# gvanhorn38/multibox

Hardware: AMD Instinct MI355X
Metric: images/sec (299x299, 5-AR priors) train (higher is better)
Workload: dtype bf16; 1 GPU; full train step: Inception-ResNet-v2 + multibox heads fwd, on-device matching+loss, bwd, RMSProp+EMA; 299x299, k=5 (P=646), BATCH_SIZE=64/GPU, MAX_NUM_BBOXES=13; global_batch=64, parallelism=dp1, hip_graph=True

## Files before the change

include/mbx.h:

```cpp
#ifndef MBX_H
#define MBX_H

#include <stddef.h>
#include <stdint.h>

#ifdef __cplusplus
extern "C" {
#endif

typedef void* mbx_stream_t;

typedef enum {
  MBX_OK = 0,
  MBX_ERR_INVALID_ARG = -1,
  MBX_ERR_UNSUPPORTED = -2,
  MBX_ERR_LAUNCH = -3,
  MBX_ERR_WORKSPACE = -4
} mbx_status;

int mbx_version(void);
const char* mbx_status_string(int status);

int mbx_priors_count(int k, const int* grids, int n_grids);

uint32_t mbx_crc32c(const void* data, uint64_t n, uint32_t crc);
int mbx_generate_priors(const double* aspect_ratios, int k, double min_scale, double max_scale,
                        int restrict_to_image_bounds, const int* grids, int n_grids,
                        double* out );

int mbx_decode_conf(const float* raw_locs , const float* logits ,
                    const float* priors , int B, int P, float eps_add,
                    float* decoded , float* conf , mbx_stream_t stream);

size_t mbx_match_workspace_bytes(int B, int P, int G);
int mbx_match(const float* decoded , const float* conf ,
              const float* gt , const int32_t* n_gt , float alpha,
              int B, int P, int G, int32_t* match , int32_t* status ,
              void* workspace, size_t workspace_bytes, mbx_stream_t stream);

size_t mbx_loss_workspace_bytes(int B);
int mbx_loss_fwd_bwd(const float* decoded , const float* conf_in ,
                     int conf_is_logit, const float* gt ,
                     const int32_t* match , float alpha, float grad_scale, int B, int P,
                     int G, float* loss2 ,
                     float* d_raw_locs , float* d_logits ,
                     void* workspace, size_t workspace_bytes, mbx_stream_t stream);

typedef struct {
  int32_t offset_y, offset_x;
  int32_t patch_h, patch_w;
  int32_t image_h, image_w;
  int32_t is_flipped;
  int32_t max_to_keep;
  float restrictions[4];
} mbx_patch_meta;

int mbx_decode_filter_topk(const float* raw_locs , const float* conf ,
                           const float* priors , const mbx_patch_meta* meta ,
                           int B, int P, int k_max, double* out_boxes ,
                           float* out_scores , int32_t* out_index ,
                           int32_t* out_count , mbx_stream_t stream);

int mbx_nms(double* boxes , float* scores , int32_t* index ,
            int32_t* count , int B, int k_max, double iou_threshold, mbx_stream_t stream);

#define MBX_MERGE_MAX_CANDIDATES 16384
int mbx_merge_detections(const double* boxes , const float* scores ,
                         const int32_t* count , const int32_t* image_rows , int I, int k_max,
                         int max_det, double iou_threshold, double* out_boxes ,
                         float* out_scores , int32_t* out_src ,
                         int32_t* out_count , int32_t* out_status , mbx_stream_t stream);

typedef enum {
  MBX_EPI_STORE = 0,
  MBX_EPI_AFFINE = 1,
  MBX_EPI_RESIDUAL = 2,
  MBX_EPI_STORE_F32 = 3
} mbx_epilogue;

typedef struct {
  int32_t n, rows_mod;
  int32_t c_begin[4];
  const void* y[4]; int32_t ld_y[4];
  const float* relu_thr[4];
  float* stats[4]; int32_t stats_ld[4];
} mbx_bn_bwd_stats;

#define MBX_GRID_BARRIER_BYTES 6400
typedef struct {
  void* barrier;
  void* a; int32_t ld_a;
  const float* beta;
  float* mean; float* rstd;
  float* moving_mean; float* moving_var;
  float* relu_thr;
  int32_t relu; float eps, decay;
  float* step_poison;
} mbx_bn_apply_desc;

#define MBX_BN_BWD_SLOTS 8
typedef struct {
  void* barrier;
  int32_t n;
  int32_t c_begin[4];
  const void* y[4]; int32_t ld_y[4];
  void* dy[4]; int32_t ld_dy[4];
  const float* mean[4]; const float* rstd[4]; const float* beta[4];
  float* dbeta[4];
  float* acc[4]; int32_t acc_ld[4];
  int32_t relu[4];
  float* step_poison;
} mbx_bn_bwd_fused;

typedef struct {
  const void* x; int64_t x_img_stride; int32_t ldx;
  int32_t N, H_in, W_in, C_in;
  const void* w; int32_t C_out, R, S;
  int32_t stride, transposed, pad_t, pad_l, H_out, W_out;
  void* y; int64_t y_img_stride; int32_t ldy;
  int32_t epilogue, relu, accumulate;
  const float* scale; const float* shift;
  const void* skip; int64_t skip_img_stride; int32_t ld_skip; float rscale;
  float* stats_partial;
  int32_t tile_config;
  const void* acc_src; int64_t acc_img_stride; int32_t ld_acc;
  int32_t* work_counter;
  int32_t max_workgroups;
  void* splitk_ws; int64_t splitk_ws_bytes;
  int32_t stats_rows_mod, stats_ld;
  const mbx_bn_bwd_stats* bn_bwd_stats;
  void* relu_bits; int32_t ld_bits;
  const mbx_bn_apply_desc* bn_apply;
  const mbx_bn_bwd_fused* bn_bwd;
} mbx_conv_desc;
#define MBX_CONV_TILE_CONFIGS 14

int mbx_conv_stats_rows(const mbx_conv_desc* desc );
int mbx_conv(const mbx_conv_desc* desc , mbx_stream_t stream);
int mbx_conv_supported(const mbx_conv_desc* desc );
int mbx_conv_pair(const mbx_conv_desc* a , const mbx_conv_desc* b , mbx_stream_t stream);
size_t mbx_conv_splitk_workspace_bytes(const mbx_conv_desc* desc );

int mbx_conv_wgrad(const mbx_conv_desc* desc , const void* dy,
                   int64_t dy_img_stride, int32_t ld_dy, float* dw, float* db, mbx_stream_t stream);

typedef struct {
  mbx_conv_desc desc;
  const void* dy; int64_t dy_img_stride; int32_t ld_dy;
  float scale;
  float* dw; float* db;
} mbx_wgrad_job;
typedef struct {
  int32_t n_layers, n_items;
  int64_t layers_off, items_off;
  int64_t queues_off, heads_off;
  double flops;
  int64_t tally_off;
} mbx_wgrad_plan_info;
#define MBX_WGRAD_DETERMINISTIC 1
#define MBX_WGRAD_SCATTER 2
size_t mbx_wgrad_plan_bytes(const mbx_wgrad_job* jobs , int n_jobs, int flags);
int mbx_wgrad_plan(const mbx_wgrad_job* jobs , int n_jobs, int flags, void* host_image, size_t bytes,
                   mbx_wgrad_plan_info* info );
int mbx_conv_wgrad_grouped(void* device_image , const mbx_wgrad_plan_info* info ,
                           mbx_stream_t stream);
int mbx_conv_wgrad_grouped_capped(void* device_image, const mbx_wgrad_plan_info* info , int max_workgroups,
                                  mbx_stream_t stream);

int mbx_conv_wgrad_scaled(const mbx_conv_desc* desc, const void* dy, int64_t dy_img_stride,
                          int32_t ld_dy, float scale, float* dw, float* db, mbx_stream_t stream);

int mbx_bn_finalize(const float* stats_partial , int rows, int C, int64_t count,
                    float eps, float decay, float* mean , float* rstd ,
                    float* moving_mean , float* moving_var ,
                    mbx_stream_t stream);
int mbx_bn_apply(const void* y, int64_t M, int C, const float* mean, const float* rstd,
                 const float* beta, int relu, void* a, int ld_a, mbx_stream_t stream);
int mbx_bn_apply_fused(const float* stats_partial, int rows, int64_t count, float eps, float decay,
                       const void* y, int64_t M, int C, const float* beta, int relu, void* a, int ld_a,
                       float* mean, float* rstd, float* moving_mean, float* moving_var,
                       mbx_stream_t stream);
int mbx_bn_apply_fused_mapped(const void* stats_fixed, int rows, int64_t count, float eps, float decay,
                              const void* y, int64_t M, int C, const float* beta, int relu, void* a, int ld_a,
                              const struct mbx_chan_map_s* a_map , float* mean, float* rstd, float* moving_mean,
                              float* moving_var, float* relu_thr, mbx_stream_t stream);
int mbx_bn_moving_update(float* moving_mean, float* moving_var, const float* batch_mean, const float* batch_var,
                         int64_t n, float decay, const float* skip_ctl, uint64_t* skipped_steps,
                         float* ema_mean, float* ema_var, float ema_decay, mbx_stream_t stream);
typedef struct mbx_chan_map_s { int32_t n; int32_t c_begin[4]; int32_t offset[4]; } mbx_chan_map;
int mbx_bn_finalize_parts(const float* const* parts , const int32_t* rows ,
                          const int32_t* Cs , int n_parts, int64_t count, float eps, float decay, float* mean,
                          float* rstd, float* moving_mean, float* moving_var, mbx_stream_t stream);
int mbx_bn_apply_mapped(const void* y, int64_t M, int C, const float* mean, const float* rstd, const float* beta,
                        int relu, void* a, int ld_a, const mbx_chan_map* a_map , mbx_stream_t stream);
int mbx_bn_apply_maxpool(const void* y, int N, int H, int W, int C, const float* mean, const float* rstd, const float* beta,
                         int relu, void* p, int64_t p_img_stride, int ld_p, int Ho, int Wo, uint8_t* argmax,
                         mbx_stream_t stream);
int mbx_bn_fold(const float* moving_mean, const float* moving_var, const float* beta, float eps,
                int C, float* scale, float* shift, mbx_stream_t stream);
int mbx_bn_bwd_rows(int64_t M, int C);
int mbx_bn_bwd_reduce(const void* da, int ld_da, const void* a, int ld_a, int relu, const void* y,
                      int64_t M, int C, const float* mean, const float* rstd, const float* beta,
                      float* partial , mbx_stream_t stream);
int mbx_bn_bwd_finalize(const float* partial, int rows, int C, int64_t M, float* dbeta ,
                        float* m12 , mbx_stream_t stream);
int mbx_bn_bwd_apply(const void* da, int ld_da, const void* a, int ld_a, int relu, const void* y,
                     int64_t M, int C, const float* mean, const float* rstd, const float* beta,
                     const float* m12, void* dy , mbx_stream_t stream);

int mbx_bn_bwd_reduce_mapped(const void* da, int ld_da, const void* a, int ld_a, int relu, const void* y, int64_t M, int C,
                             const float* mean, const float* rstd, const float* beta, float* partial,
                             const mbx_chan_map* da_map , mbx_stream_t stream);
int mbx_bn_bwd_apply_mapped(const void* da, int ld_da, const void* a, int ld_a, int relu, const void* y, int64_t M, int C,
                            const float* mean, const float* rstd, const float* beta, const float* m12, void* dy,
                            const mbx_chan_map* da_map , mbx_stream_t stream);

int mbx_bn_bwd_apply_rows(const float* stats, int rows, const void* da, int ld_da, const void* y, int64_t M, int C,
                          const float* mean, const float* rstd, const float* relu_thr, float* dbeta, void* dy,
                          const mbx_chan_map* da_map , mbx_stream_t stream);

size_t mbx_bn_bwd_onepass_workspace_bytes(int C);
int mbx_bn_bwd_onepass_supported(int64_t M, int C, int max_workgroups);
int mbx_bn_bwd_onepass(const void* da, int ld_da, int relu, const void* y, int64_t M, int C,
                       const float* mean, const float* rstd, const float* beta, float* dbeta ,
                       void* dy , void* ws, int max_workgroups, float* step_poison ,
                       mbx_stream_t stream);

int mbx_bn_bwd_rows_pooled(int N, int H, int W, int C);
int mbx_bn_bwd_reduce_pooled(const void* gy, int64_t gy_img_stride, int ld_gy, const uint8_t* argmax, int N, int H, int W,
                             int Ho, int Wo, int relu, const void* y, int C, const float* mean, const float* rstd,
                             const float* beta, float* partial , mbx_stream_t stream);
int mbx_bn_bwd_apply_pooled(const void* gy, int64_t gy_img_stride, int ld_gy, const uint8_t* argmax, int N, int H, int W,
                            int Ho, int Wo, int relu, const void* y, int C, const float* mean, const float* rstd,
                            const float* beta, const float* m12, void* dy, mbx_stream_t stream);
int mbx_bn_bwd_onepass_mapped(const void* da, int ld_da, int relu, const void* y, int64_t M, int C, const float* mean,
                              const float* rstd, const float* beta, float* dbeta, void* dy, void* ws, int max_workgroups,
                              float* step_poison, const mbx_chan_map* da_map , mbx_stream_t stream);

int mbx_maxpool_fwd(const void* x, int64_t x_img_stride, int ldx, int N, int H, int W, int C,
                    int k, int stride, void* y, int64_t y_img_stride, int ldy, int Ho, int Wo,
                    uint8_t* argmax , mbx_stream_t stream);
int mbx_maxpool_bwd(const void* dy, int64_t dy_img_stride, int ld_dy, const uint8_t* argmax,
                    int N, int H, int W, int C, int k, int stride, int Ho, int Wo, void* dx,
                    int64_t dx_img_stride, int ld_dx, int accumulate, mbx_stream_t stream);
int mbx_avgpool_fwd(const void* x, int64_t x_img_stride, int ldx, int N, int H, int W, int C,
                    int k, int pad, void* y, int64_t y_img_stride, int ldy, int Ho, int Wo,
                    mbx_stream_t stream);
int mbx_avgpool_bwd(const void* dy, int64_t dy_img_stride, int ld_dy, int N, int H, int W, int C,
                    int k, int pad, int Ho, int Wo, void* dx, int64_t dx_img_stride, int ld_dx,
                    int accumulate, mbx_stream_t stream);

int mbx_relu_mask(void* g, int ld_g, const void* a, int ld_a, int64_t M, int C, mbx_stream_t stream);
int mbx_pack_input(const float* img, int64_t pixels, void* out, mbx_stream_t stream);
int mbx_head_gather(const float* h, int ld_h, int N, int cells, int k, int P, int off,
                    float* locs, float* logits, mbx_stream_t stream);
int mbx_head_scatter(const float* d_locs, const float* d_logits, int N, int cells, int k, int P,
                     int off, void* g, int ld_g, mbx_stream_t stream);

typedef struct {
  const float* h; int32_t ld_h;
  void* g; int32_t ld_g;
  int32_t cells, k, off;
} mbx_head;
int mbx_head_gather_all(const mbx_head* heads , int n_heads, int N, int P, float* locs, float* logits,
                        mbx_stream_t stream);
int mbx_head_scatter_all(const float* d_locs, const float* d_logits, const mbx_head* heads , int n_heads, int N,
                         int P, mbx_stream_t stream);

int mbx_step_begin(float* grads, int64_t n_grads, float* bn_ws, int64_t n_ws, int64_t ctl_index, uint64_t* timeouts_total,
                   float* zero_scalar, mbx_stream_t stream);

typedef struct {
  int64_t src_off;
  int64_t dst_off;
  int32_t K, R, S, C, Kpad;
  int32_t first_block;
} mbx_filter_entry;
int mbx_filter_prepare(const void* w_bf16, void* w_dgrad, const mbx_filter_entry* table ,
                       int n_entries, int total_blocks, mbx_stream_t stream);

int mbx_rmsprop_ema_step(float* w, const float* g, float* ms, float* mom ,
                         float* ema , void* w_bf16 , int64_t n, float lr,
                         float decay, float momentum, float eps, float wd, float ema_decay,
                         int trainable, float* reg_loss, const float* skip_ctl, mbx_stream_t stream);
int mbx_ema_update(float* ema, const float* value, int64_t n, float ema_decay, const float* skip_ctl ,
                   mbx_stream_t stream);

typedef struct {
  uint64_t src_offset;
  int32_t src_h, src_w;
  int32_t method;
  int32_t flip;
  int32_t n_ops;
  int32_t op[4];
  int32_t pad_;
  double arg[4];
} mbx_augment_item;
size_t mbx_augment_workspace_bytes(int B, int S);
int mbx_augment_batch(const uint8_t* src , const mbx_augment_item* items , int B, int S,
                      int any_contrast, float* out , void* workspace, mbx_stream_t stream);

typedef struct {
  uint64_t src_offset;
  int32_t img_h, img_w;
  int32_t win_y, win_x, win_h, win_w;
  int32_t flip_source;
  int32_t pad_;
} mbx_patch_item;
int mbx_extract_patches(const uint8_t* src , const mbx_patch_item* items , int n, int S,
                        float* out , mbx_stream_t stream);

#ifdef __cplusplus
}
#endif
#endif
```

multibox_amd/_lib.py:

```python
from __future__ import annotations

import ctypes as C
import os

_HERE = os.path.dirname(os.path.abspath(__file__))
LIB_PATH = os.path.join(_HERE, "libmbx.so")

P = C.c_void_p
I = C.c_int
F = C.c_float
D = C.c_double
SZ = C.c_size_t


class PatchMeta(C.Structure):
    _fields_ = [("offset_y", C.c_int32), ("offset_x", C.c_int32), ("patch_h", C.c_int32), ("patch_w", C.c_int32),
                ("image_h", C.c_int32), ("image_w", C.c_int32), ("is_flipped", C.c_int32),
                ("max_to_keep", C.c_int32), ("restrictions", C.c_float * 4)]


_SIGS = {
    "mbx_version": (I, []),
    "mbx_status_string": (C.c_char_p, [I]),
    "mbx_priors_count": (I, [I, P, I]),
    "mbx_crc32c": (C.c_uint32, [P, C.c_uint64, C.c_uint32]),
    "mbx_generate_priors": (I, [P, I, D, D, I, P, I, P]),
    "mbx_decode_conf": (I, [P, P, P, I, I, F, P, P, P]),
    "mbx_match_workspace_bytes": (SZ, [I, I, I]),
    "mbx_match": (I, [P, P, P, P, F, I, I, I, P, P, P, SZ, P]),
    "mbx_loss_workspace_bytes": (SZ, [I]),
    "mbx_loss_fwd_bwd": (I, [P, P, I, P, P, F, F, I, I, I, P, P, P, P, SZ, P]),
    "mbx_decode_filter_topk": (I, [P, P, P, P, I, I, I, P, P, P, P, P]),
    "mbx_nms": (I, [P, P, P, P, I, I, C.c_double, P]),
    "mbx_merge_detections": (I, [P, P, P, P, I, I, I, C.c_double, P, P, P, P, P, P]),
    "mbx_augment_workspace_bytes": (SZ, [I, I]),
    "mbx_augment_batch": (I, [P, P, I, I, I, P, P, P]),
    "mbx_extract_patches": (I, [P, P, I, I, P, P]),
    "mbx_conv_stats_rows": (I, [P]),
    "mbx_conv": (I, [P, P]),
    "mbx_conv_supported": (I, [P]),
    "mbx_conv_pair": (I, [P, P, P]),
    "mbx_conv_splitk_workspace_bytes": (SZ, [P]),
    "mbx_conv_wgrad": (I, [P, P, C.c_int64, I, P, P, P]),
    "mbx_conv_wgrad_scaled": (I, [P, P, C.c_int64, I, F, P, P, P]),
    "mbx_wgrad_plan_bytes": (SZ, [P, I, I]),
    "mbx_wgrad_plan": (I, [P, I, I, P, SZ, P]),
    "mbx_conv_wgrad_grouped": (I, [P, P, P]),
    "mbx_conv_wgrad_grouped_capped": (I, [P, P, I, P]),
    "mbx_bn_finalize": (I, [P, I, I, C.c_int64, F, F, P, P, P, P, P]),
    "mbx_bn_apply": (I, [P, C.c_int64, I, P, P, P, I, P, I, P]),
    "mbx_bn_moving_update": (I, [P, P, P, P, C.c_int64, F, P, P, P, P, F, P]),
    "mbx_bn_finalize_parts": (I, [P, P, P, I, C.c_int64, F, F, P, P, P, P, P]),
    "mbx_bn_apply_mapped": (I, [P, C.c_int64, I, P, P, P, I, P, I, P, P]),
    "mbx_bn_bwd_reduce_mapped": (I, [P, I, P, I, I, P, C.c_int64, I, P, P, P, P, P, P]),
    "mbx_bn_bwd_apply_mapped": (I, [P, I, P, I, I, P, C.c_int64, I, P, P, P, P, P, P, P]),
    "mbx_bn_apply_maxpool": (I, [P, I, I, I, I, P, P, P, I, P, C.c_int64, I, I, I, P, P]),
    "mbx_bn_bwd_rows_pooled": (I, [I, I, I, I]),
    "mbx_bn_bwd_reduce_pooled": (I, [P, C.c_int64, I, P, I, I, I, I, I, I, P, I, P, P, P, P, P]),
    "mbx_bn_bwd_apply_pooled": (I, [P, C.c_int64, I, P, I, I, I, I, I, I, P, I, P, P, P, P, P, P]),
    "mbx_bn_bwd_onepass_mapped": (I, [P, I, I, P, C.c_int64, I, P, P, P, P, P, P, I, P, P, P]),
    "mbx_bn_fold": (I, [P, P, P, F, I, P, P, P]),
    "mbx_bn_apply_fused": (I, [P, I, C.c_int64, F, F, P, C.c_int64, I, P, I, P, I, P, P, P, P, P]),
    "mbx_bn_apply_fused_mapped": (I, [P, I, C.c_int64, F, F, P, C.c_int64, I, P, I, P, I, P, P, P, P, P, P, P]),
    "mbx_bn_bwd_apply_rows": (I, [P, I, P, I, P, C.c_int64, I, P, P, P, P, P, P, P]),
    "mbx_bn_bwd_rows": (I, [C.c_int64, I]),
    "mbx_bn_bwd_onepass_workspace_bytes": (C.c_size_t, [I]),
    "mbx_bn_bwd_onepass_supported": (I, [C.c_int64, I, I]),
    "mbx_bn_bwd_onepass": (I, [P, I, I, P, C.c_int64, I, P, P, P, P, P, P, I, P, P]),
    "mbx_bn_bwd_reduce": (I, [P, I, P, I, I, P, C.c_int64, I, P, P, P, P, P]),
    "mbx_bn_bwd_finalize": (I, [P, I, I, C.c_int64, P, P, P]),
    "mbx_bn_bwd_apply": (I, [P, I, P, I, I, P, C.c_int64, I, P, P, P, P, P, P]),
    "mbx_maxpool_fwd": (I, [P, C.c_int64, I, I, I, I, I, I, I, P, C.c_int64, I, I, I, P, P]),
    "mbx_maxpool_bwd": (I, [P, C.c_int64, I, P, I, I, I, I, I, I, I, I, P, C.c_int64, I, I, P]),
    "mbx_avgpool_fwd": (I, [P, C.c_int64, I, I, I, I, I, I, I, P, C.c_int64, I, I, I, P]),
    "mbx_avgpool_bwd": (I, [P, C.c_int64, I, I, I, I, I, I, I, I, I, P, C.c_int64, I, I, P]),
    "mbx_relu_mask": (I, [P, I, P, I, C.c_int64, I, P]),
    "mbx_pack_input": (I, [P, C.c_int64, P, P]),
    "mbx_head_gather": (I, [P, I, I, I, I, I, I, P, P, P]),
    "mbx_head_scatter": (I, [P, P, I, I, I, I, I, P, I, P]),
    "mbx_head_gather_all": (I, [P, I, I, I, P, P, P]),
    "mbx_head_scatter_all": (I, [P, P, P, I, I, I, P]),
    "mbx_step_begin": (I, [P, C.c_int64, P, C.c_int64, C.c_int64, P, P, P]),
    "mbx_filter_prepare": (I, [P, P, P, I, I, P]),
    "mbx_rmsprop_ema_step": (I, [P, P, P, P, P, P, C.c_int64, F, F, F, F, F, F, I, P, P, P]),
    "mbx_ema_update": (I, [P, P, C.c_int64, F, P, P]),
}

_lib = None


class MbxError(RuntimeError):
    pass


class ChanMap(C.Structure):
    _fields_ = [("n", C.c_int32), ("c_begin", C.c_int32 * 4), ("offset", C.c_int32 * 4)]


class BnBwdStats(C.Structure):
    _fields_ = [("n", C.c_int32), ("rows_mod", C.c_int32), ("c_begin", C.c_int32 * 4), ("y", C.c_void_p * 4), ("ld_y", C.c_int32 * 4),
                ("relu_thr", C.c_void_p * 4), ("stats", C.c_void_p * 4), ("stats_ld", C.c_int32 * 4)]


class Head(C.Structure):
    _fields_ = [("h", C.c_void_p), ("ld_h", C.c_int32), ("g", C.c_void_p), ("ld_g", C.c_int32), ("cells", C.c_int32),
                ("k", C.c_int32), ("off", C.c_int32)]


class FilterEntry(C.Structure):
    _fields_ = [("src_off", C.c_int64), ("dst_off", C.c_int64), ("K", C.c_int32), ("R", C.c_int32), ("S", C.c_int32),
                ("C", C.c_int32), ("Kpad", C.c_int32), ("first_block", C.c_int32)]


def lib():
    global _lib
    if _lib is None:
        if not os.path.exists(LIB_PATH):
            raise MbxError("libmbx.so not built at %s -- run `python -c 'import __graft_entry__ as g; g.build()'` "
                           "(needs hipcc); there is no CPU fallback" % LIB_PATH)
        import torch
        l = C.CDLL(LIB_PATH)
        for name, (res, args) in _SIGS.items():
            fn = getattr(l, name)
            fn.restype = res
            fn.argtypes = args
        _lib = l
    return _lib


def check(status, what=""):
    if status != 0:
        msg = lib().mbx_status_string(int(status))
        raise MbxError("%s failed: %s (%d)" % (what or "libmbx call", msg.decode() if msg else "?", status))


def declared_symbols():
    return sorted(_SIGS)
```

multibox_amd/build.py:

```python
from __future__ import annotations

import os
import shutil
import subprocess
import sys

HERE = os.path.dirname(os.path.abspath(__file__))
CSRC = os.path.join(HERE, "csrc")
OBJ = os.path.join(CSRC, "_obj")
LIB = os.path.join(HERE, "libmbx.so")
ARCH = "gfx950"

SOURCES = {
    "priors.cpp": ["-ffp-contract=off"],
    "postproc.hip": ["-ffp-contract=off"],
    "merge.hip": ["-ffp-contract=off"],
    "conv.hip": ["-munsafe-fp-atomics"],
    "conv5.hip": ["-mllvm", "-amdgpu-atomic-optimizer-strategy=None"],
    "conv7.hip": ["-mllvm", "-amdgpu-atomic-optimizer-strategy=None"],
    "convd.hip": [],
    "convr.hip": [],
    "nnops.hip": ["-munsafe-fp-atomics"],
    "augment.hip": ["-ffp-contract=off"],
}
COMMON = ["-O3", "-std=c++17", "-fPIC", "--offload-arch=" + ARCH, "-Wall", "-Wno-unused-function"]
COMMON += os.environ.get("MBX_BUILD_DEFS", "").split()


def _hipcc():
    for c in (shutil.which("hipcc"), "/opt/rocm/bin/hipcc"):
        if c and os.path.exists(c):
            return c
    raise RuntimeError("hipcc not found: libmbx needs ROCm's hipcc to build")


def _newer(a, bs):
    if not os.path.exists(a):
        return True
    ta = os.path.getmtime(a)
    return any(os.path.getmtime(b) > ta for b in bs)


def build(force=False, verbose=True):
    hipcc = _hipcc()
    os.makedirs(OBJ, exist_ok=True)
    headers = [os.path.join(CSRC, f) for f in os.listdir(CSRC) if f.endswith(".h")]
    headers.append(os.path.join(os.path.dirname(HERE), "include", "mbx.h"))
    headers.append(os.path.abspath(__file__))
    objs = []
    procs = []
    for src, flags in SOURCES.items():
        s = os.path.join(CSRC, src)
        o = os.path.join(OBJ, src.rsplit(".", 1)[0] + ".o")
        objs.append(o)
        if force or _newer(o, [s] + headers):
            cmd = [hipcc] + COMMON + flags + (["-x", "hip"] if src.endswith(".hip") else []) + ["-c", s, "-o", o]
            if verbose:
                print("[mbx build]", " ".join(cmd), flush=True)
            procs.append((src, subprocess.Popen(cmd, stdout=subprocess.PIPE, stderr=subprocess.STDOUT, text=True)))
    failed = []
    for src, p in procs:
        out, _ = p.communicate()
        if p.returncode != 0:
            failed.append((src, out))
        elif verbose and out.strip():
            print(out)
    if failed:
        raise RuntimeError("hipcc failed:\n" + "\n".join("== %s ==\n%s" % f for f in failed))
    if force or _newer(LIB, objs):
        cmd = [hipcc, "-shared", "-fPIC", "--offload-arch=" + ARCH, "-o", LIB] + objs
        if verbose:
            print("[mbx build]", " ".join(cmd), flush=True)
        subprocess.check_call(cmd)
    return LIB


if __name__ == "__main__":
    build(force="--force" in sys.argv)
    print(LIB)
```

multibox_amd/csrc/conv.hip:

```cpp
#include <stdlib.h>
#include <string.h>
#include <algorithm>
#include <vector>

#include "conv_common.h"

int mbx_launch_igemm5(void* convk, int index, hipStream_t s);
int mbx_launch_igemm7(void* convk, hipStream_t s);
int mbx_launch_direct3(void* convk, int N, int H_out, hipStream_t s);
int mbx_direct3_grid(int N, int H_out, int W_out);
int mbx_launch_directw(void* convk, int N, int H_out, hipStream_t s);
int mbx_directw_grid(int N, int H_out, int W_out);
int mbx_launch_resident(void* convk, int N, int H_out, hipStream_t s);
int mbx_resident_rows(int N);
int mbx_launch_pwres(void* convk, hipStream_t s);
extern const int mbx_i5_tiles[][2];
extern const int mbx_i5_num_tiles;

namespace {

template <int BM, int BN, int WNW, int WMW, int EV, int MODE = 0, int NSTG = 3>
__device__ __forceinline__ void conv_igemm3_body(const ConvK& p, const int bid_, const int nblk_) {
  constexpr bool SH = MODE == 2, PW = MODE == 1;
  static_assert(WNW * WMW == 4 || WNW * WMW == 8, "four or eight waves");
// ... 56 lines not shown
    if (c0 == pixel_class(p, mlast)) {
      kr0 = (p.pad_t + (c0 >> 1)) & 1;
      ks0 = (p.pad_l + (c0 & 1)) & 1;
      kstep = 2;
      nk = ((p.R - kr0 + 1) >> 1) * ((p.S - ks0 + 1) >> 1) * (p.C_in >> 6);
    }
  }
  int kt0 = 0;
  if constexpr (EV == 5) { kt0 = split * p.kps; nk = min(p.kps, nk - kt0); }
  int kc = chunk * 8 + kt0 * 64, kr = kr0, ks = ks0;
  while (kc >= p.C_in) { kc -= p.C_in; if ((ks += kstep) >= p.S) { ks = ks0; kr += kstep; } }
  const int ldx2 = p.ldx * 2;
  int st_issue = 0, st_comp = 0;
#define MBX_ISSUE_TILE(LT)                                                                                   \
  do {                                                                                                       \
    u32x4* sp = smem + st_issue * STAGE + wave * 64;                                                         \
    const bool kv = kr < p.R;                                                                                \
    if (PW) {                                                                                                \
      _Pragma("unroll") for (int i = 0; i < PI; ++i)                                                         \
        glds16(xr, sp + i * NT, (kv && ro[i] >= 0) ? (ro[i] + kc * 2) : (int)kOOB);                          \
    } else if (!SH) {                                                                                        \
      const int toff = (kr * p.W_in + ks) * ldx2 + kc * 2;                                                   \
      _Pragma("unroll") for (int i = 0; i < PI; ++i) {                                                       \
        const bool ok = kv && ((unsigned)(hb[i] + kr) < (unsigned)p.H_in) &&                                 \
                        ((unsigned)(wb[i] + ks) < (unsigned)p.W_in);                                         \
        glds16(xr, sp + i * NT, ok ? (ro[i] + toff) : (int)kOOB);                                            \
      }                                                                                                      \
    } else {                                                                                                 \
      _Pragma("unroll") for (int i = 0; i < PI; ++i) {                                                       \
        const int hn = hb[i] + kr, wn_ = wb[i] + ks;                                                         \
        const bool ok = kv && (((hn | wn_) & 1) == 0) && ((unsigned)(hn >> 1) < (unsigned)p.H_in) &&         \
                        ((unsigned)(wn_ >> 1) < (unsigned)p.W_in);                                           \
        glds16(xr, sp + i * NT, ok ? (ro[i] + ((hn >> 1) * p.W_in + (wn_ >> 1)) * ldx2 + kc * 2) : (int)kOOB); \
      }                                                                                                      \
    }                                                                                                        \
                                 \
    const int kb = (SH && kstep == 2) ? ((kr * p.S + ks) * p.C_in + kc + (chunkw - chunk) * 8) * 2                \
                                      : (((LT) + kt0) * 64 + chunkw * 8) * 2;                                  \
    const bool kvw = (SH && kstep == 2) ? kv : (kb < p.Ktot * 2);                                              \
    u32x4* sw = sp + BM * 8;                                                                                 \
    _Pragma("unroll") for (int i = 0; i < WI; ++i)                                                           \
      glds16(wr, sw + i * NT, (kvw && wo[i] >= 0) ? (wo[i] + kb) : (int)kOOB);                               \
    kc += 64;                                                                                                \
    while (kc >= p.C_in) { kc -= p.C_in; if ((ks += kstep) >= p.S) { ks = ks0; kr += kstep; } }              \
    st_issue = st_issue == NSTG - 1 ? 0 : st_issue + 1;                                                      \
  } while (0)

  static_assert(NSTG == 2 || NSTG == 3, "ring depth");
  u32x4* const probe_base = smem + (PI + WI - 1) * NT + wave * 64 + lane;
  MBX_ISSUE_TILE(0);
  if (NSTG == 3 && nk > 1) { MBX_ISSUE_TILE(1); wait_vmcnt<NL>(); } else wait_vmcnt<0>();
  lds_readback_wait(lds_readback_issue(probe_base));
  raw_barrier();
  for (int it = 0; it < nk; ++it) {
    const bool more = it + NSTG - 1 < nk;
    if (more) MBX_ISSUE_TILE(it + NSTG - 1);
    st_comp = st_comp == NSTG - 1 ? 0 : st_comp + 1;
    const int st_prev = st_comp == 0 ? NSTG - 1 : st_comp - 1;
#ifndef MBX_NO_PROBE_I3
    unsigned probe;
    if constexpr (NSTG == 3) {
      if (more) wait_vmcnt<NL>(); else wait_vmcnt<0>();
      probe = lds_readback_issue(probe_base + st_comp * STAGE);
    }
#endif
    {
      const u32x4* cP = smem + st_prev * STAGE + (wm * TM) * 8;
      const u32x4* cW = smem + st_prev * STAGE + BM * 8 + (wn * TN) * 8;
#pragma unroll
      for (int kk = 0; kk < 2; ++kk) {
        const int fr = kk ? fr1 : fr0, fw = kk ? fw1 : fw0;
        bf16x8 wf[NI], pf[MI];
#pragma unroll
        for (int a = 0; a < NI; ++a) wf[a] = __builtin_bit_cast(bf16x8, cW[(a >> 1) * 256 + (a & 1) * 32 + fw]);
#pragma unroll
        for (int b = 0; b < MI; ++b) pf[b] = __builtin_bit_cast(bf16x8, cP[b * 128 + fr]);
#pragma unroll
        for (int a = 0; a < NI; ++a)
#pragma unroll
          for (int b = 0; b < MI; ++b)
            acc[a][b] = __builtin_amdgcn_mfma_f32_16x16x32_bf16(wf[a], pf[b], acc[a][b], 0, 0, 0);
      }
    }
#ifndef MBX_NO_PROBE_I3
    if constexpr (NSTG == 2) {
      wait_vmcnt<0>();
      probe = lds_readback_issue(probe_base + st_comp * STAGE);
    }
    lds_readback_wait(probe);
#else
    if (NSTG == 3 && more) wait_vmcnt<NL>(); else wait_vmcnt<0>();
#endif
    raw_barrier();
  }
#undef MBX_ISSUE_TILE
  wait_vmcnt<0>();
  static_assert(NI % 2 == 0, "wave tile: a multiple of 32 output channels");
  constexpr int NA = NI / 2;
  const int cl0 = wn * TN + fch * 8;
  if constexpr (EV == 5) {
#pragma unroll
    for (int b = 0; b < MI; ++b) {
      const int m = m0 + wm * TM + b * 16 + frow;
      if (m >= p.M) continue;
      const int img = (int)fast_div((unsigned)m, p.mg_hw, p.sh_hw), pix = m - img * p.HW_out;
      float* yrow = reinterpret_cast<float*>(p.y) + split * p.y_split_stride + img * p.y_img_stride + pix * p.ldy;
#pragma unroll
      for (int a = 0; a < NI; ++a) {
        const int c0 = n0 + cl0 + 32 * (a >> 1) + 4 * (a & 1);
#pragma unroll
        for (int r = 0; r < 4; ++r)
          if (c0 + r < p.C_out) yrow[c0 + r] = acc[a][b][r];
      }
    }
  } else {
    float s1[NA][8], s2[NA][8];
    conv_epilogue_direct<EV, SH, NI, MI, ((EV == 2 || EV == 6) && MI * NA >= 8 && MI % 2 == 0) ? 2 : MI>(p, acc, m0 + wm * TM + frow, n0 + cl0, s1, s2);
    if constexpr (EV == 1 || EV == 6) {
      float* red = reinterpret_cast<float*>(smem);
#pragma unroll
      for (int A = 0; A < NA; ++A) { row_sum16_x8(s1[A]); row_sum16_x8(s2[A]); }
#pragma unroll
      for (int A = 0; A < NA; ++A)
#pragma unroll
        for (int j = 0; j < 8; ++j) {
          const float x1 = s1[A][j], x2 = s2[A][j];
          if (frow == 0) {
            red[((wm * BN) + cl0 + 32 * A + j) * 2] = x1;
            red[((wm * BN) + cl0 + 32 * A + j) * 2 + 1] = x2;
          }
        }
      __syncthreads();
      if (tid < BN && n0 + tid < p.C_out) {
        float x1 = 0.f, x2 = 0.f;
#pragma unroll
        for (int w = 0; w < WMW; ++w) { x1 += red[(w * BN + tid) * 2]; x2 += red[(w * BN + tid) * 2 + 1]; }
        if constexpr (EV == 6) bw_stats_write(p, tile_m, n0 + tid, x1, x2); else stats_write(p, tile_m, n0 + tid, x1, x2);
      }
    }
  }
}

template <int BM, int BN, int WNW, int WMW, int EV, int MODE = 0, int NSTG = 3>
__global__ void __launch_bounds__(64 * WNW * WMW)
conv_igemm3_kernel(const ConvK p) {
  conv_igemm3_body<BM, BN, WNW, WMW, EV, MODE, NSTG>(p, (int)blockIdx.x, (int)gridDim.x);
}

template <int BM, int BN, int WNW, int WMW, int EV, int MODE = 0, int NSTG = 3>
__global__ void __launch_bounds__(64 * WNW * WMW)
conv_igemm3_pair_kernel(const ConvK p0, const ConvK p1, const int n0) {
  if ((int)blockIdx.x < n0) conv_igemm3_body<BM, BN, WNW, WMW, EV, MODE, NSTG>(p0, (int)blockIdx.x, n0);
  else conv_igemm3_body<BM, BN, WNW, WMW, EV, MODE, NSTG>(p1, (int)blockIdx.x - n0, (int)gridDim.x - n0);
}


struct WgradK {
  const unsigned short* x; int x_img_stride, ldx, H_in, W_in, C_in;
  const unsigned short* dy; int dy_img_stride, ld_dy;
  int C_out, S, Ktot, stride, pad_t, pad_l, W_out, HW_out, M;
  float* dw; float* db; float scale;
  unsigned x_bytes, dy_bytes;
  unsigned mg_hw, sh_hw, mg_w, sh_w;
  int H_out;
  int tiles_n, tiles_k, m_per_split;
};

__device__ __forceinline__ int wg_swz(int row) { return ((row & 3) | (((row >> 3) & 1) << 2)) << 1; }

struct WgradK2 {
  WgradK b;
  int pw;
  int ydense;
  int dbg;
};

template <int NST, int NG, bool LIN, bool BIAS>
__device__ __forceinline__ void wgrad_wide_body(const WgradK2& q, u32x4* smem, const int tile_n, const int tile_k,
                                                const int blk_begin, const int blk_end) {
  const WgradK& p = q.b;
  constexpr int STAGE = 2 * 64 * 16;
  const int lane = threadIdx.x & 63;
  const int wave8 = wave_id();
  const int grp = NG == 2 ? (wave8 >> 2) : 0, wave = wave8 & 3;
  const int tid = threadIdx.x & 255;
  const int wn = wave & 1, wk = wave >> 1;
  const int n0 = tile_n * 128, k0 = tile_k * 128;
  const int half = NG == 2 ? ((((blk_end - blk_begin) + 1) / 2 + 63) & ~63) : (blk_end - blk_begin);
  const int m_begin = blk_begin + grp * half;
  const int m_end = NG == 2 ? (grp == 0 ? min(blk_end, blk_begin + half) : blk_end) : blk_end;
  const __amdgpu_buffer_rsrc_t xr = make_rsrc(p.x, p.x_bytes);
  const __amdgpu_buffer_rsrc_t yr = make_rsrc(p.dy, p.dy_bytes);

  const int r4 = lane >> 4;
  const int swz = ((r4 & 3) | (((wave >> 1) & 1) << 2)) << 1;
  const int lc = (lane & 15) ^ swz;
  const int kcol = k0 + lc * 8;
  const bool kvalid = kcol < p.Ktot;
  const int tap = (kvalid ? kcol : 0) / p.C_in, tc = (kvalid ? kcol : 0) - tap * p.C_in;
  const int tr = kvalid ? tap / p.S : (1 << 24), ts = tap - (tap / p.S) * p.S;
  const int toff = ((tr * p.W_in + ts) * p.ldx + tc) * 2;
  const int ycol = (n0 + lc * 8 < p.C_out) ? (n0 + lc * 8) * 2 : -1;
  const int ldx2 = p.ldx * 2, ldy2 = p.ld_dy * 2;
  int m_run = m_begin + wave * 4 + r4;
  int img = 0, oh = 0, ow = 0;
  {
    const unsigned mm = (unsigned)min(m_run, p.M - 1);
    img = (int)fast_div(mm, p.mg_hw, p.sh_hw);
    const int pix = (int)mm - img * p.HW_out;
    oh = (int)fast_div((unsigned)pix, p.mg_w, p.sh_w);
    ow = pix - oh * p.W_out;
  }

  const int g = lane >> 4, t = lane & 15, fq = t >> 2, pp = t & 3;
  const int lb = (8 * g + fq) * 256 + (pp & 1) * 8;
  const int sx = ((fq & 3) | ((g & 1) << 2)) << 1;
  int yo[4], xo[4];
#pragma unroll
  for (int a = 0; a < 4; ++a) {
    yo[a] = lb + (((2 * (wn * 4 + a) + (pp >> 1)) ^ sx) << 4);
    xo[a] = lb + (((2 * (wk * 4 + a) + (pp >> 1)) ^ sx) << 4) + 64 * 256;
  }

  f32x4 acc[4][4];
#pragma unroll
  for (int a = 0; a < 4; ++a)
#pragma unroll
    for (int b = 0; b < 4; ++b) acc[a][b] = f32x4{0.f, 0.f, 0.f, 0.f};
  float bsum = 0.f;
  const bool do_bias = BIAS && p.db != nullptr && tile_k == 0 && tid < 128 && n0 + tid < p.C_out;

  const int nsteps = (half + 63) >> 6;
  int st_issue = 0, st_comp = 0;
  typedef s16x4 __attribute__((address_space(3))) * lds_tr;
  typedef __attribute__((ext_vector_type(8))) short s16x8;
#define MBX_ISSUE_STEP()                                                                                      \
  do {                                                                                                        \
    u32x4* sp = smem + (grp * NST + st_issue) * STAGE + wave * 64;                                            \
    _Pragma("unroll") for (int i = 0; i < 4; ++i) {                                                           \
      const bool mv = m_run < m_end;                                                                          \
      int xoff, yoff;                                                                                         \
      if (LIN || q.pw) xoff = (mv && kvalid) ? (m_run * ldx2 + kcol * 2) : (int)kOOB;                         \
      else {                                                                                                  \
        const int hb = oh * p.stride - p.pad_t + tr, wb = ow * p.stride - p.pad_l + ts;                       \
        const bool ok = mv && ((unsigned)hb < (unsigned)p.H_in) && ((unsigned)wb < (unsigned)p.W_in);         \
        xoff = ok ? ((img * p.x_img_stride + ((oh * p.stride - p.pad_t) * p.W_in + ow * p.stride - p.pad_l) * p.ldx) * 2 + toff) \
                  : (int)kOOB;                                                                                \
      }                                                                                                       \
      if (LIN || q.ydense) yoff = (mv && ycol >= 0) ? (m_run * ldy2 + ycol) : (int)kOOB;                      \
      else yoff = (mv && ycol >= 0) ? ((img * p.dy_img_stride + (oh * p.W_out + ow) * p.ld_dy) * 2 + ycol) : (int)kOOB; \
      glds16(yr, sp + i * 256, yoff);                                                                         \
      glds16(xr, sp + 1024 + i * 256, xoff);                                                                  \
      m_run += 16;                                                                                            \
      if (!LIN && !(q.pw && q.ydense)) {                                                                      \
        ow += 16;                                                                                             \
        while (ow >= p.W_out) { ow -= p.W_out; ++oh; }                                                        \
        while (oh >= p.H_out) { oh -= p.H_out; ++img; }                                                       \
      }                                                                                                       \
    }                                                                                                         \
    st_issue = st_issue == NST - 1 ? 0 : st_issue + 1;                                                        \
  } while (0)

  static_assert(NST == 2, "ring depth 2: one step in flight");
  if (nsteps > 0) MBX_ISSUE_STEP();
  wait_vmcnt<0>();
  raw_barrier();
  for (int it = 0; it < nsteps; ++it) {
    if (it + 1 < nsteps) MBX_ISSUE_STEP();
    {
      const char* base = reinterpret_cast<const char*>(smem + (grp * NST + st_comp) * STAGE);
#pragma unroll
      for (int kk = 0; kk < 2; ++kk) {
        bf16x8 yf[4], xf[4];
#pragma unroll
        for (int a = 0; a < 4; ++a) {
          const s16x4 lo = __builtin_amdgcn_ds_read_tr16_b64_v4i16((lds_tr)(base + yo[a] + kk * 8192));
          const s16x4 hi = __builtin_amdgcn_ds_read_tr16_b64_v4i16((lds_tr)(base + yo[a] + kk * 8192 + 1024));
          const s16x8 v = {lo[0], lo[1], lo[2], lo[3], hi[0], hi[1], hi[2], hi[3]};
          yf[a] = __builtin_bit_cast(bf16x8, v);
        }
#pragma unroll
        for (int b = 0; b < 4; ++b) {
          const s16x4 lo = __builtin_amdgcn_ds_read_tr16_b64_v4i16((lds_tr)(base + xo[b] + kk * 8192));
          const s16x4 hi = __builtin_amdgcn_ds_read_tr16_b64_v4i16((lds_tr)(base + xo[b] + kk * 8192 + 1024));
          const s16x8 v = {lo[0], lo[1], lo[2], lo[3], hi[0], hi[1], hi[2], hi[3]};
          xf[b] = __builtin_bit_cast(bf16x8, v);
        }
#pragma unroll
        for (int a = 0; a < 4; ++a)
#pragma unroll
          for (int b = 0; b < 4; ++b)
            acc[a][b] = __builtin_amdgcn_mfma_f32_16x16x32_bf16(yf[a], xf[b], acc[a][b], 0, 0, 0);
      }
      if (do_bias) {
        const unsigned short* cY = reinterpret_cast<const unsigned short*>(base);
        const int ch = tid >> 3, e = tid & 7;
        for (int r = 0; r < 64; ++r) bsum += bf2f(cY[r * 128 + ((ch ^ wg_swz(r)) << 3) + e]);
      }
      st_comp = st_comp == NST - 1 ? 0 : st_comp + 1;
    }
    wait_vmcnt<0>();
    if (it + 1 < nsteps) {
      lds_readback_wait(lds_readback_issue(smem + (grp * NST + (st_issue ^ 1)) * STAGE + wave * 64 + lane));
    }
    raw_barrier();
  }
// ... 631 lines not shown
    const long tiles5 = ((M + 255) / 256) * ((C_out + 127) / 128);
    const long rounds5 = (tiles5 + 255) / 256;
    if (tiles5 >= 128 && (double)tiles5 / (double)(rounds5 * 256) >= 0.7) return 5;
  }
  return pick_cfg(M, C_out);
}

struct PairCapture { ConvK k; int bm, bn, wnw, wmw, nstg, ev, mode, valid; };
thread_local PairCapture g_capture;

template <int BM, int BN, int WNW, int WMW, int EV, int NSTG>
int launch_pair_inst(const ConvK& a, const ConvK& b, hipStream_t s) {
  static bool attr = false;
  const size_t lds = NSTG * (size_t)(BM + BN) * 128;
  if (!attr) {
    (void)hipFuncSetAttribute(reinterpret_cast<const void*>(conv_igemm3_pair_kernel<BM, BN, WNW, WMW, EV, 0, NSTG>),
                              hipFuncAttributeMaxDynamicSharedMemorySize, (int)lds);
    attr = true;
  }
  const int n0 = a.tiles_m * a.tiles_n, n1 = b.tiles_m * b.tiles_n;
  hipLaunchKernelGGL((conv_igemm3_pair_kernel<BM, BN, WNW, WMW, EV, 0, NSTG>), dim3(n0 + n1), dim3(64 * WNW * WMW), lds, s, a, b, n0);
  MBX_LAUNCH_CHECK();
  return MBX_OK;
}

template <int BM, int BN, int WNW, int WMW, int NSTG = 3>
int launch_igemm(ConvK& k, hipStream_t s) {
  k.tiles_m = (k.M + BM - 1) / BM;
  k.tiles_n = (k.C_out + BN - 1) / BN;
  k.stats_cap = stats_cap_for(k.tiles_m);
  if (k.dry == 2) {
    g_capture.k = k; g_capture.bm = BM; g_capture.bn = BN; g_capture.wnw = WNW; g_capture.wmw = WMW; g_capture.nstg = NSTG;
    g_capture.ev = k.epi == MBX_EPI_STORE_F32 ? 5 : k.epi == MBX_EPI_RESIDUAL ? 4 : k.epi == MBX_EPI_AFFINE ? 3
                   : k.bw_n ? 6 : k.stats ? 1 : (k.accumulate || k.skip || k.bits) ? 2 : 0;
    g_capture.mode = k.shift ? 2 : k.pw ? 1 : 0;
    g_capture.valid = 1;
    return MBX_OK;
  }
  {
    const size_t lds = NSTG * (size_t)(BM + BN) * 128;
    const int ev = k.epi == MBX_EPI_STORE_F32 ? 5 : k.epi == MBX_EPI_RESIDUAL ? 4 : k.epi == MBX_EPI_AFFINE ? 3
                   : k.bw_n ? 6 : k.stats ? 1 : (k.accumulate || k.skip || k.bits) ? 2 : 0;
    static bool attr_set3[7] = {false, false, false, false, false, false, false};
#define MBX_LAUNCH_EV(EV)                                                                                     \
    case EV:                                                                                                  \
      if (!attr_set3[EV]) {                                                                                   \
        (void)hipFuncSetAttribute(reinterpret_cast<const void*>(conv_igemm3_kernel<BM, BN, WNW, WMW, EV, 0, NSTG>), \
                                  hipFuncAttributeMaxDynamicSharedMemorySize, (int)lds);                      \
        (void)hipFuncSetAttribute(reinterpret_cast<const void*>(conv_igemm3_kernel<BM, BN, WNW, WMW, EV, 1, NSTG>), \
                                  hipFuncAttributeMaxDynamicSharedMemorySize, (int)lds);                      \
        attr_set3[EV] = true;                                                                                 \
      }                                                                                                       \
      if (k.pw)                                                                                               \
        hipLaunchKernelGGL((conv_igemm3_kernel<BM, BN, WNW, WMW, EV, 1, NSTG>), dim3(k.tiles_m * k.tiles_n * (EV == 5 ? k.ksplit : 1)), \
                           dim3(64 * WNW * WMW), lds, s, k);                                                  \
      else                                                                                                    \
        hipLaunchKernelGGL((conv_igemm3_kernel<BM, BN, WNW, WMW, EV, 0, NSTG>), dim3(k.tiles_m * k.tiles_n * (EV == 5 ? k.ksplit : 1)), \
                           dim3(64 * WNW * WMW), lds, s, k);                                                  \
      break;
    static bool attr_sh[2] = {false, false};
#define MBX_LAUNCH_SH(EV, SLOT)                                                                               \
    do {                                                                                                      \
      if (!attr_sh[SLOT]) {                                                                                   \
        (void)hipFuncSetAttribute(reinterpret_cast<const void*>(conv_igemm3_kernel<BM, BN, WNW, WMW, EV, 2, NSTG>), \
                                  hipFuncAttributeMaxDynamicSharedMemorySize, (int)lds);                      \
        attr_sh[SLOT] = true;                                                                                 \
      }                                                                                                       \
      hipLaunchKernelGGL((conv_igemm3_kernel<BM, BN, WNW, WMW, EV, 2, NSTG>), dim3(k.tiles_m * k.tiles_n),      \
                         dim3(64 * WNW * WMW), lds, s, k);                                                    \
    } while (0)
    if (k.dry) return (k.shift && ev != 0 && ev != 2) ? MBX_ERR_UNSUPPORTED : MBX_OK;
    if (k.shift) {
      if (ev == 0) MBX_LAUNCH_SH(0, 0);
      else if (ev == 2) MBX_LAUNCH_SH(2, 1);
      else return MBX_ERR_UNSUPPORTED;
    } else
    switch (ev) {
      MBX_LAUNCH_EV(0) MBX_LAUNCH_EV(1) MBX_LAUNCH_EV(2) MBX_LAUNCH_EV(3) MBX_LAUNCH_EV(4) MBX_LAUNCH_EV(5) MBX_LAUNCH_EV(6)
    }
#undef MBX_LAUNCH_SH
#undef MBX_LAUNCH_EV
  }
  MBX_LAUNCH_CHECK();
  return MBX_OK;
}

void set_magic(unsigned d, unsigned& mg, unsigned& sh) {
  unsigned l = 0;
  while ((1ull << l) < d) ++l;
  sh = 31 + l;
  mg = (unsigned)((1ull << sh) / d + 1);
}

int check_desc(const mbx_conv_desc* d) {
  if (!d || !d->x || !d->N || d->N < 0) return MBX_ERR_INVALID_ARG;
  if (d->C_in <= 0 || d->C_in % 8 || d->ldx % 8 || d->ldx < d->C_in) return MBX_ERR_INVALID_ARG;
  if (d->R <= 0 || d->S <= 0 || d->C_out <= 0 || d->H_out <= 0 || d->W_out <= 0) return MBX_ERR_INVALID_ARG;
  if (d->stride != 1 && d->stride != 2) return MBX_ERR_UNSUPPORTED;
  if ((reinterpret_cast<uintptr_t>(d->x) & 15)) return MBX_ERR_INVALID_ARG;
  const long long xe = (long long)d->N * d->x_img_stride;
  if (xe >= (1LL << 30) || (long long)d->N * d->H_out * d->W_out >= (1LL << 31)) return MBX_ERR_UNSUPPORTED;
  return MBX_OK;
}

}

extern "C" int mbx_conv_stats_rows(const mbx_conv_desc* d) {
  if (!d) return MBX_ERR_INVALID_ARG;
  if (d->stats_rows_mod > 0) return d->stats_rows_mod;
  const long M = (long)d->N * d->H_out * d->W_out;
  if (d->tile_config > kSplitFlag) return (int)((M + kSplitRows - 1) / kSplitRows);
  if (d->tile_config == kDirectCfg) return mbx_direct3_grid(d->N, d->H_out, d->W_out);
  if (d->tile_config == kDirectWCfg) { const int g = mbx_directw_grid(d->N, d->H_out, d->W_out); return g > 0 ? g : MBX_ERR_UNSUPPORTED; }
  if (d->tile_config == kResidentCfg) return mbx_resident_rows(d->N);
  if (d->tile_config == kI7Cfg) return (int)((M + 127) / 128);
  if (d->tile_config > kI5Flag) {
    const int i = d->tile_config - kI5Flag - 1;
    if (i >= mbx_i5_num_tiles) return MBX_ERR_INVALID_ARG;
    return (int)((M + mbx_i5_tiles[i][0] - 1) / mbx_i5_tiles[i][0]);
  }
  const TileCfg& c = kCfgs[choose_cfg(M, d->C_out, d->tile_config)];
  return (int)((M + c.BM - 1) / c.BM);
}

static int conv_impl(const mbx_conv_desc* d, mbx_stream_t stream, int dry);
extern "C" int mbx_conv(const mbx_conv_desc* d, mbx_stream_t stream) { return conv_impl(d, stream, 0); }
extern "C" int mbx_conv_supported(const mbx_conv_desc* d) { return conv_impl(d, nullptr, 1); }
extern "C" int mbx_conv_pair(const mbx_conv_desc* a, const mbx_conv_desc* b, mbx_stream_t stream) {
  PairCapture ca, cb;
  g_capture.valid = 0;
  int st = conv_impl(a, stream, 2);
  if (st != MBX_OK) return st;
  if (!g_capture.valid) return MBX_ERR_UNSUPPORTED;
  ca = g_capture;
  g_capture.valid = 0;
  st = conv_impl(b, stream, 2);
  if (st != MBX_OK) return st;
  if (!g_capture.valid) return MBX_ERR_UNSUPPORTED;
  cb = g_capture;
  if (ca.bm != cb.bm || ca.bn != cb.bn || ca.wnw != cb.wnw || ca.wmw != cb.wmw || ca.nstg != cb.nstg || ca.ev != cb.ev ||
      ca.mode != 0 || cb.mode != 0 || (ca.ev != 0 && ca.ev != 1 && ca.ev != 6) || ca.wnw != 2 || ca.wmw != 2 || ca.bn != 64)
    return MBX_ERR_UNSUPPORTED;
  ca.k.dry = cb.k.dry = 0;
  hipStream_t s = mbx_s(stream);
#define MBX_PAIR(BM_, NSTG_)                                                                                      \
  if (ca.bm == BM_ && ca.nstg == NSTG_)                                                                           \
    return ca.ev == 6 ? launch_pair_inst<BM_, 64, 2, 2, 6, NSTG_>(ca.k, cb.k, s)                                    \
           : ca.ev ? launch_pair_inst<BM_, 64, 2, 2, 1, NSTG_>(ca.k, cb.k, s) : launch_pair_inst<BM_, 64, 2, 2, 0, NSTG_>(ca.k, cb.k, s);
  MBX_PAIR(128, 2) MBX_PAIR(128, 3) MBX_PAIR(64, 2) MBX_PAIR(64, 3)
#undef MBX_PAIR
  return MBX_ERR_UNSUPPORTED;
}

extern "C" size_t mbx_conv_splitk_workspace_bytes(const mbx_conv_desc* d) {
  if (!d || d->tile_config <= kSplitFlag || d->tile_config > kSplitFlag + kSplitMax) return 0;
  int ksplit, kps;
  splitk_geom((d->R * d->S * d->C_in + 63) >> 6, d->tile_config - kSplitFlag, ksplit, kps);
  return (size_t)4 * d->N * d->H_out * d->W_out * (((d->C_out + 7) / 8) * 8) * ksplit;
}

static int conv_impl(const mbx_conv_desc* d, mbx_stream_t stream, int dry) {
  int st = check_desc(d);
  if (st != MBX_OK) return st;
  if (!d->w || !d->y) return MBX_ERR_INVALID_ARG;
  if ((reinterpret_cast<uintptr_t>(d->w) & 15)) return MBX_ERR_INVALID_ARG;
  const bool f32 = d->epilogue == MBX_EPI_STORE_F32;
  if (!f32 && (d->C_out % 8 || d->ldy % 8 || (reinterpret_cast<uintptr_t>(d->y) & 15))) return MBX_ERR_INVALID_ARG;
  if (d->epilogue == MBX_EPI_RESIDUAL && (!d->skip || d->ld_skip % 8 || (reinterpret_cast<uintptr_t>(d->skip) & 15)))
    return MBX_ERR_INVALID_ARG;
  if ((long long)d->N * d->y_img_stride >= (1LL << 31)) return MBX_ERR_UNSUPPORTED;
  if (d->stats_partial && (d->epilogue != MBX_EPI_STORE || d->accumulate || d->skip)) return MBX_ERR_INVALID_ARG;
  if (d->epilogue == MBX_EPI_STORE && d->skip && (d->ld_skip % 8 || (reinterpret_cast<uintptr_t>(d->skip) & 15))) return MBX_ERR_INVALID_ARG;
  MBX_ENTER();
  ConvK k;
  k.x = reinterpret_cast<const unsigned short*>(d->x);
  k.x_img_stride = (int)d->x_img_stride; k.ldx = d->ldx; k.H_in = d->H_in; k.W_in = d->W_in; k.C_in = d->C_in;
  k.w = reinterpret_cast<const unsigned short*>(d->w);
  k.C_out = d->C_out; k.R = d->R; k.S = d->S; k.Ktot = d->R * d->S * d->C_in;
  k.x_bytes = (unsigned)(2 * ((long long)(d->N - 1) * d->x_img_stride + ((long long)d->H_in * d->W_in - 1) * d->ldx + d->C_in));
  k.w_bytes = (unsigned)(2LL * d->C_out * k.Ktot);
  if (d->transposed) { k.mul = 1; k.shift = d->stride == 2 ? 1 : 0; } else { k.mul = d->stride; k.shift = 0; }
  k.pad_t = d->pad_t; k.pad_l = d->pad_l; k.W_out = d->W_out; k.HW_out = d->H_out * d->W_out;
  k.M = d->N * k.HW_out;
  k.y = d->y; k.y_img_stride = (int)d->y_img_stride; k.ldy = d->ldy;
  k.epi = d->epilogue; k.relu = d->relu; k.accumulate = d->accumulate;
  k.scale = d->scale; k.shiftv = d->shift;
  k.skip = reinterpret_cast<const unsigned short*>(d->skip);
  k.skip_img_stride = (int)d->skip_img_stride; k.ld_skip = d->ld_skip; k.rscale = d->rscale;
  k.bits = nullptr; k.bits_ld = 0; k.bits_bytes = 0;
  if (d->relu_bits) {
    const bool wr = d->epilogue == MBX_EPI_RESIDUAL && d->relu, rd = d->epilogue == MBX_EPI_STORE && !d->skip;
    if ((!wr && !rd) || d->ld_bits % 4 || d->ld_bits < 4 * ((d->C_out + 31) / 32) || (reinterpret_cast<uintptr_t>(d->relu_bits) & 3)) return MBX_ERR_INVALID_ARG;
    if (d->stats_partial || d->bn_bwd_stats) return MBX_ERR_UNSUPPORTED;
    const long long bb = (long long)d->N * d->H_out * d->W_out * d->ld_bits;
    if (bb >= (1LL << 31)) return MBX_ERR_UNSUPPORTED;
    k.bits = reinterpret_cast<unsigned char*>(d->relu_bits); k.bits_ld = d->ld_bits; k.bits_bytes = (unsigned)bb;
  }
  k.stats = d->stats_partial;
  if (d->stats_rows_mod < 0 || d->stats_rows_mod > 1024 || d->stats_ld < 0 || (d->stats_ld && d->stats_ld < d->C_out)) return MBX_ERR_INVALID_ARG;
  k.stats_mod = d->stats_rows_mod; k.stats_ld = d->stats_ld ? d->stats_ld : d->C_out;
  k.stats_cap = 0.f;
  k.fa = FusedApply{};
  k.fa.bar = nullptr;
  k.fb = FusedBwd{};
  k.fb.bar = nullptr;
  if (d->bn_bwd) {
    const mbx_bn_bwd_fused* b = d->bn_bwd;
    if (!b->barrier || (reinterpret_cast<uintptr_t>(b->barrier) & 127) || b->n < 1 || b->n > 4 || b->c_begin[0] != 0) return MBX_ERR_INVALID_ARG;
    if (d->epilogue != MBX_EPI_STORE || d->accumulate || d->skip || d->relu_bits || d->stats_partial || d->bn_bwd_stats || d->bn_apply ||
        d->stride != 1 || d->C_out > 2048 || d->y_img_stride != (int64_t)d->H_out * d->W_out * d->ldy)
      return MBX_ERR_UNSUPPORTED;
    const int tc = d->tile_config;
    if (!((tc > kI5Flag && tc <= kI5Flag + 7) || tc == kDirectWCfg || tc == kResidentCfg)) return MBX_ERR_UNSUPPORTED;
    const long long Mll = (long long)d->N * d->H_out * d->W_out;
    for (int i = 0; i < 4; ++i) k.fb.cb[i] = 1 << 30;
    for (int i = 0; i < b->n; ++i) {
      if (!b->y[i] || !b->dy[i] || !b->mean[i] || !b->rstd[i] || (b->relu[i] && !b->beta[i]) || !b->acc[i] ||
          (reinterpret_cast<uintptr_t>(b->y[i]) & 15) || (reinterpret_cast<uintptr_t>(b->dy[i]) & 15) || b->ld_y[i] % 8 || b->ld_dy[i] % 8 ||
          b->c_begin[i] % 8 || b->c_begin[i] >= d->C_out || (i && b->c_begin[i] <= b->c_begin[i - 1]) || b->acc_ld[i] <= 0)
        return MBX_ERR_INVALID_ARG;
      if (Mll * b->ld_y[i] >= (1LL << 31) || Mll * b->ld_dy[i] >= (1LL << 31)) return MBX_ERR_UNSUPPORTED;
      k.fb.cb[i] = b->c_begin[i];
      k.fb.y[i] = reinterpret_cast<const unsigned short*>(b->y[i]); k.fb.ldy[i] = b->ld_y[i];
      k.fb.dy[i] = reinterpret_cast<unsigned short*>(b->dy[i]); k.fb.lddy[i] = b->ld_dy[i];
      k.fb.mean[i] = b->mean[i]; k.fb.rstd[i] = b->rstd[i]; k.fb.beta[i] = b->beta[i]; k.fb.dbeta[i] = b->dbeta[i];
      k.fb.acc[i] = b->acc[i]; k.fb.acc_ld[i] = b->acc_ld[i]; k.fb.relu[i] = b->relu[i];
    }
    static int fault = -1;
    if (fault < 0) { const char* e = getenv("MBX_DEBUG_BARRIER_FAULT"); fault = (e && e[0] == '3') ? 1 : 0; }
    k.fb.n = b->n;
    k.fb.bar = reinterpret_cast<unsigned*>(b->barrier);
    static int probe = -1;
    if (probe < 0) { const char* e = getenv("MBX_FUSED_PROBE"); probe = e ? (atoi(e) & ~1) : 0; }
    k.fb.spin_limit = fault ? (1u << 10) : (1u << 22); k.fb.fault = fault | probe; k.fb.step_poison = b->step_poison;
    k.fb.inv_M = (float)(1.0 / (double)Mll);
  }
  if (d->bn_apply) {
    const mbx_bn_apply_desc* b = d->bn_apply;
    if (!b->barrier || !b->a || !b->beta || !b->mean || !b->rstd || (reinterpret_cast<uintptr_t>(b->barrier) & 127) ||
        (reinterpret_cast<uintptr_t>(b->a) & 15) || b->ld_a % 8 || b->ld_a < d->C_out)
      return MBX_ERR_INVALID_ARG;
    if (!d->stats_partial || d->stats_rows_mod < 1 || d->stats_rows_mod > 16 || d->epilogue != MBX_EPI_STORE || d->accumulate || d->skip ||
        d->transposed || d->rscale != 0.f || d->C_out > 2048 || d->y_img_stride != (int64_t)d->H_out * d->W_out * d->ldy ||
        (long long)d->N * d->H_out * d->W_out * b->ld_a >= (1LL << 31))
      return MBX_ERR_UNSUPPORTED;
    const int tc = d->tile_config;
    if (!((tc > kI5Flag && tc <= kI5Flag + 7) || tc == kDirectWCfg || tc == kResidentCfg)) return MBX_ERR_UNSUPPORTED;
    static int fault = -1;
    if (fault < 0) { const char* e = getenv("MBX_DEBUG_BARRIER_FAULT"); fault = (e && e[0] == '2') ? 1 : 0; }
    k.fa.bar = reinterpret_cast<unsigned*>(b->barrier);
    static int probe = -1;
    if (probe < 0) { const char* e = getenv("MBX_FUSED_PROBE"); probe = e ? (atoi(e) & ~1) : 0; }
    k.fa.spin_limit = fault ? (1u << 10) : (1u << 22); k.fa.fault = fault | probe; k.fa.step_poison = b->step_poison;
    k.fa.a = reinterpret_cast<unsigned short*>(b->a); k.fa.ld_a = b->ld_a; k.fa.beta = b->beta;
    k.fa.mean = b->mean; k.fa.rstd = b->rstd; k.fa.mmean = b->moving_mean; k.fa.mvar = b->moving_var; k.fa.thr = b->relu_thr;
    k.fa.relu = b->relu; k.fa.eps = b->eps; k.fa.decay = b->decay;
    k.fa.inv_count = 1.0 / (double)((long long)d->N * d->H_out * d->W_out);
  }
  k.bw_n = 0; k.bw_mod = 1;
  for (int i = 0; i < 4; ++i) { k.bw_cb[i] = 1 << 30; k.bw_ldy[i] = 0; k.bw_sld[i] = 0; k.bw_y[i] = nullptr; k.bw_thr[i] = nullptr; k.bw_stats[i] = nullptr; }
  if (d->bn_bwd_stats) {
    const mbx_bn_bwd_stats* b = d->bn_bwd_stats;
    if (d->epilogue != MBX_EPI_STORE || d->accumulate || d->skip || d->stats_partial || b->n < 1 || b->n > 4 || b->rows_mod < 1 ||
        b->rows_mod > 1024 || b->c_begin[0] != 0)
      return MBX_ERR_INVALID_ARG;
    for (int i = 0; i < b->n; ++i) {
      if (!b->y[i] || !b->relu_thr[i] || !b->stats[i] || (reinterpret_cast<uintptr_t>(b->y[i]) & 15) || b->ld_y[i] % 8 || b->c_begin[i] % 32 ||
          b->c_begin[i] >= d->C_out || (i && b->c_begin[i] <= b->c_begin[i - 1]) || b->stats_ld[i] <= 0)
        return MBX_ERR_INVALID_ARG;
      k.bw_cb[i] = b->c_begin[i]; k.bw_ldy[i] = b->ld_y[i]; k.bw_sld[i] = b->stats_ld[i];
      k.bw_y[i] = reinterpret_cast<const unsigned short*>(b->y[i]); k.bw_thr[i] = b->relu_thr[i]; k.bw_stats[i] = b->stats[i];
    }
    k.bw_n = b->n; k.bw_mod = b->rows_mod;
  }
  if (d->accumulate && d->acc_src) {
    if (d->ld_acc % 8 || (reinterpret_cast<uintptr_t>(d->acc_src) & 15) || (long long)d->N * d->acc_img_stride >= (1LL << 31))
      return MBX_ERR_INVALID_ARG;
    k.acc_src = reinterpret_cast<const unsigned short*>(d->acc_src); k.acc_img_stride = (int)d->acc_img_stride; k.ld_acc = d->ld_acc;
  } else {
    k.acc_src = reinterpret_cast<const unsigned short*>(d->y); k.acc_img_stride = (int)d->y_img_stride; k.ld_acc = d->ldy;
  }
  {
    const long long last_pix = (long long)k.HW_out - 1, span = ((d->C_out + 7) / 8) * 8;
    const long long yb = 2 * ((long long)(d->N - 1) * d->y_img_stride + last_pix * d->ldy + span);
    const long long sb = d->skip ? 2 * ((long long)(d->N - 1) * d->skip_img_stride + last_pix * d->ld_skip + span) : 0;
    const long long ab = 2 * ((long long)(d->N - 1) * k.acc_img_stride + last_pix * k.ld_acc + span);
    if (!f32 && (yb >= (1LL << 31) || sb >= (1LL << 31) || ab >= (1LL << 31))) return MBX_ERR_UNSUPPORTED;
    k.y_bytes = (unsigned)yb; k.skip_bytes = (unsigned)sb; k.acc_bytes = (unsigned)ab;
  }
  set_magic((unsigned)k.HW_out, k.mg_hw, k.sh_hw);
  set_magic((unsigned)k.W_out, k.mg_w, k.sh_w);
  k.pw = (d->R == 1 && d->S == 1 && d->pad_t == 0 && d->pad_l == 0 && d->stride == 1) ? 1 : 0;
  k.skip_taps = 0; k.parity = 0;
  k.work_counter = d->work_counter;
  k.max_wg = d->max_workgroups;
  k.dry = dry;
  k.ksplit = 1; k.kps = 1 << 30; k.y_split_stride = 0;
#ifdef MBX_I5_STAMPS
  {
    static const unsigned long long sp = getenv("MBX_I5_STAMP_PTR") ? strtoull(getenv("MBX_I5_STAMP_PTR"), nullptr, 10) : 0ull;
    k.stamps = reinterpret_cast<unsigned long long*>(sp);
    k.dbg = getenv("MBX_I5_DBG") ? atoi(getenv("MBX_I5_DBG")) : 0;
    k.stagger = getenv("MBX_STAGGER") ? atoi(getenv("MBX_STAGGER")) : 0;
  }
#endif
  for (int c = 0; c < 4; ++c) { k.cls_m0[c] = 0; k.cls_hw[c] = 1; k.cls_w[c] = 1; }
// ... 379 lines not shown
```

multibox_amd/csrc/nnops.hip:

```cpp
#include "common.h"
#include <stdlib.h>
#include <string.h>

namespace {

__device__ __forceinline__ int xcd_logical(int bid, int nblk) {
  const int xcd = bid & 7, q = nblk >> 3, r = nblk & 7;
  return (xcd < r ? xcd * (q + 1) : r * (q + 1) + (xcd - r) * q) + (bid >> 3);
}
inline int xcd_rows_on() { static const int v = [] { const char* e = getenv("MBX_XCD_ROWS"); return e ? atoi(e) : 0; }(); return v; }


typedef __attribute__((ext_vector_type(4))) unsigned int u32x4;
typedef __attribute__((ext_vector_type(2))) unsigned int u32x2;
constexpr int kT = 256;

__device__ __forceinline__ float bf2f(unsigned h) { return __uint_as_float(h << 16); }
__device__ __forceinline__ unsigned f2bf(float f) { return (unsigned)__builtin_bit_cast(unsigned short, (__bf16)f); }
__device__ __forceinline__ unsigned pack2bf(float lo, float hi) {
  typedef float pk_f32x2 __attribute__((ext_vector_type(2)));
  typedef __bf16 pk_bf16x2 __attribute__((ext_vector_type(2)));
  return __builtin_bit_cast(unsigned, __builtin_convertvector(pk_f32x2{lo, hi}, pk_bf16x2));
}
__device__ __forceinline__ float relu_f(float x) {
// ... 211 lines not shown
    for (int j = 0; j < 8; ++j) { s1[j] = 0.f; s2[j] = 0.f; }
    for (int r = 0; r < rpi; ++r) {
      const float* o = sred + ((size_t)r * C8 + threadIdx.x) * 16;
#pragma unroll
      for (int j = 0; j < 8; ++j) { s1[j] += o[j]; s2[j] += o[8 + j]; }
    }
    float* p = partial + ((size_t)blockIdx.x * C + (threadIdx.x << 3)) * 2;
#pragma unroll
    for (int j = 0; j < 8; ++j) { p[2 * j] = s1[j]; p[2 * j + 1] = s2[j]; }
  }
}

__global__ void __launch_bounds__(kT)
bn_bwd_finalize_kernel(const float* __restrict__ part, int rows, int C, double inv_M, float* __restrict__ dbeta,
                       float* __restrict__ m12) {
  const int c = blockIdx.x;
  double s1 = 0.0, s2 = 0.0;
  for (int r = threadIdx.x; r < rows; r += kT) {
    const float2 v = *reinterpret_cast<const float2*>(part + ((size_t)r * C + c) * 2);
    s1 += v.x; s2 += v.y;
  }
  block_sum2(s1, s2);
  if (threadIdx.x == 0) {
    if (dbeta) dbeta[c] += (float)s1;
    m12[c] = (float)(s1 * inv_M);
    m12[C + c] = (float)(s2 * inv_M);
  }
}

template <int MASK>
__global__ void __launch_bounds__(kT)
bn_bwd_apply_kernel(const unsigned short* __restrict__ da, int ld_da, const unsigned short* __restrict__ a, int ld_a,
                    const unsigned short* __restrict__ y, long long M, int C,
                    const float* __restrict__ mean, const float* __restrict__ rstd, const float* __restrict__ beta,
                    const float* __restrict__ m12, unsigned short* __restrict__ dy, const ChanMap map) {
  const int C8 = C >> 3;
  const long long total = M * C8;
  for (long long i = (long long)blockIdx.x * kT + threadIdx.x; i < total; i += (long long)gridDim.x * kT) {
    const long long m = i / C8;
    const int c = (int)(i - m * C8) << 3;
    float g[8], yy[8], aa[8], o[8];
    unpack8(ld8(da + m * ld_da + c + chan_off(map, c)), g);
    unpack8(ld8(y + m * C + c), yy);
    if (MASK == 1) unpack8(ld8(a + m * ld_a + c), aa);
#pragma unroll
    for (int j = 0; j < 8; ++j) {
      const float rs = rstd[c + j];
      const float xh = (yy[j] - mean[c + j]) * rs;
      const bool pass = MASK == 0 || (MASK == 1 ? aa[j] > 0.f : xh + beta[c + j] > 0.f);
      const float gj = pass ? g[j] : 0.f;
      o[j] = rs * (gj - m12[c + j] - xh * m12[C + c + j]);
    }
    st8(dy + m * C + c, pack8(o));
  }
}

constexpr int kBnGroup = 64;

__global__ void __launch_bounds__(kT)
bn_apply_fused_kernel(const float* __restrict__ part, int rows, double inv_count, float eps, float decay,
                      const unsigned short* __restrict__ y, long long M, int C, const float* __restrict__ beta, int relu,
                      unsigned short* __restrict__ a, int ld_a, float* __restrict__ mean, float* __restrict__ rstd,
                      float* __restrict__ mmean, float* __restrict__ mvar, int rows_per_chunk, const ChanMap map,
                      float* __restrict__ thr) {
  __shared__ double red[8][kBnGroup][2];
  __shared__ float s_mean[kBnGroup], s_rstd[kBnGroup], s_beta[kBnGroup];
  const int c0 = blockIdx.x * kBnGroup;
  const int cw = min(kBnGroup, C - c0);
  const int V = cw >> 3;
  const long long r_begin = (long long)blockIdx.y * rows_per_chunk;
  long long r_end = r_begin + rows_per_chunk;
  if (r_end > M) r_end = M;
  const int total = (int)(r_end - r_begin) * V;
  constexpr int kPre = 4;
  u32x4 pre[kPre];
#pragma unroll
  for (int u = 0; u < kPre; ++u) {
    const int i = threadIdx.x + u * kT;
    pre[u] = u32x4{0u, 0u, 0u, 0u};
    if (i < total) pre[u] = ld8(y + (r_begin + i / V) * C + c0 + ((i % V) << 3));
  }
  {
    const int cp = (threadIdx.x & 31) * 2, rl = threadIdx.x >> 5;
    double s1a = 0.0, s2a = 0.0, s1b = 0.0, s2b = 0.0;
    if (cp < cw) {
      const float* src = part + ((size_t)c0 + cp) * 2;
      int r = rl;
      for (; r + 8 * 15 < rows; r += 8 * 16) {
        float4 v[16];
#pragma unroll
        for (int u = 0; u < 16; ++u) v[u] = *reinterpret_cast<const float4*>(src + (size_t)(r + 8 * u) * C * 2);
#pragma unroll
        for (int u = 0; u < 16; ++u) { s1a += v[u].x; s2a += v[u].y; s1b += v[u].z; s2b += v[u].w; }
      }
      if (r + 8 < rows) {
        const float4 v0 = *reinterpret_cast<const float4*>(src + (size_t)r * C * 2);
        const float4 v1 = *reinterpret_cast<const float4*>(src + (size_t)(r + 8) * C * 2);
        s1a += v0.x; s2a += v0.y; s1b += v0.z; s2b += v0.w;
        s1a += v1.x; s2a += v1.y; s1b += v1.z; s2b += v1.w;
        r += 16;
      }
      for (; r < rows; r += 8) {
        const float4 v = *reinterpret_cast<const float4*>(src + (size_t)r * C * 2);
        s1a += v.x; s2a += v.y; s1b += v.z; s2b += v.w;
      }
    }
    red[rl][cp][0] = s1a; red[rl][cp][1] = s2a; red[rl][cp + 1][0] = s1b; red[rl][cp + 1][1] = s2b;
    __syncthreads();
    const int ch = threadIdx.x;
    if (ch < cw) {
      double s1 = red[0][ch][0], s2 = red[0][ch][1];
      for (int r = 1; r < 8; ++r) { s1 += red[r][ch][0]; s2 += red[r][ch][1]; }
      const double m = s1 * inv_count;
      double var = s2 * inv_count - m * m;
      if (var < 0.0) var = 0.0;
      const float fm = (float)m, fr = (float)(1.0 / sqrt(var + (double)eps));
      s_mean[ch] = fm; s_rstd[ch] = fr; s_beta[ch] = beta[c0 + ch];
      if (blockIdx.y == 0) {
        mean[c0 + ch] = fm; rstd[c0 + ch] = fr;
        if (thr) thr[c0 + ch] = relu ? fm - s_beta[ch] / fr : -__builtin_inff();
        if (decay < 0.f) {
          if (mmean) mmean[c0 + ch] = fm;
          if (mvar) mvar[c0 + ch] = (float)var;
        } else {
          if (mmean) mmean[c0 + ch] -= (1.0f - decay) * (mmean[c0 + ch] - fm);
          if (mvar) mvar[c0 + ch] -= (1.0f - decay) * (mvar[c0 + ch] - (float)var);
        }
      }
    }
    __syncthreads();
  }
  auto finish = [&](const int i, const u32x4 raw) {
    const long long m = r_begin + i / V;
    const int vc = (i % V) << 3;
    float f[8];
    unpack8(raw, f);
#pragma unroll
    for (int j = 0; j < 8; ++j) {
      const float v = (f[j] - s_mean[vc + j]) * s_rstd[vc + j] + s_beta[vc + j];
      f[j] = relu ? relu_f(v) : v;
    }
    st8(a + m * ld_a + c0 + vc + chan_off(map, c0 + vc), pack8(f));
  };
#pragma unroll
  for (int u = 0; u < kPre; ++u) {
    const int i = threadIdx.x + u * kT;
    if (i < total) finish(i, pre[u]);
  }
  for (int i = threadIdx.x + kPre * kT; i < total; i += kT)
    finish(i, ld8(y + (r_begin + i / V) * C + c0 + ((i % V) << 3)));
}

constexpr int kRowsMaxC = 2048;
__global__ void __launch_bounds__(kT)
bn_apply_rows_kernel(const float* __restrict__ part, int rows, double inv_count, float eps, float decay,
                     const unsigned short* __restrict__ y, long long M, int C, const float* __restrict__ beta, int relu,
                     unsigned short* __restrict__ a, int ld_a, float* __restrict__ mean, float* __restrict__ rstd,
                     float* __restrict__ mmean, float* __restrict__ mvar, const ChanMap map, float* __restrict__ thr, int xcd_rows) {
  extern __shared__ __attribute__((aligned(16))) float s_par[];
  const int C8 = C >> 3;
  const int rpi = kT / C8 > 0 ? kT / C8 : 1;
  const int vc = threadIdx.x % C8, rr = threadIdx.x / C8;
  const bool active = rr < rpi;
  const int c = vc << 3;
  long long step = (long long)gridDim.x * rpi, Mend = M;
  long long m = (long long)blockIdx.x * rpi + rr;
  if (xcd_rows && gridDim.x >= 8) {
    const int xcd = (int)blockIdx.x & 7, nx = ((int)gridDim.x - xcd + 7) >> 3;
    const long long perx = ((M + 7) / 8 + rpi - 1) / rpi * rpi;
    const long long lo = (long long)xcd * perx;
    step = (long long)nx * rpi; m = lo + (long long)((int)blockIdx.x >> 3) * rpi + rr; Mend = lo + perx < M ? lo + perx : M;
  }
  constexpr int kRowsAhead = 4;
  u32x4 pre[kRowsAhead];
#pragma unroll
  for (int i = 0; i < kRowsAhead; ++i) {
    const long long mi = m + i * step;
    pre[i] = (active && mi < Mend) ? ld8(y + mi * C + c) : u32x4{0u, 0u, 0u, 0u};
  }
  for (int chb = threadIdx.x; chb < C; chb += 2 * kT) {
   longlong2 w0[8], w1[8];
   const bool two = chb + kT < C;
   const float be0 = beta[chb], be1 = beta[two ? chb + kT : chb];
   if (rows == 8) {
     const longlong2* a0 = reinterpret_cast<const longlong2*>(part) + chb;
     const longlong2* a1 = reinterpret_cast<const longlong2*>(part) + (two ? chb + kT : chb);
#pragma unroll
     for (int r = 0; r < 8; ++r) { w0[r] = a0[(size_t)r * C]; w1[r] = a1[(size_t)r * C]; }
   }
   for (int half = 0; half < (two ? 2 : 1); ++half) {
    const int ch = chb + half * kT;
    const longlong2* src = reinterpret_cast<const longlong2*>(part) + ch;
    long long i1 = 0, i2 = 0;
    bool bad = false;
    int r = 0;
    if (rows == 8) {
#pragma unroll
      for (int q = 0; q < 8; ++q) {
        const longlong2 v = half ? w1[q] : w0[q];
        i1 += v.x; i2 += v.y;
        bad |= v.y < 0;
      }
      r = 8;
    }
    for (; r + 3 < rows; r += 4) {
      const longlong2 v0 = src[(size_t)(r + 0) * C], v1 = src[(size_t)(r + 1) * C], v2 = src[(size_t)(r + 2) * C], v3 = src[(size_t)(r + 3) * C];
      i1 += (v0.x + v1.x) + (v2.x + v3.x);
      i2 += (v0.y + v1.y) + (v2.y + v3.y);
      bad |= ((v0.y | v1.y) | (v2.y | v3.y)) < 0;
    }
    for (; r < rows; ++r) {
      const longlong2 v = src[(size_t)r * C];
      i1 += v.x; i2 += v.y;
      bad |= v.y < 0;
    }
    const double s1 = (double)i1 * (1.0 / 1048576.0), s2 = (double)i2 * (1.0 / 1048576.0);
    const double mu = s1 * inv_count;
    double var = s2 * inv_count - mu * mu;
    if (var < 0.0) var = 0.0;
    const bool poisoned = bad || i2 < 0;
    if (poisoned) var = (double)__builtin_nanf("");
    const float fm = poisoned ? __builtin_nanf("") : (float)mu, fr = poisoned ? __builtin_nanf("") : (float)(1.0 / sqrt(var + (double)eps)), be = half ? be1 : be0;
    s_par[ch] = fm; s_par[C + ch] = fr; s_par[2 * C + ch] = be;
    if (blockIdx.x == 0) {
      mean[ch] = fm; rstd[ch] = fr;
      if (thr) thr[ch] = relu ? fm - be / fr : -__builtin_inff();
      if (decay < 0.f) {
        if (mmean) mmean[ch] = fm;
        if (mvar) mvar[ch] = (float)var;
      } else {
        if (mmean) mmean[ch] -= (1.0f - decay) * (mmean[ch] - fm);
        if (mvar) mvar[ch] -= (1.0f - decay) * (mvar[ch] - (float)var);
      }
    }
   }
  }
  __syncthreads();
  if (!active) return;
  a += chan_off(map, c);
  float mu[8], rs[8], be[8];
#pragma unroll
  for (int j = 0; j < 8; ++j) { mu[j] = s_par[c + j]; rs[j] = s_par[C + c + j]; be[j] = s_par[2 * C + c + j]; }
  auto finish = [&](const long long mi, const u32x4 v) {
    float f[8];
    unpack8(v, f);
#pragma unroll
    for (int j = 0; j < 8; ++j) {
      const float t = (f[j] - mu[j]) * rs[j] + be[j];
      f[j] = relu ? relu_f(t) : t;
    }
    st8(a + mi * ld_a + c, pack8(f));
  };
  u32x4 cur = u32x4{0u, 0u, 0u, 0u};
  const long long mrest = m + kRowsAhead * step;
  if (mrest < Mend) cur = ld8(y + mrest * C + c);
#pragma unroll
  for (int i = 0; i < kRowsAhead; ++i) {
    const long long mi = m + i * step;
    if (mi < Mend) finish(mi, pre[i]);
  }
  for (m = mrest; m < Mend; m += step) {
    u32x4 nxt = u32x4{0u, 0u, 0u, 0u};
    if (m + step < Mend) nxt = ld8(y + (m + step) * C + c);
    finish(m, cur);
    cur = nxt;
  }
}

__global__ void __launch_bounds__(kT)
bn_bwd_rows_kernel(const float* __restrict__ part, int rows, double inv_M, const unsigned short* __restrict__ da, int ld_da,
                   const unsigned short* __restrict__ y, long long M, int C, const float* __restrict__ mean,
                   const float* __restrict__ rstd, const float* __restrict__ thr, float* __restrict__ dbeta,
                   unsigned short* __restrict__ dy, const ChanMap map) {
  extern __shared__ __attribute__((aligned(16))) float s_par[];
  const int C8 = C >> 3;
  const int rpi = kT / C8 > 0 ? kT / C8 : 1;
  const int vc = threadIdx.x % C8, rr = threadIdx.x / C8;
  const bool active = rr < rpi;
  const int c = vc << 3;
  const long long step = (long long)gridDim.x * rpi;
  long long m = (long long)blockIdx.x * rpi + rr;
  const unsigned short* dap = da + c + chan_off(map, c);
  u32x4 g0 = u32x4{0u, 0u, 0u, 0u}, y0 = u32x4{0u, 0u, 0u, 0u};
  if (active && m < M) { g0 = ld8(dap + m * ld_da); y0 = ld8(y + m * C + c); }
  for (int ch = threadIdx.x; ch < C; ch += kT) {
    const float* src = part + (size_t)ch * 2;
    double s1 = 0.0, s2 = 0.0;
    int r = 0;
    for (; r + 3 < rows; r += 4) {
      const float2 v0 = *reinterpret_cast<const float2*>(src + (size_t)(r + 0) * C * 2);
      const float2 v1 = *reinterpret_cast<const float2*>(src + (size_t)(r + 1) * C * 2);
      const float2 v2 = *reinterpret_cast<const float2*>(src + (size_t)(r + 2) * C * 2);
      const float2 v3 = *reinterpret_cast<const float2*>(src + (size_t)(r + 3) * C * 2);
      s1 += ((double)v0.x + (double)v1.x) + ((double)v2.x + (double)v3.x);
      s2 += ((double)v0.y + (double)v1.y) + ((double)v2.y + (double)v3.y);
    }
    for (; r < rows; ++r) {
      const float2 v = *reinterpret_cast<const float2*>(src + (size_t)r * C * 2);
      s1 += v.x; s2 += v.y;
    }
    const float mu = mean[ch], rs = rstd[ch];
    const double sgx = (double)rs * (s2 - (double)mu * s1);
    s_par[ch] = mu; s_par[C + ch] = rs; s_par[2 * C + ch] = thr[ch];
    s_par[3 * C + ch] = (float)(s1 * inv_M); s_par[4 * C + ch] = (float)(sgx * inv_M);
    if (blockIdx.x == 0 && dbeta) dbeta[ch] += (float)s1;
  }
  __syncthreads();
  if (!active) return;
  float mu[8], rs[8], th[8], m1[8], m2[8];
#pragma unroll
  for (int j = 0; j < 8; ++j) {
    mu[j] = s_par[c + j]; rs[j] = s_par[C + c + j]; th[j] = s_par[2 * C + c + j]; m1[j] = s_par[3 * C + c + j]; m2[j] = s_par[4 * C + c + j];
  }
  u32x4 gc = g0, yc = y0;
  for (; m < M; m += step) {
    u32x4 gn = u32x4{0u, 0u, 0u, 0u}, yn = u32x4{0u, 0u, 0u, 0u};
    if (m + step < M) { gn = ld8(dap + (m + step) * ld_da); yn = ld8(y + (m + step) * C + c); }
    float g[8], yy[8], o[8];
    unpack8(gc, g);
    unpack8(yc, yy);
#pragma unroll
    for (int j = 0; j < 8; ++j) {
      const float xh = (yy[j] - mu[j]) * rs[j];
      const float gj = yy[j] > th[j] ? g[j] : 0.f;
      o[j] = rs[j] * (gj - m1[j] - xh * m2[j]);
    }
    st8(dy + m * C + c, pack8(o));
    gc = gn; yc = yn;
  }
}

inline int env_int(const char* name, int dflt) { const char* e = getenv(name); return e ? atoi(e) : dflt; }
inline void bn_fused_grid(long long M, int C, int rows, int& groups, int& chunks, int& rpc) {
  groups = (C + kBnGroup - 1) / kBnGroup;
  static const int blocks_few = env_int("MBX_BN_FUSED_BLOCKS", 1024), blocks_many = env_int("MBX_BN_FUSED_BLOCKS_MANY", 256);
  long long want = (rows > 16 ? blocks_many : blocks_few) / groups;
  if (want < 1) want = 1;
  long long maxc = (M + 255) / 256;
  if (want > maxc) want = maxc;
  rpc = (int)((M + want - 1) / want);
  chunks = (int)((M + rpc - 1) / rpc);
}

#ifndef MBX_OB_SLOTS
#define MBX_OB_SLOTS 8
#endif
#ifndef MBX_OB_SLEEP
#define MBX_OB_SLEEP 8
#endif
constexpr int kObT = 512;
constexpr int kObSlots = MBX_OB_SLOTS;
constexpr int kObMaxNV = 20;
#ifndef MBX_OB_SUB
#define MBX_OB_SUB 16
#endif
#ifndef MBX_OB_REL
#define MBX_OB_REL 32
#endif
constexpr int kObSub = MBX_OB_SUB, kObRel = MBX_OB_REL, kObLine = 32;
constexpr int kObCtlWords = kObLine * (2 + kObSub + kObRel);

struct ObGeom { int C8, rpi, G, rpb, nv; };
inline ObGeom ob_geom(long long M, int C, int ncu) {
  ObGeom g;
  g.C8 = C / 8;
  g.rpi = g.C8 <= kObT ? kObT / g.C8 : 0;
  if (g.rpi == 0) { g.G = g.rpb = 0; g.nv = 1 << 30; return g; }
  long long G = (M + g.rpi - 1) / g.rpi;
  if (G > ncu) G = ncu;
  g.rpb = (int)((M + G - 1) / G);
  g.G = (int)((M + g.rpb - 1) / g.rpb);
  g.nv = (g.rpb + g.rpi - 1) / g.rpi;
  return g;
}

__device__ __forceinline__ unsigned ld_agent(const unsigned* p) {
  return __hip_atomic_load(p, __ATOMIC_RELAXED, __HIP_MEMORY_SCOPE_AGENT);
}
__device__ __forceinline__ float ld_agent(const float* p) {
  return __hip_atomic_load(p, __ATOMIC_RELAXED, __HIP_MEMORY_SCOPE_AGENT);
}

__device__ __forceinline__ __amdgpu_buffer_rsrc_t ob_rsrc(const void* p, unsigned bytes) {
  return __builtin_amdgcn_make_buffer_rsrc(const_cast<void*>(p), (short)0, (int)bytes, 0x00020000);
}
__device__ __forceinline__ u32x4 ob_load16(__amdgpu_buffer_rsrc_t r, unsigned byte_off) {
  return __builtin_amdgcn_raw_buffer_load_b128(r, (int)byte_off, 0, 0);
}
__device__ __forceinline__ void ob_store16(__amdgpu_buffer_rsrc_t r, unsigned byte_off, u32x4 v) {
  __builtin_amdgcn_raw_buffer_store_b128(v, r, (int)byte_off, 0, 0);
}

template <int NV, bool RELU>
__global__ void __launch_bounds__(kObT)
bn_bwd_onepass_kernel(const unsigned short* __restrict__ da, int ld_da, const unsigned short* __restrict__ y,
                      long long M, int C, const float* __restrict__ mean, const float* __restrict__ rstd,
                      const float* __restrict__ beta, float* __restrict__ dbeta, unsigned short* __restrict__ dy,
                      float* __restrict__ ws, int rpi, int rpb, float inv_M, unsigned spin_limit, int fault,
                      float* __restrict__ step_poison, const ChanMap map, int map_max) {
  extern __shared__ __attribute__((aligned(16))) float sred[];
  __shared__ int s_timeout;
  const int C8 = C >> 3;
  const int vc = threadIdx.x % C8, rr = threadIdx.x / C8;
  const bool active = rr < rpi;
  const int c = vc << 3;
  const long long r0 = (long long)((fault & 2) ? xcd_logical((int)blockIdx.x, (int)gridDim.x) : (int)blockIdx.x) * rpb;
  long long nr = (r0 + rpb > M ? M : r0 + rpb) - r0;
  const int nrows = nr > 0 ? (int)nr : 0;
  const __amdgpu_buffer_rsrc_t gr = ob_rsrc(da + r0 * ld_da, nrows ? (unsigned)(((nrows - 1) * ld_da + C + map_max) * 2) : 0u);
  const int cg = c + chan_off(map, c);
  const __amdgpu_buffer_rsrc_t yr = ob_rsrc(y + r0 * C, (unsigned)(nrows * C * 2));
  const __amdgpu_buffer_rsrc_t dr = ob_rsrc(dy + r0 * C, (unsigned)(nrows * C * 2));
  constexpr unsigned kPast = 0x80000000u;
  u32x4 vg[NV], vy[NV];
#pragma unroll
  for (int i = 0; i < NV; ++i) {
    const int lr = rr + i * rpi;
    const bool ok = active && lr < nrows;
    vg[i] = ob_load16(gr, ok ? (unsigned)((lr * ld_da + cg) * 2) : kPast);
// ... 1200 lines not shown
  return MBX_OK;
}

extern "C" int mbx_pack_input(const float* img, int64_t pixels, void* out, mbx_stream_t stream) {
  if (!img || !out || pixels <= 0 || !al16(out)) return MBX_ERR_INVALID_ARG;
  MBX_ENTER();
  hipLaunchKernelGGL(pack_input_kernel, dim3(grid_for(pixels)), dim3(kT), 0, mbx_s(stream), img, (long long)pixels, (us)out);
  MBX_LAUNCH_CHECK();
  return MBX_OK;
}

extern "C" int mbx_head_gather(const float* h, int ld_h, int N, int cells, int k, int P, int off, float* locs,
                               float* logits, mbx_stream_t stream) {
  if (!h || !locs || !logits || N <= 0 || cells <= 0 || k <= 0 || ld_h < 5 * k || off < 0 || off + cells * k > P)
    return MBX_ERR_INVALID_ARG;
  MBX_ENTER();
  hipLaunchKernelGGL(head_gather_kernel, dim3(grid_for((long long)N * cells * k)), dim3(kT), 0, mbx_s(stream), h, ld_h, N,
                     cells, k, P, off, locs, logits);
  MBX_LAUNCH_CHECK();
  return MBX_OK;
}

extern "C" int mbx_head_scatter(const float* d_locs, const float* d_logits, int N, int cells, int k, int P, int off, void* g,
                                int ld_g, mbx_stream_t stream) {
  if (!d_locs || !d_logits || !g || N <= 0 || cells <= 0 || k <= 0 || ld_g < 5 * k || off < 0 || off + cells * k > P)
    return MBX_ERR_INVALID_ARG;
  MBX_ENTER();
  hipLaunchKernelGGL(head_scatter_kernel, dim3(grid_for((long long)N * cells * ld_g)), dim3(kT), 0, mbx_s(stream), d_locs,
                     d_logits, N, cells, k, P, off, (us)g, ld_g);
  MBX_LAUNCH_CHECK();
  return MBX_OK;
}

static int fill_head_table(const mbx_head* heads, int n_heads, int N, int P, bool scatter, HeadTable& t) {
  if (!heads || n_heads <= 0 || n_heads > kMaxHeads || N <= 0 || P <= 0) return MBX_ERR_INVALID_ARG;
  long long acc = 0;
  t.n = n_heads;
  for (int j = 0; j < n_heads; ++j) {
    const mbx_head& H = heads[j];
    if (H.cells <= 0 || H.k <= 0 || H.off < 0 || H.off + H.cells * H.k > P) return MBX_ERR_INVALID_ARG;
    if (scatter ? (!H.g || H.ld_g < 5 * H.k) : (!H.h || H.ld_h < 5 * H.k)) return MBX_ERR_INVALID_ARG;
    t.h[j] = H.h; t.g[j] = reinterpret_cast<unsigned short*>(H.g);
    t.ld_h[j] = H.ld_h; t.ld_g[j] = H.ld_g; t.cells[j] = H.cells; t.k[j] = H.k; t.off[j] = H.off;
    t.start[j] = (int)acc;
    acc += (long long)N * H.cells * (scatter ? H.ld_g : H.k);
    if (acc >= (1LL << 31)) return MBX_ERR_UNSUPPORTED;
  }
  for (int j = n_heads; j <= kMaxHeads; ++j) t.start[j] = (int)acc;
  return MBX_OK;
}

extern "C" int mbx_head_gather_all(const mbx_head* heads, int n_heads, int N, int P, float* locs, float* logits,
                                   mbx_stream_t stream) {
  if (!locs || !logits) return MBX_ERR_INVALID_ARG;
  HeadTable t;
  const int st = fill_head_table(heads, n_heads, N, P, false, t);
  if (st != MBX_OK) return st;
  MBX_ENTER();
  hipLaunchKernelGGL(head_gather_all_kernel, dim3(grid_for(t.start[t.n])), dim3(kT), 0, mbx_s(stream), t, P, locs, logits);
  MBX_LAUNCH_CHECK();
  return MBX_OK;
}

extern "C" int mbx_head_scatter_all(const float* d_locs, const float* d_logits, const mbx_head* heads, int n_heads, int N,
                                    int P, mbx_stream_t stream) {
  if (!d_locs || !d_logits) return MBX_ERR_INVALID_ARG;
  HeadTable t;
  const int st = fill_head_table(heads, n_heads, N, P, true, t);
  if (st != MBX_OK) return st;
  MBX_ENTER();
  hipLaunchKernelGGL(head_scatter_all_kernel, dim3(grid_for(t.start[t.n])), dim3(kT), 0, mbx_s(stream), t, P, d_locs, d_logits);
  MBX_LAUNCH_CHECK();
  return MBX_OK;
}

extern "C" int mbx_step_begin(float* grads, int64_t n_grads, float* bn_ws, int64_t n_ws, int64_t ctl_index,
                              uint64_t* timeouts_total, float* zero_scalar, mbx_stream_t stream) {
  if (!grads || n_grads <= 0 || n_grads % 4 || n_ws < 0 || n_ws % 4 || (n_ws && !bn_ws) || !al16(grads) || (bn_ws && !al16(bn_ws)) ||
      (timeouts_total && (ctl_index < 0 || ctl_index >= n_grads)))
    return MBX_ERR_INVALID_ARG;
  MBX_ENTER();
  hipLaunchKernelGGL(step_begin_kernel, dim3(grid_for((n_grads + n_ws) / 4)), dim3(kT), 0, mbx_s(stream), grads,
                     (long long)n_grads, bn_ws, (long long)n_ws, (long long)ctl_index,
                     reinterpret_cast<unsigned long long*>(timeouts_total), zero_scalar);
  MBX_LAUNCH_CHECK();
  return MBX_OK;
}

extern "C" int mbx_filter_prepare(const void* w_bf16, void* w_dgrad, const mbx_filter_entry* table, int n_entries,
                                  int total_blocks, mbx_stream_t stream) {
  if (!w_bf16 || !w_dgrad || !table || n_entries <= 0 || total_blocks <= 0) return MBX_ERR_INVALID_ARG;
  MBX_ENTER();
  hipLaunchKernelGGL(filter_prepare_kernel, dim3(total_blocks), dim3(kT), 0, mbx_s(stream), (cus)w_bf16, (us)w_dgrad, table,
                     n_entries);
  MBX_LAUNCH_CHECK();
  return MBX_OK;
}

extern "C" int mbx_rmsprop_ema_step(float* w, const float* g, float* ms, float* mom, float* ema, void* w_bf16, int64_t n,
                                    float lr, float decay, float momentum, float eps, float wd, float ema_decay,
                                    int trainable, float* reg_loss, const float* skip_ctl, mbx_stream_t stream) {
  if (!w || n <= 0 || (trainable && (!g || !ms))) return MBX_ERR_INVALID_ARG;
  if (trainable && momentum != 0.f && !mom) return MBX_ERR_INVALID_ARG;
  MBX_ENTER();
  hipLaunchKernelGGL(rmsprop_ema_kernel, dim3(grid_for(n)), dim3(kT), 0, mbx_s(stream), w, g, ms, momentum != 0.f ? mom : nullptr,
                     ema, (us)w_bf16, (long long)n, lr, decay, momentum, eps, wd, ema_decay, trainable, reg_loss, skip_ctl);
  MBX_LAUNCH_CHECK();
  return MBX_OK;
}

extern "C" int mbx_bn_moving_update(float* moving_mean, float* moving_var, const float* batch_mean, const float* batch_var,
                                    int64_t n, float decay, const float* skip_ctl, uint64_t* skipped_steps,
                                    float* ema_mean, float* ema_var, float ema_decay, mbx_stream_t stream) {
  if (!moving_mean || !moving_var || !batch_mean || !batch_var || n <= 0 || decay < 0.f) return MBX_ERR_INVALID_ARG;
  MBX_ENTER();
  hipLaunchKernelGGL(bn_moving_update_kernel, dim3(grid_for(n)), dim3(kT), 0, mbx_s(stream), moving_mean, moving_var,
                     batch_mean, batch_var, (long long)n, decay, skip_ctl, reinterpret_cast<unsigned long long*>(skipped_steps),
                     ema_mean, ema_var, ema_decay);
  MBX_LAUNCH_CHECK();
  return MBX_OK;
}

extern "C" int mbx_ema_update(float* ema, const float* value, int64_t n, float ema_decay, const float* skip_ctl,
                              mbx_stream_t stream) {
  if (!ema || !value || n <= 0) return MBX_ERR_INVALID_ARG;
  MBX_ENTER();
  hipLaunchKernelGGL(ema_update_kernel, dim3(grid_for(n)), dim3(kT), 0, mbx_s(stream), ema, value, (long long)n, ema_decay, skip_ctl);
  MBX_LAUNCH_CHECK();
  return MBX_OK;
}

extern "C" int mbx_bn_apply_fused_mapped(const void* stats_partial, int rows, int64_t count, float eps, float decay,
                                         const void* y, int64_t M, int C, const float* beta, int relu, void* a, int ld_a,
                                         const mbx_chan_map* a_map, float* mean, float* rstd, float* mmean, float* mvar,
                                         float* relu_thr, mbx_stream_t stream) {
  if (!stats_partial || !y || !a || !beta || !mean || !rstd || rows <= 0 || M <= 0 || C <= 0 || C % 8 || ld_a % 8 ||
      count <= 0 || !al16(y) || !al16(a) || !al16(stats_partial))
    return MBX_ERR_INVALID_ARG;
  if (rows > 16 || C > kRowsMaxC) return MBX_ERR_UNSUPPORTED;
  ChanMap cm;
  if (to_chan_map(a_map, C, cm) != MBX_OK) return MBX_ERR_INVALID_ARG;
  MBX_ENTER();
  static const int rows_blocks = env_int("MBX_BN_ROWS_BLOCKS", 1024);
  const int C8 = C / 8, rpi = kT / C8 > 0 ? kT / C8 : 1;
  long long g = (M + rpi - 1) / rpi;
  if (g > rows_blocks) g = rows_blocks;
  hipLaunchKernelGGL(bn_apply_rows_kernel, dim3((unsigned)g), dim3(kT), (size_t)3 * C * sizeof(float), mbx_s(stream),
                     reinterpret_cast<const float*>(stats_partial), rows, 1.0 / (double)count, eps, decay, (cus)y, (long long)M, C,
                     beta, relu, (us)a, ld_a, mean, rstd, mmean, mvar, cm, relu_thr, xcd_rows_on());
  MBX_LAUNCH_CHECK();
  return MBX_OK;
}

extern "C" int mbx_bn_apply_fused(const float* stats_partial, int rows, int64_t count, float eps, float decay, const void* y,
                                  int64_t M, int C, const float* beta, int relu, void* a, int ld_a, float* mean,
                                  float* rstd, float* mmean, float* mvar, mbx_stream_t stream) {
  if (!stats_partial || !y || !a || !beta || !mean || !rstd || rows <= 0 || M <= 0 || C <= 0 || C % 8 || ld_a % 8 ||
      count <= 0 || !al16(y) || !al16(a))
    return MBX_ERR_INVALID_ARG;
  static const int fused_rows = env_int("MBX_BN_FUSED_ROWS", 16);
  static const long long fused_elems = env_int("MBX_BN_FUSED_KELEMS", 6200) * 1000LL;
  if (rows > 16 && (rows > fused_rows || M * C > fused_elems)) {
    int st = mbx_bn_finalize(stats_partial, rows, C, count, eps, decay, mean, rstd, mmean, mvar, stream);
    if (st != MBX_OK) return st;
    return mbx_bn_apply(y, M, C, mean, rstd, beta, relu, a, ld_a, stream);
  }
  MBX_ENTER();
  int groups, chunks, rpc;
  bn_fused_grid(M, C, rows, groups, chunks, rpc);
  hipLaunchKernelGGL(bn_apply_fused_kernel, dim3(groups, chunks), dim3(kT), 0, mbx_s(stream), stats_partial, rows,
                     1.0 / (double)count, eps, decay, (cus)y, (long long)M, C, beta, relu, (us)a, ld_a, mean, rstd, mmean,
                     mvar, rpc, ChanMap{}, nullptr);
  MBX_LAUNCH_CHECK();
  return MBX_OK;
}
```

multibox_amd/engine.py:

```python
from __future__ import annotations

import ctypes as C
import math
import os
import re

import numpy as np
import torch

from . import _lib, ops
from .ops import View

BN_EPS = 0.001
STATS_ROWS = int(os.environ.get("MBX_STATS_ROWS", "8"))
WEIGHT_DECAY = 0.00004


def _same_pad(n, k, s):
    out = -(-n // s)
    total = max((out - 1) * s + k - n, 0)
    return out, total // 2


def _valid(n, k, s):
    return (n - k) // s + 1, 0


class ParamSpec:

    def __init__(self, scope, K, R, S, Cin, bn, bias):
        self.scope, self.K, self.R, self.S, self.Cin, self.bn, self.bias = scope, K, R, S, Cin, bn, bias


class ConvOp:

    def __init__(self, net, members, x: View, out: View, R, S, stride, pad_t, pad_l, kind, relu=True, skip=None,
                 rscale=0.0, trainable=True, need_dx=True, head=None):
        self.net, self.members, self.x, self.out = net, members, x, out
        self.R, self.S, self.stride, self.pad_t, self.pad_l = R, S, stride, pad_t, pad_l
        self.kind, self.relu, self.skip, self.rscale = kind, relu, skip, rscale
        self.trainable, self.need_dx, self.head = trainable, need_dx, head
        self.K = sum(m.K for m in members)
        self.Cin = x.C
        self.M = out.M
        self.name = members[0].scope if len(members) == 1 else "+".join(m.scope for m in members)

    w_off = b_off = beta_off = dw_off = -1


class BnGroup:

    def __init__(self, members):
        self.members = list(members)
        self.K = sum(m.K for m in members)
        self.koff, k = [], 0
        for m in members:
            self.koff.append(k)
            k += m.K
        self.y = self.dy = None
        self.fwd_desc, self.dgrad_desc = {}, {}
        self.pair_fwd = self.pair_bwd = False
        self.rows = [0] * len(members)
        self.stats_off = [0] * len(members)

    def chan_map(self, views):
        rel = [v.ch_off - ko for v, ko in zip(views, self.koff)]
        base = min(rel)
        m = _lib.ChanMap()
        m.n = len(self.members)
        for i, (ko, r) in enumerate(zip(self.koff, rel)):
            m.c_begin[i], m.offset[i] = ko, r - base
        return base, m


class Net:
    def __init__(self, batch, input_size=299, k=5, mode="train", fine_tune=False, device="cuda", seed=2,
                 bn_decay=0.9997, repeats=(10, 20, 9), bn_max_workgroups=0, wgrad_overlap_cus=None):
        assert mode in ("train", "infer")
        self.repeats = tuple(repeats)
        self.B, self.S, self.k, self.mode, self.fine_tune, self.dev = batch, input_size, k, mode, fine_tune, device
        self.bn_decay = bn_decay
        self.tune_registry = []
        self.deterministic = bool(int(os.environ.get("MBX_DETERMINISTIC", "0")))
        self.no_onepass = self.deterministic or bool(int(os.environ.get("MBX_NO_BN_ONEPASS", "0")))
        self.atomic_stats = mode == "train" and not self.deterministic and os.environ.get("MBX_ATOMIC_STATS", "1") != "0"
        self.bw_stats = self.atomic_stats and os.environ.get("MBX_BW_STATS", "0") == "1"
        self.fuse_apply = self.atomic_stats and os.environ.get("MBX_FUSE_APPLY", "0") == "1"
        self.fused_apply_launches = 0
        self.fuse_bwd = (mode == "train" and not self.deterministic and not self.bw_stats and torch.device(device).type == "cuda"
                         and os.environ.get("MBX_FUSE_BWD", "0") == "1")
        self.fused_bwd_launches = self.fused_bwd_layers = 0
        self.relu_bits = mode == "train" and os.environ.get("MBX_RELU_BITS", "1") != "0"
        self.autotune = torch.device(device).type == "cuda" and bool(int(os.environ.get("MBX_AUTOTUNE", "1")))
        self.bn_max_wg = int(os.environ.get("MBX_BN_MAX_WG", "0")) or (bn_max_workgroups or 0)
        self.wgrad_overlap_cus = ops.wgrad_overlap_cus() if wgrad_overlap_cus is None else int(wgrad_overlap_cus)
        self.n_cus = torch.cuda.get_device_properties(device).multi_processor_count if torch.device(device).type == "cuda" else 256
        self.chain_cap = 0
        if self.wgrad_overlap_cus > 0 and mode == "train":
            self.wgrad_overlap_cus = min(self.wgrad_overlap_cus, self.n_cus // 2)
            self.chain_cap = min(self.bn_max_wg or self.n_cus, self.n_cus - self.wgrad_overlap_cus)
        self.cu_cap = 0
        self.defer_moving = False
        self.i5_counters = torch.zeros(8192, dtype=torch.int32, device=device)
        self._i5_used = 0
        self._probe_skip_apply = self._probe_skip_bn_bwd = False
        self.convs, self.fwd, self.bwd = [], [], []
        self._bn_group_requests, self.bn_groups = [], []
        self.grad_alias = {}
        self.written = set()
        self.heads = []
        self._bufs = []
        self._build()
        self._finalize(seed)

    def alloc(self, H, W, Cc, dtype=torch.bfloat16, zero=False):
        v = View.alloc(self.B, H, W, Cc, dtype=dtype, device=self.dev, zero=zero)
        self._bufs.append(v.buf)
        return v

    def grad_of(self, v: View) -> View:
        key = id(v.buf)
        if key not in self.grad_alias:
            g = torch.zeros_like(v.buf)
            self._bufs.append(g)
            self.grad_alias[key] = g
        return View(self.grad_alias[key], v.N, v.H, v.W, v.C, v.ld, v.ch_off, v.elem_size)

    def share_grad(self, v: View, like: View):
        self.grad_alias[id(v.buf)] = self.grad_of(like).buf

    def _training_bn(self, is_head):
        if self.mode == "infer":
            return False
        return is_head if self.fine_tune else True

    def conv(self, members, x, out, kh, kw, stride=1, padding="SAME", kind=None, relu=True, skip=None, rscale=0.0,
             is_head=False, need_dx=True, head=None):
        fh = _same_pad if padding == "SAME" else _valid
        Ho, pt = fh(x.H, kh, stride)
        Wo, pl = fh(x.W, kw, stride)
        assert (Ho, Wo) == (out.H, out.W), (members, Ho, Wo, out.H, out.W)
        if kind is None:
            kind = "bn" if self._training_bn(is_head) else "frozen"
        trainable = self.mode == "train" and (is_head or not self.fine_tune)
        specs = [ParamSpec(s, K, kh, kw, x.C, bn=kind in ("bn", "frozen"), bias=kind == "residual") for s, K in members]
        op = ConvOp(self, specs, x, out, kh, kw, stride, pt, pl, kind, relu, skip, rscale, trainable,
                    need_dx and trainable, head)
        op.is_head = is_head
        assert op.K == out.C or kind == "head", (op.name, op.K, out.C)
        self.convs.append(op)
        self.fwd.append(op)
        return op

    def group_bn(self, *members):
        if os.environ.get("MBX_BN_GROUPS", "1") != "0" and len(members) >= 2:
            self._bn_group_requests.append(members)

    def _build(self):
        B, S, k = self.B, self.S, self.k
        P = "InceptionResnetV2/"
        self.images = self.alloc(S, S, 8)
        s1, _ = _valid(S, 3, 2)
        a1 = self.alloc(s1, s1, 32)
        self.conv([(P + "Conv2d_1a_3x3", 32)], self.images, a1, 3, 3, 2, "VALID", need_dx=False)
        s2 = s1 - 2
        a2 = self.alloc(s2, s2, 32)
        self.conv([(P + "Conv2d_2a_3x3", 32)], a1, a2, 3, 3, 1, "VALID")
        a3 = self.alloc(s2, s2, 64)
        self.conv([(P + "Conv2d_2b_3x3", 64)], a2, a3, 3, 3, 1, "SAME")
        s3, _ = _valid(s2, 3, 2)
        p3 = self.alloc(s3, s3, 64)
        self.pool("max", a3, p3, 3, 2, scope=P + "MaxPool_3a_3x3")
        a4 = self.alloc(s3, s3, 80)
        self.conv([(P + "Conv2d_3b_1x1", 80)], p3, a4, 1, 1, 1, "VALID")
        s4 = s3 - 2
        a5 = self.alloc(s4, s4, 192)
        self.conv([(P + "Conv2d_4a_3x3", 192)], a4, a5, 3, 3, 1, "VALID")
        s5, _ = _valid(s4, 3, 2)
        t5 = self.alloc(s5, s5, 192)
        self.pool("max", a5, t5, 3, 2, scope=P + "MaxPool_5a_3x3")

        Q = P + "Mixed_5b/"
        z = self.alloc(s5, s5, 528)
        self.conv([(Q + "Branch_1/Conv2d_0a_1x1", 48), (Q + "Branch_2/Conv2d_0a_1x1", 64), (Q + "Branch_0/Conv2d_1x1", 96)],
                  t5, z.slice(0, 208), 1, 1)
        ga = self.conv([(Q + "Branch_1/Conv2d_0b_5x5", 64)], z.slice(0, 48), z.slice(208, 64), 5, 5)
        gb = self.conv([(Q + "Branch_2/Conv2d_0b_3x3", 96)], z.slice(48, 64), z.slice(432, 96), 3, 3)
        self.group_bn(ga, gb)
        self.conv([(Q + "Branch_2/Conv2d_0c_3x3", 96)], z.slice(432, 96), z.slice(272, 96), 3, 3)
        p5 = self.alloc(s5, s5, 192)
        self.pool("avg", t5, p5, 3, 1, pad=1, scope=Q + "Branch_3/AvgPool_0a_3x3")
        self.conv([(Q + "Branch_3/Conv2d_0b_1x1", 64)], p5, z.slice(368, 64), 1, 1)
        net = z.slice(112, 320)
        self.endpoints = {"MaxPool_5a_3x3": t5, "Mixed_5b": net}

        trunk0 = net
        zg = None
        for i in range(1, self.repeats[0] + 1):
            Q = P + "Repeat/block35_%d/" % i
            z = self.alloc(s5, s5, 240)
            if zg is None:
                zg = z
            else:
                self.share_grad(z, zg)
            self.conv([(Q + "Branch_1/Conv2d_0a_1x1", 32), (Q + "Branch_2/Conv2d_0a_1x1", 32), (Q + "Branch_0/Conv2d_1x1", 32)],
                      net, z.slice(0, 96), 1, 1)
            ga = self.conv([(Q + "Branch_1/Conv2d_0b_3x3", 32)], z.slice(0, 32), z.slice(96, 32), 3, 3)
            gb = self.conv([(Q + "Branch_2/Conv2d_0b_3x3", 48)], z.slice(32, 32), z.slice(192, 48), 3, 3)
            self.group_bn(ga, gb)
            self.conv([(Q + "Branch_2/Conv2d_0c_3x3", 64)], z.slice(192, 48), z.slice(128, 64), 3, 3)
            out = self.alloc(s5, s5, 320)
            self.residual(Q + "Conv2d_1x1", z.slice(64, 128), net, out, 0.17, True, trunk0)
            net = out

        Q = P + "Mixed_6a/"
        s6, _ = _valid(s5, 3, 2)
        o6 = self.alloc(s6, s6, 1088)
        self.conv([(Q + "Branch_0/Conv2d_1a_3x3", 384)], net, o6.slice(0, 384), 3, 3, 2, "VALID")
        t6a = self.alloc(s5, s5, 256)
        self.conv([(Q + "Branch_1/Conv2d_0a_1x1", 256)], net, t6a, 1, 1)
        t6b = self.alloc(s5, s5, 256)
        self.conv([(Q + "Branch_1/Conv2d_0b_3x3", 256)], t6a, t6b, 3, 3)
        self.conv([(Q + "Branch_1/Conv2d_1a_3x3", 384)], t6b, o6.slice(384, 384), 3, 3, 2, "VALID")
        self.pool("max", net, o6.slice(768, 320), 3, 2, scope=Q + "Branch_2/MaxPool_1a_3x3")
        self.endpoints["block35_10"] = net
        net = o6
        self.endpoints["Mixed_6a"] = net

        trunk0, zg = net, None
        for i in range(1, self.repeats[1] + 1):
            Q = P + "Repeat_1/block17_%d/" % i
            z = self.alloc(s6, s6, 672)
            if zg is None:
                zg = z
            else:
                self.share_grad(z, zg)
            self.conv([(Q + "Branch_1/Conv2d_0a_1x1", 128), (Q + "Branch_0/Conv2d_1x1", 192)], net, z.slice(0, 320), 1, 1)
            self.conv([(Q + "Branch_1/Conv2d_0b_1x7", 160)], z.slice(0, 128), z.slice(512, 160), 1, 7)
            self.conv([(Q + "Branch_1/Conv2d_0c_7x1", 192)], z.slice(512, 160), z.slice(320, 192), 7, 1)
            out = self.alloc(s6, s6, 1088)
            self.residual(Q + "Conv2d_1x1", z.slice(128, 384), net, out, 0.10, True, trunk0)
            net = out

        Q = P + "Mixed_7a/"
# ... 410 lines not shown

        def readers(buf, lo, hi):
            r = [o for o in self.fwd if o.x.buf is buf and o.x.ch_off < hi and o.x.ch_off + o.x.C > lo]
            r += [o for o in self.fwd if isinstance(o, ConvOp) and o.skip is not None and o.skip.buf is buf and
                  o.skip.ch_off < hi and o.skip.ch_off + o.skip.C > lo]
            return r

        def segments(X):
            segs, c, end = [], X.x.ch_off, X.x.ch_off + X.x.C
            while c < end:
                m = member_at(X.x.buf, c)
                if m is None:
                    return None
                n = min(end, m.out.ch_off + m.K) - c
                segs.append((c - X.x.ch_off, m, c - m.out.ch_off, n))
                c += n
            if len(segs) > 4 or any(sg[0] % 8 for sg in segs):
                return None
            return segs

        eligible = set(id(u) for u in units)
        conv_ok = {}
        while True:
            conv_ok = {}
            for X in self.fwd:
                if not isinstance(X, ConvOp) or not X.need_dx or not X.trainable or X.stride != 1:
                    continue
                if X.x.img_stride != X.x.H * X.x.W * X.x.ld or X.Cin % 8 or (only is not None and not only.search(X.name)):
                    continue
                if not pairs_ok and X.kind == "bn" and X.group is not None and len(X.group.members) == 2:
                    continue
                segs = segments(X)
                if segs is None or any(id(unit_of[id(sg[1])]) not in eligible for sg in segs):
                    continue
                if len(readers(X.x.buf, X.x.ch_off, X.x.ch_off + X.x.C)) != 1:
                    continue
                dd = ops.ConvDesc()
                dd.R, dd.S, dd.stride, dd.epilogue, dd.C_in, dd.C_out = X.R, X.S, 1, ops.EPI_STORE, X.K, X.Cin
                dd.N, dd.H_in, dd.W_in, dd.H_out, dd.W_out = X.x.N, X.out.H, X.out.W, X.x.H, X.x.W
                if ops.direct3_applies(dd):
                    continue
                if ops.fused_tail_rounds(dd, self.n_cus) > int(os.environ.get("MBX_FUSE_BWD_MAX_ROUNDS", "1")):
                    continue
                conv_ok[id(X)] = segs
            drop = set()
            for u in units:
                if id(u) not in eligible:
                    continue
                for m in u:
                    rd = readers(m.out.buf, m.out.ch_off, m.out.ch_off + m.K)
                    covered = sorted((max(o.x.ch_off, m.out.ch_off), min(o.x.ch_off + o.x.C, m.out.ch_off + m.K)) for o in rd)
                    tiled = bool(covered) and covered[0][0] == m.out.ch_off and covered[-1][1] == m.out.ch_off + m.K and \
                        all(a[1] == b[0] for a, b in zip(covered, covered[1:]))
                    if not tiled or any(id(o) not in conv_ok for o in rd):
                        drop.add(id(u))
            if not drop:
                break
            eligible -= drop
        for u in units:
            if id(u) in eligible:
                for m in u:
                    m.fb_unit = u
        for X in self.fwd:
            if isinstance(X, ConvOp) and id(X) in conv_ok:
                X.fb_segments = conv_ok[id(X)]

    def _fb_table(self, X):
        t = ops.BnBwdFused()
        t.barrier = self.bn_ws.data_ptr() + 4 * X.fb_bar_off
        t.n = len(X.fb_segments)
        t.step_poison = self.step_ctl.data_ptr()
        for i, (c_rel, m, c_in, n) in enumerate(X.fb_segments):
            lead = m.fb_unit[0]
            K_all = sum(q.K for q in m.fb_unit)
            ko = m.y_view.ch_off
            assert m.y_view.ld == K_all and m.dy_view.ld == K_all and lead.fb_acc_off >= 0
            t.c_begin[i] = c_rel
            t.y[i], t.ld_y[i] = m.y_view.buf.data_ptr() + 2 * (ko + c_in), K_all
            t.dy[i], t.ld_dy[i] = m.dy_view.buf.data_ptr() + 2 * (ko + c_in), K_all
            t.mean[i] = self.bn_mean.data_ptr() + 4 * (m.beta_off + c_in)
            t.rstd[i] = self.bn_rstd.data_ptr() + 4 * (m.beta_off + c_in)
            t.beta[i] = self.Bt.data_ptr() + 4 * (m.beta_off + c_in)
            t.dbeta[i] = self.Btg.data_ptr() + 4 * (m.beta_off + c_in)
            t.acc[i], t.acc_ld[i] = self.bn_ws.data_ptr() + 4 * (lead.fb_acc_off + ko + c_in), K_all
            t.relu[i] = int(m.relu)
        self._keep_fb = getattr(self, "_keep_fb", []) + [t]
        return t

    def _bw_table(self, X):
        t = _lib.BnBwdStats()
        t.n, t.rows_mod = len(X.bw_segments), STATS_ROWS
        for i, (c_rel, m, c_in, n) in enumerate(X.bw_segments):
            lead = m.bw_unit[0]
            K_all = sum(q.K for q in m.bw_unit)
            ko = m.y_view.ch_off
            t.c_begin[i] = c_rel
            t.y[i], t.ld_y[i] = m.y_view.buf.data_ptr() + 2 * (ko + c_in), K_all
            t.relu_thr[i] = self.bn_thr.data_ptr() + 4 * (m.beta_off + c_in)
            t.stats[i], t.stats_ld[i] = self.bn_ws.data_ptr() + 4 * (lead.bw_rows_off + 2 * (ko + c_in)), K_all
        self._keep_bw = getattr(self, "_keep_bw", []) + [t]
        return t

    def _w(self, op):
        return self.Wb[op.w_off:]

    def _desc(self, op, y: View, **kw):
        return ops.make_desc(op.x, self._w(op), op.K, op.R, op.S, op.stride, op.pad_t, op.pad_l, y, **kw)

    def _sl(self, t, off, n):
        return t[off:off + n]

    def _tune(self, op, d, what):
        key = (what, op.x.N, op.x.H, op.x.W, op.x.C, op.K, op.R, op.S, op.stride, op.pad_t, op.pad_l, d.C_out, d.C_in,
               d.epilogue, bool(d.stats_partial), d.accumulate, bool(d.skip) or (bool(d.relu_bits) and d.epilogue == ops.EPI_STORE), d.relu)
        if d.relu_bits and d.epilogue == ops.EPI_RESIDUAL:
            key = key + ("bits",)
        self.tune_registry.append((repr(key), d, what))
        if self.autotune:
            ops.autotune(d, key)
            over = ops._TUNED.get(repr(key) + "#norule") if os.environ.get("MBX_NO_RULE_EXCEPTIONS") != "1" else None
            if over is not None:
                keep = d.tile_config
                d.tile_config = int(over)
                if _lib.lib().mbx_conv_supported(C.byref(d)) != 0:
                    d.tile_config, over = keep, None
            if os.environ.get("MBX_NO_I5") == "1" and d.tile_config > ops.I5_FLAG:
                d.tile_config = ops._TUNED.get(repr(key) + "#i3", 0)
            if d.tile_config > ops.I5_FLAG and os.environ.get("MBX_I5_STATIC") != "1":
                n = ops.I7_COUNTERS if d.tile_config == ops.I7_TILE_CONFIG else 1
                assert self._i5_used + n <= self.i5_counters.numel()
                d.work_counter = self.i5_counters.data_ptr() + 4 * self._i5_used
                self._i5_used += n
            if os.environ.get("MBX_NO_2STAGE") == "1":
                d.tile_config = {9: 7, 10: 2, 11: 5, 12: 2, 13: 8, 14: 1}.get(d.tile_config, d.tile_config)
            if over is not None:
                pass
            elif ops.direct3_applies(d):
                d.tile_config, d.work_counter = ops.DIRECT3_TILE_CONFIG, None
                _lib.check(_lib.lib().mbx_conv_supported(C.byref(d)), "direct 3x3 " + op.name)
            elif ops.directw_applies(d) and not (what == "fwd" and d.stats_partial and getattr(op, "group", None) is not None
                                                 and len(op.group.members) == 2 and os.environ.get("MBX_CONV_PAIR", "1") != "0"):
                d.tile_config, d.work_counter = ops.DIRECTW_TILE_CONFIG, None
                _lib.check(_lib.lib().mbx_conv_supported(C.byref(d)), "direct 3x3 (whole-width) " + op.name)
            elif ops.pwres_applies(d):
                d.tile_config, d.work_counter = ops.PWRES_TILE_CONFIG, None
                _lib.check(_lib.lib().mbx_conv_supported(C.byref(d)), "pixel-resident 1x1 " + op.name)
            elif ops.resident_applies(d):
                d.tile_config, d.work_counter = ops.RESIDENT_TILE_CONFIG, None
                _lib.check(_lib.lib().mbx_conv_supported(C.byref(d)), "resident image " + op.name)
        return d

    def _build_forward_launches(self):
        L = []
        l = _lib.lib()
        st = lambda: torch.cuda.current_stream().cuda_stream
        for op in self.fwd:
            if isinstance(op, PoolOp):
                if not getattr(op, "fused_fwd", False):
                    L.append(op.forward)
                continue
            if op.kind == "bn" and op.group is not None:
                g = op.group
                i = g.members.index(op)
                use16 = self.atomic_stats
                if use16:
                    d = self._tune(op, self._desc(op, op.y_view, stats=self.stats16[op.stats16_off:], stats_rows_mod=STATS_ROWS,
                                                  stats_ld=g.K), "fwd")
                else:
                    d = self._tune(op, self._desc(op, op.y_view, stats=self.stats_scratch[op.stats_off:]), "fwd")
                g.rows[i] = ops.conv_stats_rows(d)
                assert use16 or g.rows[i] * op.K * 2 <= (g.stats_off[i + 1] - g.stats_off[i] if i + 1 < len(g.members) else 1 << 62)
                g.fwd_desc[i] = d
                if i + 1 < len(g.members):
                    L.append(lambda d=d, op=op, g=g: None if g.pair_fwd else _lib.check(l.mbx_conv(C.byref(d), st()), op.name))
                    continue
                if len(g.members) == 2 and torch.device(self.dev).type == "cuda" and os.environ.get("MBX_CONV_PAIR", "1") != "0":
                    g.pair_fwd = l.mbx_conv_pair(C.byref(g.fwd_desc[0]), C.byref(d), st()) == 0
                lead, n = g.members[0], len(g.members)
                parts = (C.c_void_p * n)(*[self.stats_scratch.data_ptr() + 4 * o for o in g.stats_off])
                rows_a, cs_a = (C.c_int32 * n)(*g.rows), (C.c_int32 * n)(*[m.K for m in g.members])
                base, amap = g.chan_map([m.out for m in g.members])
                a_ptr = op.out.buf.data_ptr() + 2 * base
                mean, rstd = self._sl(self.bn_mean, lead.beta_off, g.K), self._sl(self.bn_rstd, lead.beta_off, g.K)
                mm, mv = self._sl(self.MM, lead.beta_off, g.K), self._sl(self.MV, lead.beta_off, g.K)
                var, beta = self._sl(self.bn_var, lead.beta_off, g.K), self._sl(self.Bt, lead.beta_off, g.K)
                thr = self._sl(self.bn_thr, lead.beta_off, g.K)
                s16 = self.stats16[lead.stats16_base:]

                def run(d=d, op=op, g=g, parts=parts, rows_a=rows_a, cs_a=cs_a, amap=amap, a_ptr=a_ptr, mean=mean, rstd=rstd,
                        mm=mm, mv=mv, var=var, beta=beta, n=n, use16=use16, thr=thr, s16=s16):
                    s = st()
                    if g.pair_fwd:
                        _lib.check(l.mbx_conv_pair(C.byref(g.fwd_desc[0]), C.byref(d), s), "pair " + op.name)
                    else:
                        _lib.check(l.mbx_conv(C.byref(d), s), op.name)
                    decay = self.bn_decay
                    if self.defer_moving:
                        mm, mv, decay = None, var, -1.0
                    if use16:
                        _lib.check(l.mbx_bn_apply_fused_mapped(s16.data_ptr(), STATS_ROWS, op.M, BN_EPS, decay, g.y.data_ptr(), op.M,
                                                               g.K, beta.data_ptr(), int(op.relu), a_ptr, op.out.ld, C.byref(amap),
                                                               mean.data_ptr(), rstd.data_ptr(), ops._p(mm), ops._p(mv),
                                                               thr.data_ptr(), s), "bn_apply_fused_mapped")
                        return
                    _lib.check(l.mbx_bn_finalize_parts(parts, rows_a, cs_a, n, op.M, BN_EPS, decay, mean.data_ptr(), rstd.data_ptr(),
                                                       ops._p(mm), ops._p(mv), s), "bn_finalize_parts")
                    _lib.check(l.mbx_bn_apply_mapped(g.y.data_ptr(), op.M, g.K, mean.data_ptr(), rstd.data_ptr(), beta.data_ptr(),
                                                     int(op.relu), a_ptr, op.out.ld, C.byref(amap), s), "bn_apply_mapped")
                L.append(run)
            elif op.kind == "bn":
                yv = op.y_view
                fpool = getattr(op, "fused_pool", None)
                use16 = self.atomic_stats and fpool is None
                if use16:
                    d = self._tune(op, self._desc(op, yv, stats=self.stats16[op.stats16_off:], stats_rows_mod=STATS_ROWS), "fwd")
                else:
                    d = self._tune(op, self._desc(op, yv, stats=self.stats_scratch), "fwd")
                S_ = ops.splitk_slices(d, self.n_cus) if torch.device(self.dev).type == "cuda" else 0
                if S_:
                    d.tile_config = ops.SPLITK_FLAG + S_
                    need = int(l.mbx_conv_splitk_workspace_bytes(C.byref(d)))
                    ws = torch.empty(need // 4, dtype=torch.float32, device=self.dev)
                    self._splitk_ws = getattr(self, "_splitk_ws", []) + [ws]
                    d.splitk_ws, d.splitk_ws_bytes = ws.data_ptr(), ws.numel() * 4
                    _lib.check(l.mbx_conv_supported(C.byref(d)), "split-K " + op.name)
                rows = ops.conv_stats_rows(d)
                mean, rstd = self._sl(self.bn_mean, op.beta_off, op.K), self._sl(self.bn_rstd, op.beta_off, op.K)
                mm, mv = self._sl(self.MM, op.beta_off, op.K), self._sl(self.MV, op.beta_off, op.K)
                beta = self._sl(self.Bt, op.beta_off, op.K)
                out = op.out

                var = self._sl(self.bn_var, op.beta_off, op.K)
                thr = self._sl(self.bn_thr, op.beta_off, op.K)
                s16 = self.stats16[op.stats16_off:]

                if fpool is not None:
                    fpool.fused_fwd = True
                fd = ba = None
                if use16 and self.fuse_apply and not S_ and torch.device(self.dev).type == "cuda" and out.img_stride == out.H * out.W * out.ld \
                        and (not os.environ.get("MBX_FUSE_APPLY_ONLY") or re.search(os.environ["MBX_FUSE_APPLY_ONLY"], op.name)):
                    ba = ops.BnApplyDesc()
                    ba.barrier = self._fwd_barrier_base + ops.GRID_BARRIER_BYTES * self._fwd_barriers_used
                    ba.a, ba.ld_a, ba.beta, ba.mean, ba.rstd = out.ptr, out.ld, beta.data_ptr(), mean.data_ptr(), rstd.data_ptr()
                    ba.relu_thr, ba.relu, ba.eps, ba.step_poison = thr.data_ptr(), int(op.relu), BN_EPS, self.step_ctl.data_ptr()
                    fd = ops.ConvDesc.from_buffer_copy(d)
                    fd.bn_apply = C.addressof(ba)
                    fd.work_counter = None
                    if l.mbx_conv_supported(C.byref(fd)) == 0:
                        assert self._fwd_barriers_used < self._n_fwd_barriers
                        self._fwd_barriers_used += 1
                        self.fused_apply_launches += 1
                        self._keep_ba = getattr(self, "_keep_ba", []) + [ba]
                    else:
                        fd = ba = None

                def run(d=d, rows=rows, op=op, mean=mean, rstd=rstd, mm=mm, mv=mv, beta=beta, out=out, var=var, fpool=fpool,
                        use16=use16, thr=thr, s16=s16, fd=fd, ba=ba):
                    s = st()
                    decay = self.bn_decay
                    if self.defer_moving:
                        mm, mv, decay = None, var, -1.0
                    if fd is not None and not self.no_onepass:
                        ba.moving_mean, ba.moving_var, ba.decay = ops._p(mm), ops._p(mv), decay
                        fd.max_workgroups = self.cu_cap or self.bn_max_wg
                        _lib.check(l.mbx_conv(C.byref(fd), s), op.name + " + bn apply")
                        return
                    _lib.check(l.mbx_conv(C.byref(d), s), op.name)
                    if use16:
                        _lib.check(l.mbx_bn_apply_fused_mapped(s16.data_ptr(), STATS_ROWS, op.M, BN_EPS, decay, op.y_view.ptr, op.M,
                                                               op.K, beta.data_ptr(), int(op.relu), out.ptr, out.ld, None,
                                                               mean.data_ptr(), rstd.data_ptr(), ops._p(mm), ops._p(mv),
                                                               thr.data_ptr(), s), "bn_apply_fused_mapped")
                        return
                    if fpool is not None:
                        po = fpool.out
                        _lib.check(l.mbx_bn_finalize(self.stats_scratch.data_ptr(), rows, op.K, op.M, BN_EPS, decay,
                                                     mean.data_ptr(), rstd.data_ptr(), ops._p(mm), ops._p(mv), s), "bn_finalize")
                        _lib.check(l.mbx_bn_apply_maxpool(op.y_view.ptr, out.N, out.H, out.W, op.K, mean.data_ptr(), rstd.data_ptr(),
                                                          beta.data_ptr(), int(op.relu), po.ptr, po.img_stride, po.ld, po.H, po.W,
                                                          fpool.argmax.data_ptr(), s), "bn_apply_maxpool")
                        return
                    if self._probe_skip_apply and ("/block" in op.name or "/Block8" in op.name):
                        _lib.check(l.mbx_bn_finalize(self.stats_scratch.data_ptr(), rows, op.K, op.M, BN_EPS, decay,
                                                     mean.data_ptr(), rstd.data_ptr(), ops._p(mm), ops._p(mv), s), "fin")
                        return
                    _lib.check(l.mbx_bn_apply_fused(self.stats_scratch.data_ptr(), rows, op.M, BN_EPS, decay,
                                                    op.y_view.ptr, op.M, op.K, beta.data_ptr(), int(op.relu), out.ptr, out.ld,
                                                    mean.data_ptr(), rstd.data_ptr(), ops._p(mm), ops._p(mv), s), "bn_apply_fused")
                L.append(run)
            elif op.kind == "frozen":
                d = self._tune(op, self._desc(op, op.out, epilogue=ops.EPI_AFFINE, relu=op.relu,
                                              scale=self._sl(self.bn_scale, op.beta_off, op.K),
                                              shift=self._sl(self.bn_shift, op.beta_off, op.K)), "fwd")
                L.append(lambda d=d, op=op: _lib.check(l.mbx_conv(C.byref(d), st()), op.name))
            elif op.kind == "residual":
                d = self._tune(op, self._desc(op, op.out, epilogue=ops.EPI_RESIDUAL, relu=op.relu,
                                              shift=self._sl(self.W, op.b_off, op.K), skip=op.skip, rscale=op.rscale,
                                              relu_bits=getattr(op, "relu_bits", None)), "fwd")
                L.append(lambda d=d, op=op: _lib.check(l.mbx_conv(C.byref(d), st()), op.name))
            elif op.kind == "head":
                d = self._desc(op, op.out, epilogue=ops.EPI_STORE_F32)
                L.append(lambda d=d, op=op: _lib.check(l.mbx_conv(C.byref(d), st()), op.name))
                if op is self.heads[-1]:
                    L.append(lambda: _lib.check(l.mbx_head_gather_all(self.head_table, len(self.heads), self.B, self.P,
                                                                      self.locs.data_ptr(), self.logits.data_ptr(), st()), "head_gather_all"))
        return L

    def _gview(self, v: View) -> View:
        return self.grad_of(v)

    def _claim(self, g: View):
        key = (id(g.buf), g.ch_off, g.C)
        if key in self.written:
            return 1, None
        self.written.add(key)
        src = self.pending_acc.pop(key, None)
        return (1, src) if src is not None else (0, None)

    def _make_head_table(self):
        arr = (_lib.Head * len(self.heads))()
        for j, op in enumerate(self.heads):
            cells, kk, off = op.head
            op.head_grad = None
            if self.mode == "train":
                op.head_grad = View(torch.zeros((op.M, self.head_ld), dtype=torch.bfloat16, device=self.dev),
                                    op.out.N, op.out.H, op.out.W, self.head_ld)
                self._bufs.append(op.head_grad.buf)
            arr[j].h, arr[j].ld_h = op.out.buf.data_ptr(), self.head_ld
            arr[j].g, arr[j].ld_g = (op.head_grad.buf.data_ptr() if op.head_grad is not None else None), self.head_ld
            arr[j].cells, arr[j].k, arr[j].off = cells, kk, off
        self.head_table = arr

    def _build_backward(self):
        self._make_head_table()
        if self.mode != "train":
            self.fwd_launches = self._build_forward_launches()
            self.bwd_launches = []
            self.bwd_jobs = []
            return
        l = _lib.lib()
        st = lambda: torch.cuda.current_stream().cuda_stream
        entries, d_off, blocks = [], 0, 0
        for op in self.convs:
            if op.need_dx:
                kpad = (op.K + 7) // 8 * 8
                e = _lib.FilterEntry(op.w_off, d_off, op.K, op.R, op.S, op.Cin, kpad, blocks)
                op.dgrad_off, op.kpad = d_off, kpad
                n = op.Cin * op.R * op.S * kpad
                d_off += (n + 7) // 8 * 8
                blocks += op.R * op.S * ((op.Cin + 31) // 32) * ((kpad + 63) // 64)
                entries.append(e)
        self.Wd = torch.zeros(max(d_off, 8), dtype=torch.bfloat16, device=self.dev)
        arr = (_lib.FilterEntry * len(entries))(*entries)
        raw = np.frombuffer(C.string_at(C.addressof(arr), C.sizeof(arr)), dtype=np.uint8).copy()
        self.filter_table = torch.from_numpy(raw).to(self.dev)
        self.filter_blocks, self.filter_entries = blocks, len(entries)

        mask_of = {}
        fused_mask = set()
        for r in self.convs:
            if r.kind == "residual" and r.relu and r.trainable:
                for c in self.fwd:
                    if isinstance(c, ConvOp) and c.x.buf is r.out.buf:
                        if c.need_dx and c.x.ch_off == r.out.ch_off and c.x.C == r.out.C:
                            mask_of[id(c)] = r
                            fused_mask.add(id(r))
                        break
                    if isinstance(c, PoolOp) and c.x.buf is r.out.buf:
                        break
        self.pending_acc = {}
        L = []
        self.bwd_ops = []
        self.bwd_jobs = []
        for op in reversed(self.fwd):
            if isinstance(op, PoolOp):
                if op.needs_backward():
                    prod = self._pool_producer(op)
                    if prod is not None:
                        prod.fused_pool = op
                        continue
                    gx = self._gview(op.x)
                    acc, src = self._claim(gx)
                    assert src is None, "a pooling layer cannot be the first writer of a residual block's input gradient"
                    L.append(op.make_backward(self._gview(op.out), gx, acc))
                    self.bwd_ops.append(op)
                    self.bwd_jobs.append(None)
                continue
            if not op.trainable:
                continue
            K, M = op.K, op.M
            dw = self._sl(self.Wg, op.w_off, K * op.R * op.S * op.Cin)
            if op.kind == "head":
                cells, kk, off = op.head
                g = op.head_grad
                dyv, scale, db = g, 1.0, None
                pre = None
                if op is self.heads[-1]:
                    pre = lambda s: _lib.check(l.mbx_head_scatter_all(self.d_locs.data_ptr(), self.d_logits.data_ptr(), self.head_table,
                                                                      len(self.heads), self.B, self.P, s), "head_scatter_all")
            elif op.kind == "residual":
                gout = self._gview(op.out)
                gs = self._gview(op.skip)
                self.pending_acc[(id(gs.buf), gs.ch_off, gs.C)] = gout
                zb = id(self.grad_of(op.x).buf)
                self.written = {k for k in self.written if k[0] != zb}
                dyv, scale, db = gout, op.rscale, self._sl(self.Wg, op.b_off, K)
                if op.relu and id(op) not in fused_mask:
                    pre = lambda s, gout=gout, op=op: _lib.check(
                        l.mbx_relu_mask(gout.ptr, gout.ld, op.out.ptr, op.out.ld, op.M, op.K, s), "relu_mask")
                else:
                    pre = None
            else:
                dyv = op.dy_view
                scale, db = 1.0, None
                g = op.group
                if g is not None and op is not g.members[-1]:
                    pre = None
                else:
                    lead = op if g is None else g.members[0]
                    Kb = K if g is None else g.K
                    y_ptr, dy_ptr = (op.y_view.ptr, op.dy_view.ptr) if g is None else (g.y.data_ptr(), g.dy.data_ptr())
                    fpool = getattr(op, "fused_pool", None)
                    if fpool is not None:
                        da = da_ptr = dmap = None
                    elif g is None:
                        da, da_ptr, dmap = self._gview(op.out), self._gview(op.out).ptr, None
                    else:
                        gviews = [self._gview(m.out) for m in g.members]
                        assert all(v.buf is gviews[0].buf and v.ld == gviews[0].ld for v in gviews)
                        base, cm = g.chan_map(gviews)
                        da, da_ptr, dmap = gviews[0], gviews[0].buf.data_ptr() + 2 * base, C.byref(cm)
                        self._keep = getattr(self, "_keep", []) + [cm]
                    mean, rstd = self._sl(self.bn_mean, lead.beta_off, Kb), self._sl(self.bn_rstd, lead.beta_off, Kb)
                    dbeta = self._sl(self.Btg, lead.beta_off, Kb)
                    rows = l.mbx_bn_bwd_rows(M, Kb)
                    beta = self._sl(self.Bt, lead.beta_off, Kb)
                    ws_off = lead.bn_ws_off

                    def pre_onepass(s, op=op, da=da, da_ptr=da_ptr, dmap=dmap, mean=mean, rstd=rstd, beta=beta, dbeta=dbeta, Kb=Kb, M=M,
                                    y_ptr=y_ptr, dy_ptr=dy_ptr, ws_off=ws_off):
                        _lib.check(l.mbx_bn_bwd_onepass_mapped(da_ptr, da.ld, int(op.relu), y_ptr, M, Kb, mean.data_ptr(),
                                                               rstd.data_ptr(), beta.data_ptr(), dbeta.data_ptr(),
                                                               dy_ptr, self.bn_ws.data_ptr() + 4 * ws_off,
                                                               self.cu_cap or self.bn_max_wg, self.step_ctl.data_ptr(), dmap, s),
                                   "bn_bwd_onepass")

                    def pre(s, op=op, da=da, da_ptr=da_ptr, dmap=dmap, mean=mean, rstd=rstd, beta=beta, dbeta=dbeta, rows=rows, Kb=Kb,
                            M=M, y_ptr=y_ptr, dy_ptr=dy_ptr):
                        _lib.check(l.mbx_bn_bwd_reduce_mapped(da_ptr, da.ld, None, 0, int(op.relu), y_ptr, M, Kb,
                                                              mean.data_ptr(), rstd.data_ptr(), beta.data_ptr(),
                                                              self.bwd_scratch.data_ptr(), dmap, s), "bn_bwd_reduce")
                        _lib.check(l.mbx_bn_bwd_finalize(self.bwd_scratch.data_ptr(), rows, Kb, M, dbeta.data_ptr(),
                                                         self.m12.data_ptr(), s), "bn_bwd_finalize")
                        _lib.check(l.mbx_bn_bwd_apply_mapped(da_ptr, da.ld, None, 0, int(op.relu), y_ptr, M, Kb,
                                                             mean.data_ptr(), rstd.data_ptr(), beta.data_ptr(), self.m12.data_ptr(),
                                                             dy_ptr, dmap, s), "bn_bwd_apply")
                    if op.bw_unit is not None:
                        thr = self._sl(self.bn_thr, lead.beta_off, Kb)
                        rows_off = lead.bw_rows_off

                        def pre(s, da=da, da_ptr=da_ptr, dmap=dmap, mean=mean, rstd=rstd, thr=thr, dbeta=dbeta, Kb=Kb, M=M,
                                y_ptr=y_ptr, dy_ptr=dy_ptr, rows_off=rows_off):
                            _lib.check(l.mbx_bn_bwd_apply_rows(self.bn_ws.data_ptr() + 4 * rows_off, STATS_ROWS, da_ptr, da.ld, y_ptr, M, Kb,
                                                               mean.data_ptr(), rstd.data_ptr(), thr.data_ptr(), dbeta.data_ptr(),
                                                               dy_ptr, dmap, s), "bn_bwd_apply_rows")
                    if fpool is not None:
                        gy = self._gview(fpool.out)
                        rows = l.mbx_bn_bwd_rows_pooled(fpool.x.N, fpool.x.H, fpool.x.W, Kb)
                        assert 0 < rows * Kb * 2 <= self.bwd_scratch.numel()

                        def pre(s, op=op, gy=gy, fpool=fpool, mean=mean, rstd=rstd, beta=beta, dbeta=dbeta, rows=rows, Kb=Kb, M=M,
                                y_ptr=y_ptr, dy_ptr=dy_ptr):
                            geo = (gy.ptr, gy.img_stride, gy.ld, fpool.argmax.data_ptr(), fpool.x.N, fpool.x.H, fpool.x.W, fpool.out.H,
                                   fpool.out.W, int(op.relu), y_ptr, Kb, mean.data_ptr(), rstd.data_ptr(), beta.data_ptr())
                            _lib.check(l.mbx_bn_bwd_reduce_pooled(*geo, self.bwd_scratch.data_ptr(), s), "bn_bwd_reduce_pooled")
                            _lib.check(l.mbx_bn_bwd_finalize(self.bwd_scratch.data_ptr(), rows, Kb, M, dbeta.data_ptr(),
                                                             self.m12.data_ptr(), s), "bn_bwd_finalize")
                            _lib.check(l.mbx_bn_bwd_apply_pooled(*geo, self.m12.data_ptr(), dy_ptr, s), "bn_bwd_apply_pooled")
                if pre is not None and op.bw_unit is None and (op.bn_ws_off if g is None else g.members[0].bn_ws_off) >= 0:
                    def pre(s, one=pre_onepass, three=pre):
                        (three if self.no_onepass else one)(s)
                    if os.environ.get("MBX_PROBE_BN_APPLY_ONLY") == "1":
                        def pre(s, op=op, da=da, da_ptr=da_ptr, dmap=dmap, mean=mean, rstd=rstd, beta=beta, Kb=Kb, M=M, y_ptr=y_ptr,
                                dy_ptr=dy_ptr):
                            _lib.check(l.mbx_bn_bwd_apply_mapped(da_ptr, da.ld, None, 0, int(op.relu), y_ptr, M, Kb,
                                                                 mean.data_ptr(), rstd.data_ptr(), beta.data_ptr(), self.m12.data_ptr(),
                                                                 dy_ptr, dmap, s), "bn_bwd_apply")
            if op.kind == "bn" and op.fb_unit is not None and pre is not None:
                def pre(s, split=pre):
                    if self.no_onepass:
                        split(s)
                self.fused_bwd_layers += 1
            ddesc = fdesc = None
            if op.need_dx:
                gx = self._gview(op.x)
                acc, acc_src = self._claim(gx)
                dyin = View(dyv.buf, dyv.N, dyv.H, dyv.W, op.kpad, dyv.ld, dyv.ch_off, 2)
                mr = mask_of.get(id(op))
                ddesc = ops.make_desc(dyin, self.Wd[op.dgrad_off:], op.Cin, op.R, op.S, op.stride,
                                      op.R - 1 - op.pad_t, op.S - 1 - op.pad_l, gx, transposed=1, accumulate=acc,
                                      rscale=(scale if scale != 1.0 else 0.0), skip=(mr.out if mr is not None else None),
                                      acc_src=acc_src)
                if mr is not None and self.relu_bits and op.Cin % 8 == 0:
                    bits = torch.zeros((op.x.N * op.x.H * op.x.W, (op.Cin + 31) // 32 * 4), dtype=torch.uint8, device=self.dev)
                    alt = ops.make_desc(dyin, self.Wd[op.dgrad_off:], op.Cin, op.R, op.S, op.stride,
                                        op.R - 1 - op.pad_t, op.S - 1 - op.pad_l, gx, transposed=1, accumulate=acc,
                                        rscale=(scale if scale != 1.0 else 0.0), acc_src=acc_src, relu_bits=bits)
                    if torch.device(self.dev).type != "cuda" or l.mbx_conv_supported(C.byref(alt)) == 0:
                        ddesc, mr.relu_bits = alt, bits
                self._tune(op, ddesc, "dgrad")
                if op.fb_segments is not None:
                    assert acc == 0 and acc_src is None and mr is None, op.name
                    fdesc = ops.ConvDesc.from_buffer_copy(ddesc)
                    fdesc.bn_bwd = C.addressof(self._fb_table(op))
                    fdesc.work_counter = None
                    if not (ops.I5_FLAG < fdesc.tile_config <= ops.I5_FLAG + 7 or fdesc.tile_config in (ops.DIRECTW_TILE_CONFIG, ops.RESIDENT_TILE_CONFIG)):
                        fdesc.tile_config = ops.i5_tile_for(op.x.M, op.Cin, self.n_cus)
                    if l.mbx_conv_supported(C.byref(fdesc)) != 0:
                        fdesc.tile_config = ops.i5_tile_for(op.x.M, op.Cin, self.n_cus)
                    _lib.check(l.mbx_conv_supported(C.byref(fdesc)), "data gradient + BN backward " + op.name)
                    self.fused_bwd_launches += 1
                if op.bw_segments is not None:
                    assert acc == 0 and acc_src is None and mr is None, op.name
                    ddesc.bn_bwd_stats = C.addressof(self._bw_table(op))
                    if l.mbx_conv_supported(C.byref(ddesc)) != 0:
                        for alt in (ops.I5_TILE_CONFIGS[2], ops.I5_TILE_CONFIGS[1], 0):
                            ddesc.tile_config = alt
                            if alt == 0:
                                ddesc.work_counter = None
                            if l.mbx_conv_supported(C.byref(ddesc)) == 0:
                                break
                        _lib.check(l.mbx_conv_supported(C.byref(ddesc)), "statistics epilogue " + op.name)

            job = ops.WgradJob()
            job.desc = ops.make_desc(op.x, None, K, op.R, op.S, op.stride, op.pad_t, op.pad_l,
                                     View(dyv.buf, op.out.N, op.out.H, op.out.W, 8, dyv.ld, dyv.ch_off, 2))
            job.desc.C_out = K
            job.dy, job.dy_img_stride, job.ld_dy = dyv.ptr, dyv.img_stride, dyv.ld
            job.scale = float(scale)
            job.dw, job.db = dw.data_ptr(), (None if db is None else db.data_ptr())

            grp = getattr(op, "group", None) if op.kind == "bn" else None
            if grp is not None and ddesc is not None:
                grp.dgrad_desc[grp.members.index(op)] = ddesc

            op.fdesc = fdesc

            def run(op=op, pre=pre, ddesc=ddesc, grp=grp, fdesc=fdesc):
                s = st()
                if pre is not None and not (op.kind == "bn" and self._probe_skip_bn_bwd):
                    pre(s)
                if fdesc is not None and not self.no_onepass:
                    fdesc.max_workgroups = self.cu_cap or self.bn_max_wg
                    _lib.check(l.mbx_conv(C.byref(fdesc), s), "dgrad + bn backward " + op.name)
                    return
                if ddesc is not None:
                    if grp is not None and grp.pair_bwd:
                        if op is grp.members[-1]:
                            _lib.check(l.mbx_conv_pair(C.byref(ddesc), C.byref(grp.dgrad_desc[0]), s), "dgrad pair " + op.name)
                        return
                    ddesc.max_workgroups = self.cu_cap
                    _lib.check(l.mbx_conv(C.byref(ddesc), s), "dgrad " + op.name)
            L.append(run)
            self.bwd_ops.append(op)
            self.bwd_jobs.append(job)
        if torch.device(self.dev).type == "cuda" and os.environ.get("MBX_CONV_PAIR", "1") != "0":
            for grp in self.bn_groups:
                if len(grp.members) == 2 and len(grp.dgrad_desc) == 2 and not any(getattr(m, "fdesc", None) is not None for m in grp.members):
                    grp.pair_bwd = l.mbx_conv_pair(C.byref(grp.dgrad_desc[1]), C.byref(grp.dgrad_desc[0]), st()) == 0
        assert not self.pending_acc, "a residual block's input gradient was never written"
        self.bwd_launches = L
        self.fwd_launches = self._build_forward_launches()
        self._default_groups = None

    def _pool_producer(self, pool):
        if os.environ.get("MBX_POOL_FUSE", "1") == "0" or pool.kind != "max" or pool.k != 3 or pool.stride != 2 or pool.pad != 0 \
                or pool.argmax is None:
            return None
        readers = [o for o in self.fwd if o is not pool and o.x.buf is pool.x.buf]
        if readers:
            return None
        for c in self.convs:
            if c.out.buf is pool.x.buf and c.out.ch_off == pool.x.ch_off and c.out.C == pool.x.C and c.out.ld == pool.x.ld == pool.x.C:
                ok = c.kind == "bn" and c.trainable and c.group is None and (c.bn_ws_off < 0 or self.deterministic)
                return c if ok else None
        return None

    def make_wgrad_groups(self, job_lists):
        return [ops.WgradGroup(jobs, deterministic=self.deterministic, device=self.dev) for jobs in job_lists if jobs]

    def prepare_filters(self):
        if self.mode == "train" and self.filter_entries:
            _lib.check(_lib.lib().mbx_filter_prepare(self.Wb.data_ptr(), self.Wd.data_ptr(), self.filter_table.data_ptr(),
                                                     self.filter_entries, self.filter_blocks,
                                                     torch.cuda.current_stream().cuda_stream), "filter_prepare")

    def apply_moving_update(self, skip_ctl=None, skipped_steps=None, ema_mean=None, ema_var=None, ema_decay=0.0):
        lo = self.head_bt_start if self.fine_tune else 0
        n = self.nBt - lo
        if n > 0 and self.mode == "train":
            _lib.check(_lib.lib().mbx_bn_moving_update(self.MM.data_ptr() + 4 * lo, self.MV.data_ptr() + 4 * lo,
                                                       self.bn_mean.data_ptr() + 4 * lo, self.bn_var.data_ptr() + 4 * lo, n,
                                                       self.bn_decay, ops._p(skip_ctl), ops._p(skipped_steps),
                                                       None if ema_mean is None else ema_mean.data_ptr() + 4 * lo,
                                                       None if ema_var is None else ema_var.data_ptr() + 4 * lo, float(ema_decay),
                                                       torch.cuda.current_stream().cuda_stream), "bn_moving_update")

    def fold_bn(self):
        _lib.check(_lib.lib().mbx_bn_fold(self.MM.data_ptr(), self.MV.data_ptr(), self.Bt.data_ptr(), BN_EPS, self.nBt,
                                          self.bn_scale.data_ptr(), self.bn_shift.data_ptr(),
                                          torch.cuda.current_stream().cuda_stream), "bn_fold")

    def set_input(self, images_f32):
        assert images_f32.shape == (self.B, self.S, self.S, 3) and images_f32.dtype == torch.float32
        _lib.check(_lib.lib().mbx_pack_input(images_f32.contiguous().data_ptr(), self.B * self.S * self.S,
                                             self.images.buf.data_ptr(), torch.cuda.current_stream().cuda_stream), "pack_input")

    def forward(self):
        if self._i5_used or self.atomic_stats:
            self._fwd_clear.zero_()
        for f in self.fwd_launches:
            f()
        return self.locs, self.logits

    def layer_table(self):
        writers = {}

        def record(v: View, scope):
            lst = [w for w in writers.get(id(v.buf), []) if w[1] <= v.ch_off or w[0] >= v.ch_off + v.C]
            lst.append((v.ch_off, v.ch_off + v.C, scope))
            writers[id(v.buf)] = lst

        def producers(v: View):
            if v.buf is self.images.buf:
                return ["inputs"]
            inside = sorted(w for w in writers.get(id(v.buf), []) if w[0] >= v.ch_off and w[1] <= v.ch_off + v.C)
            assert inside and inside[0][0] == v.ch_off and inside[-1][1] == v.ch_off + v.C and \
                all(a[1] == b[0] for a, b in zip(inside, inside[1:])), "input view is not tiled by earlier outputs"
            return [w[2] for w in inside]

        table = []
        for op in self.fwd:
            if isinstance(op, PoolOp):
                table.append({"scope": op.scope, "op": op.kind + "_pool2d", "in_channels": op.x.C, "out_channels": op.out.C,
                              "kernel": [op.k, op.k], "stride": op.stride, "pad": [op.pad, op.pad],
                              "out_hw": [op.out.H, op.out.W], "inputs": producers(op.x)})
                record(op.out, op.scope)
                continue
            ins = producers(op.x)
            off = 0
            for m in op.members:
                e = {"scope": m.scope, "op": "conv2d", "in_channels": 3 if op.x.buf is self.images.buf else op.Cin,
                     "out_channels": m.K, "kernel": [op.R, op.S], "stride": op.stride, "pad": [op.pad_t, op.pad_l],
                     "out_hw": [op.out.H, op.out.W], "inputs": ins, "bn": op.kind in ("bn", "frozen"),
                     "bias": op.kind == "residual", "activation": "relu" if (op.relu and op.kind != "residual") else None}
                if op.kind == "residual":
                    e["residual"] = {"scale": op.rscale, "skip": producers(op.skip), "activation": "relu" if op.relu else None}
                table.append(e)
                if op.kind != "head":
                    record(op.out.slice(off, m.K), m.scope)
                off += m.K
        return table

    def flops_per_image(self, train=True):
        total = 0.0
        for op in self.convs:
            f = 2.0 * (op.M // self.B) * op.K * op.Cin * op.R * op.S
            total += f * (3.0 if (train and op.trainable) else 1.0)
        return total

    def barrier_timeouts(self):
        if self.mode != "train":
            return 0
        return int(self.bn_timeouts_total) + int(float(self.step_ctl[0]))

    def zero_grads(self):
        n_clear = self.G_off if self.fine_tune else self.G.numel()
        _lib.check(_lib.lib().mbx_step_begin(self.G.data_ptr(), n_clear, self.bn_ws.data_ptr(), self.bn_ws.numel(),
                                             self.nBt, self.bn_timeouts_total.data_ptr(), self.reg_loss.data_ptr(),
                                             torch.cuda.current_stream().cuda_stream), "step_begin")
        if self.fine_tune:
            self.Wg[self.head_w_start:].zero_()

    def backward(self):
        if self._i5_used:
            self.i5_counters.zero_()
        for f in self.bwd_launches:
            f()
        self.run_deferred_wgrad()

    def run_deferred_wgrad(self):
        if self._default_groups is None:
            jobs = [j for j in self.bwd_jobs if j is not None]
            n = max(1, (len(jobs) + 3) // 4)
            self._default_groups = self.make_wgrad_groups([jobs[i:i + n] for i in range(0, len(jobs), n)])
        for g in self._default_groups:
            g.launch()


class PoolOp:
    def __init__(self, net, kind, x: View, out: View, k, stride, pad):
        self.net, self.kind, self.x, self.out, self.k, self.stride, self.pad = net, kind, x, out, k, stride, pad
        self.argmax = None
        if kind == "max" and net.mode == "train" and not net.fine_tune:
            self.argmax = torch.zeros((out.N, out.H, out.W, out.C), dtype=torch.uint8, device=net.dev)

    def needs_backward(self):
        return self.net.mode == "train" and not self.net.fine_tune

    def forward(self):
        l, x, y = _lib.lib(), self.x, self.out
        s = torch.cuda.current_stream().cuda_stream
        if self.kind == "max":
            _lib.check(l.mbx_maxpool_fwd(x.ptr, x.img_stride, x.ld, x.N, x.H, x.W, x.C, self.k, self.stride, y.ptr,
                                         y.img_stride, y.ld, y.H, y.W, None if self.argmax is None else self.argmax.data_ptr(), s),
                       "maxpool_fwd")
        else:
            _lib.check(l.mbx_avgpool_fwd(x.ptr, x.img_stride, x.ld, x.N, x.H, x.W, x.C, self.k, self.pad, y.ptr,
# ... 15 lines not shown
```

multibox_amd/ops.py:

```python
from __future__ import annotations

import ctypes as C
import os

import torch

from . import _lib

EPI_STORE, EPI_AFFINE, EPI_RESIDUAL, EPI_STORE_F32 = 0, 1, 2, 3


class ConvDesc(C.Structure):
    _fields_ = [
        ("x", C.c_void_p), ("x_img_stride", C.c_int64), ("ldx", C.c_int32),
        ("N", C.c_int32), ("H_in", C.c_int32), ("W_in", C.c_int32), ("C_in", C.c_int32),
        ("w", C.c_void_p), ("C_out", C.c_int32), ("R", C.c_int32), ("S", C.c_int32),
        ("stride", C.c_int32), ("transposed", C.c_int32), ("pad_t", C.c_int32), ("pad_l", C.c_int32),
        ("H_out", C.c_int32), ("W_out", C.c_int32),
        ("y", C.c_void_p), ("y_img_stride", C.c_int64), ("ldy", C.c_int32),
        ("epilogue", C.c_int32), ("relu", C.c_int32), ("accumulate", C.c_int32),
        ("scale", C.c_void_p), ("shift", C.c_void_p),
        ("skip", C.c_void_p), ("skip_img_stride", C.c_int64), ("ld_skip", C.c_int32), ("rscale", C.c_float),
        ("stats_partial", C.c_void_p),
        ("tile_config", C.c_int32),
# ... 9 lines not shown
    ]


class BnApplyDesc(C.Structure):
    _fields_ = [("barrier", C.c_void_p), ("a", C.c_void_p), ("ld_a", C.c_int32), ("beta", C.c_void_p), ("mean", C.c_void_p),
                ("rstd", C.c_void_p), ("moving_mean", C.c_void_p), ("moving_var", C.c_void_p), ("relu_thr", C.c_void_p),
                ("relu", C.c_int32), ("eps", C.c_float), ("decay", C.c_float), ("step_poison", C.c_void_p)]


class BnBwdFused(C.Structure):
    _fields_ = [("barrier", C.c_void_p), ("n", C.c_int32), ("c_begin", C.c_int32 * 4), ("y", C.c_void_p * 4), ("ld_y", C.c_int32 * 4),
                ("dy", C.c_void_p * 4), ("ld_dy", C.c_int32 * 4), ("mean", C.c_void_p * 4), ("rstd", C.c_void_p * 4),
                ("beta", C.c_void_p * 4), ("dbeta", C.c_void_p * 4), ("acc", C.c_void_p * 4), ("acc_ld", C.c_int32 * 4),
                ("relu", C.c_int32 * 4), ("step_poison", C.c_void_p)]


GRID_BARRIER_BYTES = 6400
BN_BWD_SLOTS = 8


def i5_tile_for(M, C_out, n_cus=256):
    best, best_key = None, None
    for i, (bm, bn) in enumerate(I5_TILES):
        if (bm, bn) == (128, 192):
            continue
        t = -(-M // bm) * -(-C_out // bn)
        key = (0, -t, 0) if t <= n_cus else (1, -(-t // n_cus), -(-t // n_cus) * bm * bn)
        if best_key is None or key < best_key:
            best, best_key = I5_FLAG + 1 + i, key
    return best


def fused_tail_rounds(desc, n_cus=256):
    M = desc.N * desc.H_out * desc.W_out
    if resident_applies(desc, min_images=1):
        return -(-desc.N * 4 // n_cus)
    if directw_applies(desc):
        th = max(1, 256 // desc.W_out)
        return -(-desc.N * -(-desc.H_out // th) // n_cus)
    return min(-(-(-(-M // bm) * -(-desc.C_out // bn)) // n_cus) for bm, bn in I5_TILES if (bm, bn) != (128, 192))


class WgradJob(C.Structure):
    _fields_ = [("desc", ConvDesc), ("dy", C.c_void_p), ("dy_img_stride", C.c_int64), ("ld_dy", C.c_int32),
                ("scale", C.c_float), ("dw", C.c_void_p), ("db", C.c_void_p)]


class WgradPlanInfo(C.Structure):
    _fields_ = [("n_layers", C.c_int32), ("n_items", C.c_int32), ("layers_off", C.c_int64), ("items_off", C.c_int64),
                ("queues_off", C.c_int64), ("heads_off", C.c_int64), ("flops", C.c_double), ("tally_off", C.c_int64)]


class View:
    __slots__ = ("buf", "N", "H", "W", "C", "ld", "ch_off", "elem_size")

    def __init__(self, buf, N, H, W, C, ld=None, ch_off=0, elem_size=2):
        self.buf, self.N, self.H, self.W, self.C = buf, N, H, W, C
        self.ld = C if ld is None else ld
        self.ch_off, self.elem_size = ch_off, elem_size
        assert buf.numel() * buf.element_size() >= N * H * W * self.ld * elem_size, "view larger than its buffer"

    @property
    def ptr(self):
        return self.buf.data_ptr() + self.ch_off * self.elem_size

    @property
    def img_stride(self):
        return self.H * self.W * self.ld

    @property
    def M(self):
        return self.N * self.H * self.W

    def slice(self, off, C):
        assert off + C <= self.C
        return View(self.buf, self.N, self.H, self.W, C, self.ld, self.ch_off + off, self.elem_size)

    def tensor(self):
        dt = self.buf.dtype
        flat = self.buf.reshape(-1)[: self.N * self.H * self.W * self.ld].reshape(self.N, self.H, self.W, self.ld)
        return flat[..., self.ch_off:self.ch_off + self.C]

    @staticmethod
    def alloc(N, H, W, C, ld=None, dtype=torch.bfloat16, device="cuda", zero=False):
        ld = C if ld is None else ld
        f = torch.zeros if zero else torch.empty
        buf = f((N, H, W, ld), dtype=dtype, device=device)
        if not zero and os.environ.get("MBX_POISON"):
            buf.fill_(float("nan"))
        return View(buf, N, H, W, C, ld, 0, torch.empty((), dtype=dtype).element_size())


def _stream():
    return torch.cuda.current_stream().cuda_stream


def _p(t):
    return None if t is None else t.data_ptr()


def make_desc(x: View, w, C_out, R, S, stride, pad_t, pad_l, y: View, transposed=0, epilogue=EPI_STORE, relu=0,
              accumulate=0, scale=None, shift=None, skip: View = None, rscale=0.0, stats=None, acc_src: View = None,
              stats_rows_mod=0, stats_ld=0, relu_bits=None, ld_bits=0):
    d = ConvDesc()
    d.x, d.x_img_stride, d.ldx = x.ptr, x.img_stride, x.ld
    d.N, d.H_in, d.W_in, d.C_in = x.N, x.H, x.W, x.C
    d.w, d.C_out, d.R, d.S = (w.data_ptr() if w is not None else None), C_out, R, S
    d.stride, d.transposed, d.pad_t, d.pad_l = stride, transposed, pad_t, pad_l
    d.H_out, d.W_out = y.H, y.W
    d.y, d.y_img_stride, d.ldy = y.ptr, y.img_stride, y.ld
    d.epilogue, d.relu, d.accumulate = epilogue, int(relu), int(accumulate)
    d.scale, d.shift = _p(scale), _p(shift)
    if skip is not None:
        d.skip, d.skip_img_stride, d.ld_skip = skip.ptr, skip.img_stride, skip.ld
    d.rscale = float(rscale)
    d.stats_partial = _p(stats)
    d.stats_rows_mod, d.stats_ld = int(stats_rows_mod), int(stats_ld)
    if acc_src is not None:
        d.acc_src, d.acc_img_stride, d.ld_acc = acc_src.ptr, acc_src.img_stride, acc_src.ld
    if relu_bits is not None:
        d.relu_bits, d.ld_bits = relu_bits.data_ptr(), int(ld_bits if ld_bits else relu_bits.shape[-1])
    return d


def conv(desc: ConvDesc):
    _lib.check(_lib.lib().mbx_conv(C.byref(desc), _stream()), "mbx_conv")


def conv_stats_rows(desc: ConvDesc):
    r = _lib.lib().mbx_conv_stats_rows(C.byref(desc))
    if r < 0:
        _lib.check(r, "mbx_conv_stats_rows")
    return r


def conv_wgrad(desc: ConvDesc, dy: View, dw, db=None):
    _lib.check(_lib.lib().mbx_conv_wgrad(C.byref(desc), dy.ptr, dy.img_stride, dy.ld, dw.data_ptr(), _p(db), _stream()),
               "mbx_conv_wgrad")


WG_OVERLAP_DEFAULT = 0


def wgrad_overlap_cus():
    return max(0, int(os.environ.get("MBX_WG_OVERLAP", WG_OVERLAP_DEFAULT)))


N_TILE_CONFIGS = 14
I5_FLAG = 32
I5_TILE_CONFIGS = (33, 34, 35, 36, 37, 38, 39)
I5_TILES = ((128, 64), (128, 128), (192, 128), (256, 128), (256, 64), (128, 192), (128, 256))
I7_TILE_CONFIG = 65
I7_COUNTERS = 32
SPLITK_FLAG = 128
DIRECT3_TILE_CONFIG = 96


def direct3_applies(desc: ConvDesc, min_pixels=300000):
    if os.environ.get("MBX_DIRECT3", "1") == "0":
        return False
    if desc.R != 3 or desc.S != 3 or desc.epilogue not in (EPI_STORE, EPI_AFFINE) or desc.accumulate or desc.skip \
            or desc.rscale != 0.0 or (desc.epilogue == EPI_AFFINE and desc.stats_partial) or desc.bn_bwd_stats:
        return False
    if desc.stride == 2 and not desc.transposed and desc.C_in == 8 and desc.C_out <= 32 and desc.C_out % 8 == 0:
        pass
    elif desc.stride != 1 or desc.C_in not in (32, 64) or desc.C_out > 64 or desc.C_out % 8 or (desc.C_in == 64 and desc.C_out > 48):
        return False
    if -(-desc.W_out // 32) * 32 > 1.15 * desc.W_out:
        return False
    return desc.N * desc.H_out * desc.W_out >= int(os.environ.get("MBX_DIRECT3_MIN_PIXELS", min_pixels))


DIRECTW_TILE_CONFIG = 97


def directw_applies(desc: ConvDesc, min_pixels=60000):
    if os.environ.get("MBX_DIRECTW", "1") == "0":
        return False
    if desc.R != 3 or desc.S != 3 or desc.stride != 1 or desc.epilogue not in (EPI_STORE, EPI_AFFINE) or desc.accumulate or desc.skip \
            or desc.rscale != 0.0 or (desc.epilogue == EPI_AFFINE and desc.stats_partial) or desc.bn_bwd_stats:
        return False
    if desc.C_in not in (32, 48, 64) or desc.C_out > 64 or desc.C_out % 8 or (desc.C_in == 64 and desc.C_out > 48):
        return False
    if not (8 <= desc.W_out <= 64) or desc.W_in > desc.W_out + 2:
        return False
    return desc.N * desc.H_out * desc.W_out >= int(os.environ.get("MBX_DIRECTW_MIN_PIXELS", min_pixels))


RESIDENT_TILE_CONFIG = 98


def resident_applies(desc: ConvDesc, min_images=32):
    if os.environ.get("MBX_RESIDENT", "1") == "0":
        return False
    if desc.R * desc.S not in (3, 7) or min(desc.R, desc.S) != 1 or desc.stride != 1 or desc.epilogue not in (EPI_STORE, EPI_AFFINE) \
            or desc.accumulate or desc.skip or desc.rscale != 0.0 or (desc.epilogue == EPI_AFFINE and desc.stats_partial) \
            or desc.bn_bwd_stats or desc.relu_bits:
        return False
    if desc.H_in != desc.H_out or desc.W_in != desc.W_out or not (64 <= desc.H_out * desc.W_out <= 289):
        return False
    if desc.N < int(os.environ.get("MBX_RESIDENT_MIN_IMAGES", min_images)):
        return False
    if not desc.x or not desc.w or not desc.y:
        hw = desc.H_out * desc.W_out
        if desc.C_out % 8:
            return False
        if desc.R * desc.S == 3:
            return hw == 64 and desc.C_in in (192, 224, 256)
        return 65 <= hw <= 289 and desc.C_in in (128, 160, 192)
    keep = desc.tile_config
    desc.tile_config = RESIDENT_TILE_CONFIG
    ok = _lib.lib().mbx_conv_supported(C.byref(desc)) == 0
    desc.tile_config = keep
    return ok


PWRES_DEFAULT = "2"
PWRES_TILE_CONFIG = 99


def pwres_applies(desc: ConvDesc, min_pixels=4096):
    mode = os.environ.get("MBX_PWRES", PWRES_DEFAULT)
    if mode == "0":
        return False
    if desc.R != 1 or desc.S != 1 or desc.stride != 1 or desc.pad_t or desc.pad_l or desc.stats_partial or desc.bn_bwd_stats:
        return False
    if desc.C_in not in (96, 128, 320, 384, 448) or desc.C_out < 256 or desc.C_out % 8:
        return False
    res = desc.epilogue == EPI_RESIDUAL
    accm = desc.epilogue == EPI_STORE and desc.relu_bits and not desc.skip
    if not (res or accm) or (mode == "2" and not accm):
        return False
    return desc.N * desc.H_out * desc.W_out >= int(os.environ.get("MBX_PWRES_MIN_PIXELS", min_pixels))


def splitk_slices(desc: ConvDesc, n_cus=256):
    if os.environ.get("MBX_SPLITK", "1") == "0" or desc.transposed or desc.epilogue != EPI_STORE or desc.accumulate or desc.skip:
        return 0
    ktot = desc.R * desc.S * desc.C_in
    M = desc.N * desc.H_out * desc.W_out
    tiles = ((M + 127) // 128) * ((desc.C_out + 63) // 64)
    if ktot < 8192 or tiles > 96:
        return 0
    s = int(os.environ.get("MBX_SPLITK_SLICES", "0")) or max(2, min(16, (2 * n_cus) // tiles))
    return min(s, 32)
_TUNED = {}
TUNE_STATS = {"hits": 0, "remeasured": 0, "rejected": 0}
_TUNE_FILE = os.path.join(os.path.dirname(os.path.abspath(__file__)), "tune_cache.json")


def _load_tune_cache():
    if os.environ.get("MBX_TUNE_CACHE", "1") != "0" and os.path.exists(_TUNE_FILE):
        try:
            import json
            with open(_TUNE_FILE) as f:
                _TUNED.update({k: int(v) for k, v in json.load(f).items()})
        except (OSError, ValueError):
            pass


def save_tune_cache(path=None):
    import json
    with open(path or _TUNE_FILE, "w") as f:
        json.dump(dict(sorted(_TUNED.items())), f, indent=0)


_load_tune_cache()


def autotune(desc: ConvDesc, key, candidates=None, iters=10):
    key = repr(key)
    if key in _TUNED:
        desc.tile_config = _TUNED[key]
        if _lib.lib().mbx_conv_supported(C.byref(desc)) == 0:
            TUNE_STATS["hits"] += 1
            return desc.tile_config
        del _TUNED[key]
        TUNE_STATS["rejected"] += 1
    TUNE_STATS["remeasured"] += 1
    if candidates is None:
        candidates = (0, 2, 4, 5, 6, 9, 10, 12, 13, 14)
        if os.environ.get("MBX_AUTOTUNE_SET") == "all":
            candidates = tuple(range(0, N_TILE_CONFIGS + 1))
    l = _lib.lib()
    best, best_t = 0, float("inf")
    s = _stream()
    iters = int(os.environ.get("MBX_TUNE_ITERS", iters))
    for cfg in candidates:
        desc.tile_config = cfg
        if l.mbx_conv(C.byref(desc), s) != 0:
            continue
        e0, e1 = torch.cuda.Event(enable_timing=True), torch.cuda.Event(enable_timing=True)
        e0.record()
        for _ in range(iters):
            l.mbx_conv(C.byref(desc), s)
        e1.record()
        e1.synchronize()
        t = e0.elapsed_time(e1)
        if t < best_t * 0.97 or (cfg == 0 and t < best_t):
            best, best_t = cfg, t
    desc.tile_config = best
    _TUNED[key] = best
    return best


def autotune_wgrad(desc: ConvDesc, dy: View, scale, dw, db, key, candidates=(0, 2, 3, 4, 7, 8, 9, 10), iters=10):
# ... 62 lines not shown
```

Baseline: 4385 images/sec.

## Batch independent multibox head convs and BN applies into grouped launches

Adds a dependency-level scheduler for the multibox head layers. Independent convolutions, forward and dgrad, are merged into a single grouped implicit-GEMM launch, and independent BN-apply ops into one grouped rows kernel. The aim is to cut the many small, under-occupied kernel launches across the prediction heads by running them concurrently in one grid. The cost is a forced common tile config (it may override tuned tiles), more kernel-argument payload, and more complex scheduling logic that falls back to serial when the onepass mode changes.

```diff
diff --git a/include/mbx.h b/include/mbx.h
--- a/include/mbx.h
+++ b/include/mbx.h
@@ -139,6 +139,9 @@
 int mbx_conv(const mbx_conv_desc* desc , mbx_stream_t stream);
 int mbx_conv_supported(const mbx_conv_desc* desc );
 int mbx_conv_pair(const mbx_conv_desc* a , const mbx_conv_desc* b , mbx_stream_t stream);
+#define MBX_CONV_GROUP_MAX 8
+int mbx_conv_group(const mbx_conv_desc* const* descs , int n, mbx_stream_t stream);
+int mbx_conv_group_supported(const mbx_conv_desc* const* descs , int n);
 size_t mbx_conv_splitk_workspace_bytes(const mbx_conv_desc* desc );
 
 int mbx_conv_wgrad(const mbx_conv_desc* desc , const void* dy,
@@ -193,6 +196,14 @@
                           float* rstd, float* moving_mean, float* moving_var, mbx_stream_t stream);
 int mbx_bn_apply_mapped(const void* y, int64_t M, int C, const float* mean, const float* rstd, const float* beta,
                         int relu, void* a, int ld_a, const mbx_chan_map* a_map , mbx_stream_t stream);
+#define MBX_BN_APPLY_GROUP_MAX 8
+typedef struct mbx_bn_apply_item {
+  const void* stats_fixed; int32_t rows; int64_t count; float eps, decay;
+  const void* y; int64_t M; int32_t C; const float* beta; int32_t relu; void* a; int32_t ld_a;
+  const mbx_chan_map* a_map;
+  float* mean; float* rstd; float* moving_mean; float* moving_var; float* relu_thr;
+} mbx_bn_apply_item;
+int mbx_bn_apply_fused_group(const mbx_bn_apply_item* items , int n, mbx_stream_t stream);
 int mbx_bn_apply_maxpool(const void* y, int N, int H, int W, int C, const float* mean, const float* rstd, const float* beta,
                          int relu, void* p, int64_t p_img_stride, int ld_p, int Ho, int Wo, uint8_t* argmax,
                          mbx_stream_t stream);
diff --git a/multibox_amd/_lib.py b/multibox_amd/_lib.py
--- a/multibox_amd/_lib.py
+++ b/multibox_amd/_lib.py
@@ -40,6 +40,8 @@
     "mbx_conv": (I, [P, P]),
     "mbx_conv_supported": (I, [P]),
     "mbx_conv_pair": (I, [P, P, P]),
+    "mbx_conv_group": (I, [P, I, P]),
+    "mbx_conv_group_supported": (I, [P, I]),
     "mbx_conv_splitk_workspace_bytes": (SZ, [P]),
     "mbx_conv_wgrad": (I, [P, P, C.c_int64, I, P, P, P]),
     "mbx_conv_wgrad_scaled": (I, [P, P, C.c_int64, I, F, P, P, P]),
@@ -62,6 +64,7 @@
     "mbx_bn_fold": (I, [P, P, P, F, I, P, P, P]),
     "mbx_bn_apply_fused": (I, [P, I, C.c_int64, F, F, P, C.c_int64, I, P, I, P, I, P, P, P, P, P]),
     "mbx_bn_apply_fused_mapped": (I, [P, I, C.c_int64, F, F, P, C.c_int64, I, P, I, P, I, P, P, P, P, P, P, P]),
+    "mbx_bn_apply_fused_group": (I, [P, I, P]),
     "mbx_bn_bwd_apply_rows": (I, [P, I, P, I, P, C.c_int64, I, P, P, P, P, P, P, P]),
     "mbx_bn_bwd_rows": (I, [C.c_int64, I]),
     "mbx_bn_bwd_onepass_workspace_bytes": (C.c_size_t, [I]),
@@ -95,6 +98,13 @@
 
 class ChanMap(C.Structure):
     _fields_ = [("n", C.c_int32), ("c_begin", C.c_int32 * 4), ("offset", C.c_int32 * 4)]
+
+
+class BnApplyItem(C.Structure):
+    _fields_ = [("stats_fixed", C.c_void_p), ("rows", C.c_int32), ("count", C.c_int64), ("eps", C.c_float), ("decay", C.c_float),
+                ("y", C.c_void_p), ("M", C.c_int64), ("C", C.c_int32), ("beta", C.c_void_p), ("relu", C.c_int32), ("a", C.c_void_p),
+                ("ld_a", C.c_int32), ("a_map", C.c_void_p), ("mean", C.c_void_p), ("rstd", C.c_void_p), ("moving_mean", C.c_void_p),
+                ("moving_var", C.c_void_p), ("relu_thr", C.c_void_p)]
 
 
 class BnBwdStats(C.Structure):
diff --git a/multibox_amd/build.py b/multibox_amd/build.py
--- a/multibox_amd/build.py
+++ b/multibox_amd/build.py
@@ -47,6 +47,8 @@
     headers = [os.path.join(CSRC, f) for f in os.listdir(CSRC) if f.endswith(".h")]
     headers.append(os.path.join(os.path.dirname(HERE), "include", "mbx.h"))
     headers.append(os.path.abspath(__file__))
+    if not force and os.path.exists(LIB) and not _newer(LIB, [os.path.join(CSRC, s) for s in SOURCES] + headers):
+        return LIB
     objs = []
     procs = []
     for src, flags in SOURCES.items():
diff --git a/multibox_amd/csrc/conv.hip b/multibox_amd/csrc/conv.hip
--- a/multibox_amd/csrc/conv.hip
+++ b/multibox_amd/csrc/conv.hip
@@ -232,6 +232,40 @@
 conv_igemm3_pair_kernel(const ConvK p0, const ConvK p1, const int n0) {
   if ((int)blockIdx.x < n0) conv_igemm3_body<BM, BN, WNW, WMW, EV, MODE, NSTG>(p0, (int)blockIdx.x, n0);
   else conv_igemm3_body<BM, BN, WNW, WMW, EV, MODE, NSTG>(p1, (int)blockIdx.x - n0, (int)gridDim.x - n0);
+}
+
+struct GroupK {
+  const unsigned short* x; const unsigned short* w; void* y; float* stats;
+  int x_img_stride, ldx, H_in, W_in, C_in, C_out, R, S, Ktot;
+  unsigned x_bytes, w_bytes, y_bytes;
+  int mul, pad_t, pad_l, W_out, HW_out, M, y_img_stride, ldy, stats_mod, stats_ld, tiles_m, tiles_n;
+  unsigned mg_hw, sh_hw, mg_w, sh_w;
+  float rscale, stats_cap;
+};
+struct GroupArgs { GroupK m[MBX_CONV_GROUP_MAX]; int start[MBX_CONV_GROUP_MAX + 1]; int n; };
+static_assert(sizeof(GroupArgs) <= 2048, "mbx_conv_group: the members travel by value in the kernel arguments");
+
+template <int BM, int EV, int NSTG>
+__global__ void __launch_bounds__(256)
+conv_group3_kernel(const GroupArgs a) {
+  const int bid = (int)blockIdx.x;
+  int i = 0;
+#pragma unroll
+  for (int j = 1; j < MBX_CONV_GROUP_MAX; ++j)
+    if (j < a.n && bid >= a.start[j]) i = j;
+  const GroupK& g = a.m[i];
+  ConvK p{};
+  p.x = g.x; p.w = g.w; p.y = g.y; p.stats = g.stats;
+  p.x_img_stride = g.x_img_stride; p.ldx = g.ldx; p.H_in = g.H_in; p.W_in = g.W_in; p.C_in = g.C_in;
+  p.C_out = g.C_out; p.R = g.R; p.S = g.S; p.Ktot = g.Ktot;
+  p.x_bytes = g.x_bytes; p.w_bytes = g.w_bytes; p.y_bytes = g.y_bytes;
+  p.mul = g.mul; p.pad_t = g.pad_t; p.pad_l = g.pad_l; p.W_out = g.W_out; p.HW_out = g.HW_out; p.M = g.M;
+  p.y_img_stride = g.y_img_stride; p.ldy = g.ldy; p.stats_mod = g.stats_mod; p.stats_ld = g.stats_ld;
+  p.tiles_m = g.tiles_m; p.tiles_n = g.tiles_n;
+  p.mg_hw = g.mg_hw; p.sh_hw = g.sh_hw; p.mg_w = g.mg_w; p.sh_w = g.sh_w;
+  p.rscale = g.rscale; p.stats_cap = g.stats_cap;
+  p.ksplit = 1; p.kps = 1 << 30;
+  conv_igemm3_body<BM, 64, 2, 2, EV, 0, NSTG>(p, bid - a.start[i], a.start[i + 1] - a.start[i]);
 }
 
 
@@ -1169,6 +1203,69 @@
   return MBX_ERR_UNSUPPORTED;
 }
 
+template <int BM, int EV, int NSTG>
+static int launch_group_inst(const GroupArgs& a, hipStream_t s) {
+  static bool attr = false;
+  const size_t lds = NSTG * (size_t)(BM + 64) * 128;
+  if (!attr) {
+    (void)hipFuncSetAttribute(reinterpret_cast<const void*>(conv_group3_kernel<BM, EV, NSTG>),
+                              hipFuncAttributeMaxDynamicSharedMemorySize, (int)lds);
+    attr = true;
+  }
+  hipLaunchKernelGGL((conv_group3_kernel<BM, EV, NSTG>), dim3(a.start[a.n]), dim3(256), lds, s, a);
+  MBX_LAUNCH_CHECK();
+  return MBX_OK;
+}
+
+static int conv_group_impl(const mbx_conv_desc* const* descs, int n, mbx_stream_t stream, int dry) {
+  if (!descs || n < 2 || n > MBX_CONV_GROUP_MAX) return MBX_ERR_INVALID_ARG;
+  for (int i = 0; i < n; ++i)
+    if (!descs[i]) return MBX_ERR_INVALID_ARG;
+  PairCapture c[MBX_CONV_GROUP_MAX];
+  for (int i = 0; i < n; ++i) {
+    g_capture.valid = 0;
+    const int st = conv_impl(descs[i], stream, 2);
+    if (st != MBX_OK) return st;
+    if (!g_capture.valid) return MBX_ERR_UNSUPPORTED;
+    c[i] = g_capture;
+    const PairCapture& q = c[i];
+    if (q.bm != c[0].bm || q.nstg != c[0].nstg || q.ev != c[0].ev || q.bn != 64 || q.wnw != 2 || q.wmw != 2 ||
+        (q.bm != 64 && q.bm != 128) || q.mode == 2 || (q.ev != 0 && q.ev != 1 && q.ev != 5) || q.k.ksplit != 1)
+      return MBX_ERR_UNSUPPORTED;
+  }
+  int order[MBX_CONV_GROUP_MAX];
+  for (int i = 0; i < n; ++i) order[i] = i;
+  std::stable_sort(order, order + n, [&](int a, int b) { return c[a].k.Ktot > c[b].k.Ktot; });
+  GroupArgs a;
+  memset(&a, 0, sizeof(a));
+  a.n = n;
+  for (int j = 0; j < n; ++j) {
+    const ConvK& k = c[order[j]].k;
+    GroupK& g = a.m[j];
+    g.x = k.x; g.w = k.w; g.y = k.y; g.stats = k.stats;
+    g.x_img_stride = k.x_img_stride; g.ldx = k.ldx; g.H_in = k.H_in; g.W_in = k.W_in; g.C_in = k.C_in;
+    g.C_out = k.C_out; g.R = k.R; g.S = k.S; g.Ktot = k.Ktot;
+    g.x_bytes = k.x_bytes; g.w_bytes = k.w_bytes; g.y_bytes = k.y_bytes;
+    g.mul = k.mul; g.pad_t = k.pad_t; g.pad_l = k.pad_l; g.W_out = k.W_out; g.HW_out = k.HW_out; g.M = k.M;
+    g.y_img_stride = k.y_img_stride; g.ldy = k.ldy; g.stats_mod = k.stats_mod; g.stats_ld = k.stats_ld;
+    g.tiles_m = k.tiles_m; g.tiles_n = k.tiles_n;
+    g.mg_hw = k.mg_hw; g.sh_hw = k.sh_hw; g.mg_w = k.mg_w; g.sh_w = k.sh_w;
+    g.rscale = k.rscale; g.stats_cap = k.stats_cap;
+    a.start[j + 1] = a.start[j] + k.tiles_m * k.tiles_n;
+  }
+  if (dry) return MBX_OK;
+  hipStream_t s = mbx_s(stream);
+#define MBX_GROUP(BM_, NSTG_)                                                                                     \
+  if (c[0].bm == BM_ && c[0].nstg == NSTG_)                                                                       \
+    return c[0].ev == 5 ? launch_group_inst<BM_, 5, NSTG_>(a, s)                                                  \
+           : c[0].ev ? launch_group_inst<BM_, 1, NSTG_>(a, s) : launch_group_inst<BM_, 0, NSTG_>(a, s);
+  MBX_GROUP(128, 2) MBX_GROUP(128, 3) MBX_GROUP(64, 2) MBX_GROUP(64, 3)
+#undef MBX_GROUP
+  return MBX_ERR_UNSUPPORTED;
+}
+extern "C" int mbx_conv_group(const mbx_conv_desc* const* descs, int n, mbx_stream_t stream) { return conv_group_impl(descs, n, stream, 0); }
+extern "C" int mbx_conv_group_supported(const mbx_conv_desc* const* descs, int n) { return conv_group_impl(descs, n, nullptr, 1); }
+
 extern "C" size_t mbx_conv_splitk_workspace_bytes(const mbx_conv_desc* d) {
   if (!d || d->tile_config <= kSplitFlag || d->tile_config > kSplitFlag + kSplitMax) return 0;
   int ksplit, kps;
diff --git a/multibox_amd/csrc/nnops.hip b/multibox_amd/csrc/nnops.hip
--- a/multibox_amd/csrc/nnops.hip
+++ b/multibox_amd/csrc/nnops.hip
@@ -387,24 +387,25 @@
 }
 
 constexpr int kRowsMaxC = 2048;
-__global__ void __launch_bounds__(kT)
-bn_apply_rows_kernel(const float* __restrict__ part, int rows, double inv_count, float eps, float decay,
-                     const unsigned short* __restrict__ y, long long M, int C, const float* __restrict__ beta, int relu,
-                     unsigned short* __restrict__ a, int ld_a, float* __restrict__ mean, float* __restrict__ rstd,
-                     float* __restrict__ mmean, float* __restrict__ mvar, const ChanMap map, float* __restrict__ thr, int xcd_rows) {
+__device__ __forceinline__ void
+bn_apply_rows_body(const float* __restrict__ part, int rows, double inv_count, float eps, float decay,
+                   const unsigned short* __restrict__ y, long long M, int C, const float* __restrict__ beta, int relu,
+                   unsigned short* __restrict__ a, int ld_a, float* __restrict__ mean, float* __restrict__ rstd,
+                   float* __restrict__ mmean, float* __restrict__ mvar, const ChanMap& map, float* __restrict__ thr, int xcd_rows,
+                   const int bid, const int nblk) {
   extern __shared__ __attribute__((aligned(16))) float s_par[];
   const int C8 = C >> 3;
   const int rpi = kT / C8 > 0 ? kT / C8 : 1;
   const int vc = threadIdx.x % C8, rr = threadIdx.x / C8;
   const bool active = rr < rpi;
   const int c = vc << 3;
-  long long step = (long long)gridDim.x * rpi, Mend = M;
-  long long m = (long long)blockIdx.x * rpi + rr;
-  if (xcd_rows && gridDim.x >= 8) {
-    const int xcd = (int)blockIdx.x & 7, nx = ((int)gridDim.x - xcd + 7) >> 3;
+  long long step = (long long)nblk * rpi, Mend = M;
+  long long m = (long long)bid * rpi + rr;
+  if (xcd_rows && nblk >= 8) {
+    const int xcd = bid & 7, nx = (nblk - xcd + 7) >> 3;
     const long long perx = ((M + 7) / 8 + rpi - 1) / rpi * rpi;
     const long long lo = (long long)xcd * perx;
-    step = (long long)nx * rpi; m = lo + (long long)((int)blockIdx.x >> 3) * rpi + rr; Mend = lo + perx < M ? lo + perx : M;
+    step = (long long)nx * rpi; m = lo + (long long)(bid >> 3) * rpi + rr; Mend = lo + perx < M ? lo + perx : M;
   }
   constexpr int kRowsAhead = 4;
   u32x4 pre[kRowsAhead];
@@ -457,7 +458,7 @@
     if (poisoned) var = (double)__builtin_nanf("");
     const float fm = poisoned ? __builtin_nanf("") : (float)mu, fr = poisoned ? __builtin_nanf("") : (float)(1.0 / sqrt(var + (double)eps)), be = half ? be1 : be0;
     s_par[ch] = fm; s_par[C + ch] = fr; s_par[2 * C + ch] = be;
-    if (blockIdx.x == 0) {
+    if (bid == 0) {
       mean[ch] = fm; rstd[ch] = fr;
       if (thr) thr[ch] = relu ? fm - be / fr : -__builtin_inff();
       if (decay < 0.f) {
@@ -500,6 +501,37 @@
     finish(m, cur);
     cur = nxt;
   }
+}
+
+__global__ void __launch_bounds__(kT)
+bn_apply_rows_kernel(const float* __restrict__ part, int rows, double inv_count, float eps, float decay,
+                     const unsigned short* __restrict__ y, long long M, int C, const float* __restrict__ beta, int relu,
+                     unsigned short* __restrict__ a, int ld_a, float* __restrict__ mean, float* __restrict__ rstd,
+                     float* __restrict__ mmean, float* __restrict__ mvar, const ChanMap map, float* __restrict__ thr, int xcd_rows) {
+  bn_apply_rows_body(part, rows, inv_count, eps, decay, y, M, C, beta, relu, a, ld_a, mean, rstd, mmean, mvar, map, thr, xcd_rows,
+                     (int)blockIdx.x, (int)gridDim.x);
+}
+
+struct BnRowsK {
+  const float* part; const unsigned short* y; const float* beta; unsigned short* a;
+  float* mean; float* rstd; float* mmean; float* mvar; float* thr;
+  double inv_count; long long M;
+  int rows, C, relu, ld_a; float eps, decay;
+  ChanMap map;
+};
+struct BnRowsGroup { BnRowsK k[MBX_BN_APPLY_GROUP_MAX]; int start[MBX_BN_APPLY_GROUP_MAX + 1]; int n; int xcd_rows; };
+static_assert(sizeof(BnRowsGroup) <= 2048, "mbx_bn_apply_fused_group: the problems travel by value in the kernel arguments");
+__global__ void __launch_bounds__(kT)
+bn_apply_rows_group_kernel(const BnRowsGroup g) {
+  const int bid = (int)blockIdx.x;
+  int i = 0;
+#pragma unroll
+  for (int j = 1; j < MBX_BN_APPLY_GROUP_MAX; ++j)
+    if (j < g.n && bid >= g.start[j]) i = j;
+  const BnRowsK& k = g.k[i];
+  const ChanMap map = k.map;
+  bn_apply_rows_body(k.part, k.rows, k.inv_count, k.eps, k.decay, k.y, k.M, k.C, k.beta, k.relu, k.a, k.ld_a, k.mean, k.rstd,
+                     k.mmean, k.mvar, map, k.thr, g.xcd_rows, bid - g.start[i], g.start[i + 1] - g.start[i]);
 }
 
 __global__ void __launch_bounds__(kT)
@@ -2006,6 +2038,39 @@
   return MBX_OK;
 }
 
+extern "C" int mbx_bn_apply_fused_group(const mbx_bn_apply_item* items, int n, mbx_stream_t stream) {
+  if (!items || n < 1 || n > MBX_BN_APPLY_GROUP_MAX) return MBX_ERR_INVALID_ARG;
+  BnRowsGroup g;
+  memset(&g, 0, sizeof(g));
+  int maxC = 0;
+  for (int i = 0; i < n; ++i) {
+    const mbx_bn_apply_item& t = items[i];
+    if (!t.stats_fixed || !t.y || !t.a || !t.beta || !t.mean || !t.rstd || t.rows <= 0 || t.M <= 0 || t.C <= 0 || t.C % 8 || t.ld_a % 8 ||
+        t.count <= 0 || !al16(t.y) || !al16(t.a) || !al16(t.stats_fixed))
+      return MBX_ERR_INVALID_ARG;
+    if (t.rows > 16 || t.C > kRowsMaxC) return MBX_ERR_UNSUPPORTED;
+    BnRowsK& k = g.k[i];
+    if (to_chan_map(t.a_map, t.C, k.map) != MBX_OK) return MBX_ERR_INVALID_ARG;
+    k.part = reinterpret_cast<const float*>(t.stats_fixed); k.y = (cus)t.y; k.beta = t.beta; k.a = (us)t.a;
+    k.mean = t.mean; k.rstd = t.rstd; k.mmean = t.moving_mean; k.mvar = t.moving_var; k.thr = t.relu_thr;
+    k.inv_count = 1.0 / (double)t.count; k.M = (long long)t.M;
+    k.rows = t.rows; k.C = t.C; k.relu = t.relu; k.ld_a = t.ld_a; k.eps = t.eps; k.decay = t.decay;
+    if (t.C > maxC) maxC = t.C;
+  }
+  MBX_ENTER();
+  static const int rows_blocks = env_int("MBX_BN_ROWS_BLOCKS", 1024);
+  for (int i = 0; i < n; ++i) {
+    const int C8 = g.k[i].C / 8, rpi = kT / C8 > 0 ? kT / C8 : 1;
+    long long b = (g.k[i].M + rpi - 1) / rpi;
+    if (b > rows_blocks) b = rows_blocks;
+    g.start[i + 1] = g.start[i] + (int)b;
+  }
+  g.n = n; g.xcd_rows = xcd_rows_on();
+  hipLaunchKernelGGL(bn_apply_rows_group_kernel, dim3((unsigned)g.start[n]), dim3(kT), (size_t)3 * maxC * sizeof(float), mbx_s(stream), g);
+  MBX_LAUNCH_CHECK();
+  return MBX_OK;
+}
+
 extern "C" int mbx_bn_apply_fused(const float* stats_partial, int rows, int64_t count, float eps, float decay, const void* y,
                                   int64_t M, int C, const float* beta, int relu, void* a, int ld_a, float* mean,
                                   float* rstd, float* mmean, float* mvar, mbx_stream_t stream) {
diff --git a/multibox_amd/engine.py b/multibox_amd/engine.py
--- a/multibox_amd/engine.py
+++ b/multibox_amd/engine.py
@@ -8,7 +8,7 @@
 import numpy as np
 import torch
 
-from . import _lib, ops
+from . import _lib, head_schedule, ops
 from .ops import View
 
 BN_EPS = 0.001
@@ -90,6 +90,10 @@
         self.fuse_bwd = (mode == "train" and not self.deterministic and not self.bw_stats and torch.device(device).type == "cuda"
                          and os.environ.get("MBX_FUSE_BWD", "0") == "1")
         self.fused_bwd_launches = self.fused_bwd_layers = 0
+        self.head_levels = (mode == "train" and os.environ.get("MBX_HEAD_LEVELS", "1") != "0" and not self.fuse_apply
+                            and not self.fuse_bwd and not self.bw_stats)
+        self.head_groups = []
+        self.head_plan = {}
         self.relu_bits = mode == "train" and os.environ.get("MBX_RELU_BITS", "1") != "0"
         self.autotune = torch.device(device).type == "cuda" and bool(int(os.environ.get("MBX_AUTOTUNE", "1")))
         self.bn_max_wg = int(os.environ.get("MBX_BN_MAX_WG", "0")) or (bn_max_workgroups or 0)
@@ -806,12 +810,23 @@
 
     def _build_forward_launches(self):
         L = []
+        n_before, prev_op = 0, None
         l = _lib.lib()
         st = lambda: torch.cuda.current_stream().cuda_stream
-        for op in self.fwd:
+        Node, R = head_schedule.Node, self._res
+        first_head = next((i for i, o in enumerate(self.fwd) if getattr(o, "is_head", False)), len(self.fwd)) if self.head_levels else len(self.fwd)
+        nodes = []
+        for fi, op in enumerate(self.fwd):
+            heads_on = fi >= first_head
+            if fi > first_head and len(L) > n_before:
+                self._wrap_head_launches(L, n_before, prev_op, nodes)
+            n_before, prev_op = len(L), op
             if isinstance(op, PoolOp):
                 if not getattr(op, "fused_fwd", False):
-                    L.append(op.forward)
+                    if heads_on:
+                        nodes.append(Node(op.scope or "pool", "other", [R(op.x)], [R(op.out)], run=op.forward))
+                    else:
+                        L.append(op.forward)
                 continue
             if op.kind == "bn" and op.group is not None:
                 g = op.group
@@ -825,10 +840,16 @@
                 g.rows[i] = ops.conv_stats_rows(d)
                 assert use16 or g.rows[i] * op.K * 2 <= (g.stats_off[i + 1] - g.stats_off[i] if i + 1 < len(g.members) else 1 << 62)
                 g.fwd_desc[i] = d
+                lev = heads_on and use16
+                if lev:
+                    nodes.append(Node(op.name, "conv", [R(op.x)], [R(op.y_view), (("stats16", g.members[0].stats16_base), g.koff[i], g.koff[i] + op.K)],
+                                      run=lambda d=d, op=op: _lib.check(l.mbx_conv(C.byref(d), st()), op.name), key="stats", payload=d))
+                if lev and i + 1 < len(g.members):
+                    continue
                 if i + 1 < len(g.members):
                     L.append(lambda d=d, op=op, g=g: None if g.pair_fwd else _lib.check(l.mbx_conv(C.byref(d), st()), op.name))
                     continue
-                if len(g.members) == 2 and torch.device(self.dev).type == "cuda" and os.environ.get("MBX_CONV_PAIR", "1") != "0":
+                if not lev and len(g.members) == 2 and torch.device(self.dev).type == "cuda" and os.environ.get("MBX_CONV_PAIR", "1") != "0":
                     g.pair_fwd = l.mbx_conv_pair(C.byref(g.fwd_desc[0]), C.byref(d), st()) == 0
                 lead, n = g.members[0], len(g.members)
                 parts = (C.c_void_p * n)(*[self.stats_scratch.data_ptr() + 4 * o for o in g.stats_off])
@@ -840,6 +861,17 @@
                 var, beta = self._sl(self.bn_var, lead.beta_off, g.K), self._sl(self.Bt, lead.beta_off, g.K)
                 thr = self._sl(self.bn_thr, lead.beta_off, g.K)
                 s16 = self.stats16[lead.stats16_base:]
+                if lev:
+                    def aargs(op=op, g=g, amap=amap, a_ptr=a_ptr, mean=mean, rstd=rstd, mm=mm, mv=mv, var=var, beta=beta, thr=thr, s16=s16):
+                        decay = self.bn_decay
+                        if self.defer_moving:
+                            mm, mv, decay = None, var, -1.0
+                        return (s16.data_ptr(), STATS_ROWS, op.M, BN_EPS, decay, g.y.data_ptr(), op.M, g.K, beta.data_ptr(), int(op.relu),
+                                a_ptr, op.out.ld, C.addressof(amap), mean.data_ptr(), rstd.data_ptr(), ops._p(mm), ops._p(mv), thr.data_ptr())
+                    nodes.append(self._apply_node("+".join(m.name for m in g.members), aargs,
+                                                  [(id(g.y), 0, g.K), (("stats16", lead.stats16_base), 0, g.K)],
+                                                  [R(m.out) for m in g.members] + [("bn", lead.beta_off, lead.beta_off + g.K)]))
+                    continue
 
                 def run(d=d, op=op, g=g, parts=parts, rows_a=rows_a, cs_a=cs_a, amap=amap, a_ptr=a_ptr, mean=mean, rstd=rstd,
                         mm=mm, mv=mv, var=var, beta=beta, n=n, use16=use16, thr=thr, s16=s16):
@@ -907,6 +939,20 @@
                         self._keep_ba = getattr(self, "_keep_ba", []) + [ba]
                     else:
                         fd = ba = None
+
+                if heads_on and use16 and fd is None and fpool is None:
+                    nodes.append(Node(op.name, "other" if S_ else "conv", [R(op.x)], [R(yv), (("stats16", op.stats16_base), 0, op.K)],
+                                      run=lambda d=d, op=op: _lib.check(l.mbx_conv(C.byref(d), st()), op.name), key="stats", payload=d))
+
+                    def aargs(op=op, mean=mean, rstd=rstd, mm=mm, mv=mv, var=var, beta=beta, thr=thr, s16=s16, out=out):
+                        decay = self.bn_decay
+                        if self.defer_moving:
+                            mm, mv, decay = None, var, -1.0
+                        return (s16.data_ptr(), STATS_ROWS, op.M, BN_EPS, decay, op.y_view.ptr, op.M, op.K, beta.data_ptr(), int(op.relu),
+                                out.ptr, out.ld, None, mean.data_ptr(), rstd.data_ptr(), ops._p(mm), ops._p(mv), thr.data_ptr())
+                    nodes.append(self._apply_node(op.name, aargs, [R(yv), (("stats16", op.stats16_base), 0, op.K)],
+                                                  [R(out), ("bn", op.beta_off, op.beta_off + op.K)]))
+                    continue
 
                 def run(d=d, rows=rows, op=op, mean=mean, rstd=rstd, mm=mm, mv=mv, beta=beta, out=out, var=var, fpool=fpool,
                         use16=use16, thr=thr, s16=s16, fd=fd, ba=ba):
@@ -954,11 +1000,119 @@
                 L.append(lambda d=d, op=op: _lib.check(l.mbx_conv(C.byref(d), st()), op.name))
             elif op.kind == "head":
                 d = self._desc(op, op.out, epilogue=ops.EPI_STORE_F32)
-                L.append(lambda d=d, op=op: _lib.check(l.mbx_conv(C.byref(d), st()), op.name))
+                conv = lambda d=d, op=op: _lib.check(l.mbx_conv(C.byref(d), st()), op.name)
+                gather = lambda: _lib.check(l.mbx_head_gather_all(self.head_table, len(self.heads), self.B, self.P,
+                                                                  self.locs.data_ptr(), self.logits.data_ptr(), st()), "head_gather_all")
+                if heads_on:
+                    nodes.append(Node(op.name, "conv", [R(op.x)], [R(op.out)], run=conv, key="f32", payload=d))
+                    if op is self.heads[-1]:
+                        nodes.append(Node("head_gather_all", "other", [R(h.out) for h in self.heads], [("locs", 0, 1)], run=gather))
+                    continue
+                L.append(conv)
                 if op is self.heads[-1]:
-                    L.append(lambda: _lib.check(l.mbx_head_gather_all(self.head_table, len(self.heads), self.B, self.P,
-                                                                      self.locs.data_ptr(), self.logits.data_ptr(), st()), "head_gather_all"))
+                    L.append(gather)
+        if len(L) > n_before and len(self.fwd) > first_head:
+            self._wrap_head_launches(L, n_before, prev_op, nodes)
+        if nodes:
+            L.extend(fn for fn, _ in self._head_launches(nodes, "fwd"))
         return L
+
+    @staticmethod
+    def _res(v: View):
+        return (id(v.buf), v.ch_off, v.ch_off + v.C)
+
+    def _wrap_head_launches(self, L, n0, op, nodes):
+        fns = L[n0:]
+        del L[n0:]
+
+        def run(fns=fns):
+            for f in fns:
+                f()
+        w = [self._res(op.out), ("scratch", 0, 1)]
+        if getattr(op, "y_view", None) is not None:
+            w.append(self._res(op.y_view))
+            lead = op if op.group is None else op.group.members[0]
+            w.append((("stats16", lead.stats16_base), 0, 1 << 20))
+        nodes.append(head_schedule.Node(getattr(op, "name", None) or getattr(op, "scope", "pool"), "other",
+                                        [self._res(op.x), ("scratch", 0, 1)], w, run=run))
+
+    def _head_bwd_nodes(self, op, pre, ddesc, fdesc, dg_info, slot, nodes):
+        l = _lib.lib()
+        st = lambda: torch.cuda.current_stream().cuda_stream
+        Node, R = head_schedule.Node, self._res
+        if pre is not None:
+            if op.kind == "head":
+                rd, wr = [("d_locs", 0, 1)], [R(h.head_grad) for h in self.heads]
+                name = "head_scatter_all"
+            else:
+                mem = [op] if op.group is None else op.group.members
+                lead = mem[0]
+                rd = [R(self._gview(m.out)) for m in mem] + [R(m.y_view) for m in mem]
+                wr = [R(m.dy_view) for m in mem] + [("dbeta", lead.beta_off, lead.beta_off + sum(m.K for m in mem))]
+                if self.no_onepass or lead.bn_ws_off < 0 or getattr(op, "fused_pool", None) is not None:
+                    wr.append(("scratch", 0, 1))
+                name = "bn backward " + "+".join(m.name for m in mem)
+            nodes.append(Node(name, "other", rd, wr, run=lambda pre=pre: pre(st()), slot=slot))
+        if ddesc is None:
+            return
+        dyin, gx, acc, acc_src, mr = dg_info
+        rd = [R(dyin)] + ([R(gx)] if acc and acc_src is None else []) + ([R(acc_src)] if acc_src is not None else []) + ([R(mr.out)] if mr is not None else [])
+
+        def run(ddesc=ddesc, op=op):
+            ddesc.max_workgroups = self.cu_cap
+            _lib.check(l.mbx_conv(C.byref(ddesc), st()), "dgrad " + op.name)
+        plain = (fdesc is None and not acc and acc_src is None and mr is None and op.stride == 1 and not ddesc.bn_bwd_stats
+                 and not ddesc.relu_bits)
+        nodes.append(Node("dgrad " + op.name, "conv" if plain else "other", rd, [R(gx)], run=run, key="dgrad", payload=ddesc, slot=slot))
+
+    def _apply_node(self, name, aargs, reads, writes):
+        l = _lib.lib()
+        run = lambda: _lib.check(l.mbx_bn_apply_fused_mapped(*aargs(), torch.cuda.current_stream().cuda_stream), "bn_apply_fused_mapped")
+        return head_schedule.Node(name, "apply", reads, writes, run=run, key="rows", payload=aargs)
+
+    def _can_group(self, key, members):
+        if key[0] == "apply":
+            return True
+        descs = [m.payload for m in members]
+        arr = (C.c_void_p * len(descs))(*[C.addressof(d) for d in descs])
+        l = _lib.lib()
+        if l.mbx_conv_group_supported(arr, len(descs)) == 0:
+            return True
+        keep = [d.tile_config for d in descs]
+        for d in descs:
+            d.tile_config = ops.CONV_GROUP_TILE
+        if l.mbx_conv_group_supported(arr, len(descs)) == 0:
+            return True
+        for d, t in zip(descs, keep):
+            d.tile_config = t
+        return False
+
+    def _head_launches(self, nodes, direction):
+        l = _lib.lib()
+        st = lambda: torch.cuda.current_stream().cuda_stream
+        sched = head_schedule.plan(nodes, self._can_group, ops.CONV_GROUP_MAX)
+        self.head_plan[direction] = (nodes, sched)
+        out = []
+        for launch in sched:
+            if len(launch) == 1:
+                out.append((launch[0].run, launch))
+                continue
+            kind, names = launch[0].kind, [n.name for n in launch]
+            self.head_groups.append((direction, kind, names))
+            if kind == "conv":
+                arr = (C.c_void_p * len(launch))(*[C.addressof(n.payload) for n in launch])
+                out.append((lambda arr=arr, n=len(launch), what="conv group " + " | ".join(names):
+                            _lib.check(l.mbx_conv_group(arr, n, st()), what), launch))
+            else:
+                items = (_lib.BnApplyItem * len(launch))()
+
+                def run(items=items, launch=launch):
+                    for it, nd in zip(items, launch):
+                        for (f, _), v in zip(_lib.BnApplyItem._fields_, nd.payload()):
+                            setattr(it, f, v)
+                    _lib.check(l.mbx_bn_apply_fused_group(items, len(launch), st()), "bn_apply_fused_group")
+                out.append((run, launch))
+        return out
 
     def _gview(self, v: View) -> View:
         return self.grad_of(v)
@@ -1026,7 +1180,12 @@
         L = []
         self.bwd_ops = []
         self.bwd_jobs = []
-        for op in reversed(self.fwd):
+        Node, R = head_schedule.Node, self._res
+        first_head = next((i for i, o in enumerate(self.fwd) if getattr(o, "is_head", False)), len(self.fwd)) if self.head_levels else len(self.fwd)
+        bnodes = []
+        for fi in range(len(self.fwd) - 1, -1, -1):
+            op = self.fwd[fi]
+            heads_on = fi >= first_head
             if isinstance(op, PoolOp):
                 if op.needs_backward():
                     prod = self._pool_producer(op)
@@ -1037,6 +1196,9 @@
                     acc, src = self._claim(gx)
                     assert src is None, "a pooling layer cannot be the first writer of a residual block's input gradient"
                     L.append(op.make_backward(self._gview(op.out), gx, acc))
+                    if heads_on:
+                        bnodes.append(Node((op.scope or "pool") + " backward", "other", [R(self._gview(op.out))] + ([R(gx)] if acc else []), [R(gx)],
+                                           run=L[-1], slot=len(L) - 1))
                     self.bwd_ops.append(op)
                     self.bwd_jobs.append(None)
                 continue
@@ -1145,7 +1307,7 @@
                     if self.no_onepass:
                         split(s)
                 self.fused_bwd_layers += 1
-            ddesc = fdesc = None
+            ddesc = fdesc = dg_info = None
             if op.need_dx:
                 gx = self._gview(op.x)
                 acc, acc_src = self._claim(gx)
@@ -1163,6 +1325,7 @@
                     if torch.device(self.dev).type != "cuda" or l.mbx_conv_supported(C.byref(alt)) == 0:
                         ddesc, mr.relu_bits = alt, bits
                 self._tune(op, ddesc, "dgrad")
+                dg_info = (dyin, gx, acc, acc_src, mr)
                 if op.fb_segments is not None:
                     assert acc == 0 and acc_src is None and mr is None, op.name
                     fdesc = ops.ConvDesc.from_buffer_copy(ddesc)
@@ -1215,9 +1378,22 @@
                         return
                     ddesc.max_workgroups = self.cu_cap
                     _lib.check(l.mbx_conv(C.byref(ddesc), s), "dgrad " + op.name)
+            if heads_on:
+                self._head_bwd_nodes(op, pre, ddesc, fdesc, dg_info, len(L), bnodes)
             L.append(run)
             self.bwd_ops.append(op)
             self.bwd_jobs.append(job)
+        if bnodes:
+            n_slots = 1 + max(n.slot for n in bnodes)
+            self._head_plan_no_onepass = self.no_onepass
+            launches = self._head_launches(bnodes, "bwd")
+            for k, (a, b) in enumerate(head_schedule.slots([nd for _, nd in launches], n_slots)):
+                def run(serial=L[k], fns=[fn for fn, _ in launches[a:b]]):
+                    if self.no_onepass != self._head_plan_no_onepass or self._probe_skip_bn_bwd:
+                        return serial()
+                    for f in fns:
+                        f()
+                L[k] = run
         if torch.device(self.dev).type == "cuda" and os.environ.get("MBX_CONV_PAIR", "1") != "0":
             for grp in self.bn_groups:
                 if len(grp.members) == 2 and len(grp.dgrad_desc) == 2 and not any(getattr(m, "fdesc", None) is not None for m in grp.members):
diff --git a/multibox_amd/head_schedule.py b/multibox_amd/head_schedule.py
--- /dev/null
+++ b/multibox_amd/head_schedule.py
@@ -0,0 +1,72 @@
+from __future__ import annotations
+
+
+class Node:
+    __slots__ = ("name", "kind", "key", "reads", "writes", "run", "payload", "slot", "pos")
+
+    def __init__(self, name, kind, reads, writes, run=None, key=None, payload=None, slot=0):
+        self.name, self.kind, self.key = name, kind, key
+        self.reads, self.writes = tuple(reads), tuple(writes)
+        self.run, self.payload, self.slot, self.pos = run, payload, slot, -1
+
+    def __repr__(self):
+        return "Node(%s, %s)" % (self.name, self.kind)
+
+
+def overlap(a, b):
+    return any(x[0] == y[0] and x[1] < y[2] and y[1] < x[2] for x in a for y in b)
+
+
+def hazard(m, n):
+    return overlap(m.writes, n.reads) or overlap(m.writes, n.writes) or overlap(m.reads, n.writes)
+
+
+def levels(nodes):
+    lv = []
+    for i, n in enumerate(nodes):
+        lv.append(max([lv[j] + 1 for j in range(i) if hazard(nodes[j], n)], default=0))
+    return lv
+
+
+def plan(nodes, can_group=None, max_group=8):
+    for i, n in enumerate(nodes):
+        n.pos = i
+    lv = levels(nodes)
+    order = sorted(range(len(nodes)), key=lambda i: (lv[i], i))
+    out, open_groups = [], {}
+
+    def flush(key):
+        members = open_groups.pop(key)
+        if len(members) > 1 and (can_group is None or can_group(key, members)):
+            out.append(members)
+        else:
+            out.extend([m] for m in members)
+
+    for i in order:
+        n = nodes[i]
+        for key in list(open_groups):
+            if any(hazard(m, n) for m in open_groups[key]):
+                flush(key)
+        if n.kind in ("conv", "apply"):
+            open_groups.setdefault((n.kind, n.key), []).append(n)
+            if len(open_groups[(n.kind, n.key)]) == max_group:
+                flush((n.kind, n.key))
+        else:
+            out.append([n])
+    for key in list(open_groups):
+        flush(key)
+    return out
+
+
+def slots(schedule, n_slots):
+    last = [-1] * n_slots
+    for i, launch in enumerate(schedule):
+        for n in launch:
+            last[n.slot] = max(last[n.slot], i)
+    out, prev, hi = [], 0, -1
+    for k in range(n_slots):
+        hi = max(hi, last[k])
+        end = len(schedule) if k == n_slots - 1 else max(prev, hi + 1)
+        out.append((prev, end))
+        prev = end
+    return out
diff --git a/multibox_amd/ops.py b/multibox_amd/ops.py
--- a/multibox_amd/ops.py
+++ b/multibox_amd/ops.py
@@ -185,6 +185,8 @@
 I5_TILES = ((128, 64), (128, 128), (192, 128), (256, 128), (256, 64), (128, 192), (128, 256))
 I7_TILE_CONFIG = 65
 I7_COUNTERS = 32
+CONV_GROUP_MAX = 8
+CONV_GROUP_TILE = 5
 SPLITK_FLAG = 128
 DIRECT3_TILE_CONFIG = 96
 
```

Result: no change. 4419 images/sec, median of 6 (+0.8%).
